# zijinxuxu/PDFNet

Measured on AMD Instinct MI355X. Metric: train-step images/sec @256x256 RGB-D B=32, higher is better.
Workload: dtype f32

## Files before the change

### include/pdfnet_hip.h

```cpp
#ifndef PDFNET_HIP_H
#define PDFNET_HIP_H
#ifdef __cplusplus
extern "C" {
#endif

#define PDF_E_BADARG (-1)
#define PDF_E_WORKSPACE (-2)
#define PDF_ACT_NONE 0
#define PDF_ACT_RELU 1
#define PDF_ACT_LRELU01 2


int pdf_linear_fwd(const float* x, const float* w, const float* bias, float* y,
                   int M, int N, int K, int ldx, int ldw, int ldy, int act, void* stream);
int pdf_linear_bwd_weight(const float* x, const float* dy, float* dw, float* db, float* ws, long ws_floats,
                          int M, int N, int K, int ldx, int lddy, int accumulate, void* stream);
long pdf_wgrad_workspace_floats(int M, int NI, int NJ);
int pdf_init(void);
int pdf_debug_init_device(void);
int pdf_debug_kernel_timing(int on);
int pdf_set_stats_output(float* part, long cap_floats);
long pdf_stats_result_tiles(void);
long pdf_stats_result_rows(void);
int pdf_set_bn_tile_stats(const float* part, long tiles, long rows_per_tile);
int pdf_debug_kernel_record_count(void);
int pdf_debug_kernel_record(int i, char* name, int cap, double* flops, double* bytes, float* ms);
int pdf_stream_wait(void* waiter, void* signaler);
int pdf_set_gemm_precision(int bf16);
int pdf_debug_gemm_precision(void);
int pdf_debug_last_tile(void);
int pdf_debug_igemm_launches(void);
int pdf_linear_bwd_data(const float* dy, const float* w, float* dx, int M, int N, int K, int lddy, int ldw, int lddx, void* stream);
int pdf_linear_fwd_pair(const float* x, const float* w0, const float* w1, const float* b0, const float* b1, float* y,
                        int M, int N, int K, int ldx, int ldw, int ldy, int act, void* stream);
int pdf_linear_bwd_data_pair(const float* dy, const float* w0, const float* w1, float* dx, int M, int N, int K,
                             int lddy, int ldw, int lddx, void* stream);
int pdf_linear_bwd_weight_pair(const float* x, const float* dy, float* dw0, float* dw1, float* db0, float* db1,
                               float* ws, long ws_floats, int M, int N, int K, int ldx, int lddy, int accumulate, void* stream);

int pdf_conv2d_fwd(const float* x, const float* w, const float* bias, float* y,
                   int N, int H, int W, int Cin, int ldx, int Cout, int KH, int KW,
                   int stride, int pad, int OH, int OW, int ldy, int act, void* stream);
int pdf_conv2d_bwd_data(const float* dy, const float* w, float* dx,
                        int N, int H, int W, int Cin, int lddx, int Cout, int KH, int KW,
                        int stride, int pad, int OH, int OW, int lddy, void* stream);
int pdf_conv2d_bwd_data_add(const float* dy, const float* w, float* dx,
                        int N, int H, int W, int Cin, int lddx, int Cout, int KH, int KW,
                        int stride, int pad, int OH, int OW, int lddy, void* stream);
int pdf_conv2d_bwd_weight(const float* x, const float* dy, float* dw, float* db, float* ws, long ws_floats,
                          int N, int H, int W, int Cin, int ldx, int Cout, int KH, int KW,
                          int stride, int pad, int OH, int OW, int lddy, int accumulate, void* stream);

int pdf_deconv2d_fwd(const float* x, const float* w, const float* bias, float* y,
                     int N, int H, int W, int Cin, int ldx, int Cout, int KH, int KW,
                     int stride, int pad, int OH, int OW, int ldy, void* stream);
int pdf_deconv2d_bwd_data(const float* dy, const float* w, float* dx,
                          int N, int H, int W, int Cin, int lddx, int Cout, int KH, int KW,
                          int stride, int pad, int OH, int OW, int lddy, void* stream);
int pdf_deconv2d_bwd_weight(const float* x, const float* dy, float* dw, float* ws, long ws_floats,
                            int N, int H, int W, int Cin, int ldx, int Cout, int KH, int KW,
                            int stride, int pad, int OH, int OW, int lddy, int accumulate, void* stream);
int pdf_bmm_strided(const float* A, const float* B, float* C, int batch, int M, int N, int K, int RB,
                    long sab, long sar, long sam, long sak, long sbb, long sbr, long sbk, long sbn,
                    long scb, long scm, long scn, int beta, void* stream);


int pdf_knn_ball_group(const float* pts, int ldp, int C, int Bc, int N, int S, int K, float r2,
                       int* idx, float* grouped, int ldg, void* stream);
int pdf_group_bwd(const float* dg, int ldg, const int* idx, float* dpts, int ldd, int C,
                  int Bc, int N, int S, int K, void* stream);
int pdf_gather_sub_fwd(const float* u, int ldu, const float* v, int ldv, const int* idx, int Bc, int N, int S, int K, int C,
                       float* y, int ldy, void* stream);
int pdf_gather_sub_bwd(const float* dy, int lddy, const int* idx, float* du, int ldu, float* dv, int ldv,
                       int Bc, int N, int S, int K, int C, void* stream);
int pdf_invert_index(const int* idx, int Bc, int N, int E, int* start, int* list, int* tmp, void* stream);
int pdf_gather_sub_bwd_sorted(const float* dy, int lddy, const int* start, const int* list, float* du, int ldu, float* dv, int ldv,
                              int Bc, int N, int S, int K, int C, void* stream);
int pdf_gather_rows(const float* feat, int ldf, int C, long HW, const long* ind, long ind_bstride,
                    int B, int M, int R, int shift, float* out, int ldo, void* stream);
int pdf_scatter_rows_add(const float* dout, int ldo, int C, long HW, const long* ind, long ind_bstride,
                         int B, int M, int R, int shift, float* dfeat, int ldf, void* stream);
int pdf_window_op(float* feat, int ldf, int C, int H, int W, const long* ind, long ind_bstride,
                  int B, int M, int r, float* buf, const float* src, int mode, void* stream);
int pdf_nms_top1(const float* hm, int BC, int H, int W, long* ind, float* score, void* stream);
int pdf_maxk_fwd(const float* x, int ldx, int C, long R, int K, float* y, int ldy, int* arg, void* stream);
int pdf_maxk_bwd(const float* dy, int ldy, const int* arg, int C, long R, int K, float* dx, int ldx, void* stream);
int pdf_bn_relu_maxk_fwd(const float* y, int ldy, int C, long R, int K, const float* gamma, const float* beta,
                         float* running_mean, float* running_var, float momentum, float eps, int training,
                         float* out, int ldo, int* arg, float* save_mean, float* save_rstd, float* scale, float* shift,
                         float* ws, void* stream);
int pdf_bn_relu_maxk_bwd(const float* dout, int lddo, const int* arg, const float* y, int ldy, const float* save_mean, const float* save_rstd,
                         const float* gamma, const float* scale, const float* shift, int C, long R, int K,
                         float* dy, int lddy, float* dgamma, float* dbeta, int accumulate, float* ws, void* stream);
long pdf_sa_fused_workspace_floats(int Bc, int S, int K, int C1, int C2, int C3);
int pdf_sa_fused_fwd(const float* u, const float* v, const int* idx, int Bc, int N, int S, int K, int C1, int C2, int C3,
                     const float* w2, const float* b2, const float* w3, const float* b3,
                     const float* gamma1, const float* beta1, const float* gamma2, const float* beta2, const float* gamma3, const float* beta3,
                     float* rmean1, float* rvar1, float* rmean2, float* rvar2, float* rmean3, float* rvar3, float momentum, float eps, int training,
                     float* out, int* arg, float* zsel, float* saved, float* ws, long ws_floats, void* stream);
int pdf_sa_fused_bwd(const float* dout, const float* u, const float* v, const int* idx, int Bc, int N, int S, int K, int C1, int C2, int C3,
                     const float* w2, const float* b2, const float* w3, const float* b3,
                     const float* out, const int* arg, const float* zsel, const float* saved,
                     float* dz1, float* dw2, float* db2, float* dw3, float* db3,
                     float* dgamma1, float* dbeta1, float* dgamma2, float* dbeta2, float* dgamma3, float* dbeta3,
                     float* ws, long ws_floats, void* stream);


long pdf_bn_workspace_floats(int C, long R);
int pdf_bn_train_fwd(const float* x, int ldx, int C, long R, const float* gamma, const float* beta,
                     float* running_mean, float* running_var, float momentum, float eps,
                     const float* res, int ldr, int relu, float* y, int ldy,
                     float* save_mean, float* save_rstd, float* scale, float* shift, float* ws, void* stream);
int pdf_bn_eval_fwd(const float* x, int ldx, int C, long R, const float* gamma, const float* beta,
                    const float* running_mean, const float* running_var, float eps,
                    const float* res, int ldr, int relu, float* y, int ldy, float* scale, float* shift, void* stream);
int pdf_bn_train_bwd(const float* dy, int lddy, const float* y, int ldy, int relu, const float* x, int ldx,
                     const float* save_mean, const float* save_rstd, const float* gamma,
                     const float* scale, const float* shift, int C, long R,
                     float* dx, int lddx, float* dres, int lddr, float* dgamma, float* dbeta, int accumulate,
                     float* ws, void* stream);
int pdf_bn_eval_bwd(const float* dy, int lddy, const float* y, int ldy, int relu, const float* x, int ldx,
                    const float* running_mean, const float* running_var, float eps, const float* scale, const float* shift,
                    int C, long R, float* dx, int lddx, float* dres, int lddr,
                    float* dgamma, float* dbeta, int accumulate, float* ws, void* stream);
int pdf_bn_relu_maxk_eval_bwd(const float* dout, int lddo, const int* arg, const float* y, int ldy,
                              const float* running_mean, const float* running_var, float eps, const float* scale, const float* shift,
                              int C, long R, int K, float* dy, int lddy, float* dgamma, float* dbeta, int accumulate, float* ws, void* stream);
int pdf_colsum(const float* g, int ldg, int C, long R, float* out, int accumulate, float* ws, void* stream);
int pdf_colsum_pair(const float* g, int ldg, int C, long R, float* out0, float* out1, int accumulate, float* ws, void* stream);
int pdf_layernorm_fwd(const float* x, int ldx, int F, long R, const float* gamma, const float* beta, float eps,
                      float* y, int ldy, float* mean, float* rstd, void* stream);
int pdf_layernorm_bwd(const float* dy, int lddy, const float* x, int ldx, int F, long R, const float* gamma,
                      const float* mean, const float* rstd, float* dx, int lddx, float* dgamma, float* dbeta, void* stream);
int pdf_layernorm_fused_fwd(const float* x, int ldx, const float* add, int ldadd, float p, unsigned long long seed,
                            const unsigned long long* step, int F, long R, long R_split,
                            const float* gamma0, const float* beta0, const float* gamma1, const float* beta1, float eps, int act,
                            float* z, int ldz, float* y, int ldy, float* mean, float* rstd, void* stream);
int pdf_layernorm_fused_bwd(const float* dy, int lddy, const float* y, int ldy, int act, const float* z, int ldz, int F, long R, long R_split,
                            const float* gamma0, const float* gamma1, const float* mean, const float* rstd,
                            const float* dz_in, int lddzin, float* dz, int lddz, float* dadd, int lddadd,
                            float p, unsigned long long seed, const unsigned long long* step,
                            float* dgamma0, float* dbeta0, float* dgamma1, float* dbeta1, void* stream);
int pdf_l2norm_fwd(const float* x, int ldx, int C, long R, const float* w, float eps, float* y, int ldy, float* norm, void* stream);
int pdf_l2norm_bwd(const float* dy, int lddy, const float* x, int ldx, int C, long R, const float* w, float eps,
                   const float* norm, float* dx, int lddx, float* dw, void* stream);
int pdf_l2norm_cat_fwd(int nparts, const float* const* x, const int* C, const float* const* w, float eps, long R,
                       float* y, int ldy, float* const* norm, void* stream);
int pdf_l2norm_cat_bwd(int nparts, const float* dy, int lddy, const float* const* x, const int* C, const float* const* w, float eps, long R,
                       float* const* norm, float* const* dx, float* const* dw, void* const* dx16_or_null, void* stream);

int pdf_act_fwd(const float* x, int ldx, float* y, int ldy, int C, long R, int act, void* stream);
int pdf_act_bwd(const float* dy, int lddy, const float* y, int ldy, float* dx, int lddx, int C, long R, int act, void* stream);
int pdf_sft_fwd(const float* fea, int ldf, const float* scale, int lds, const float* shift, int ldh,
                float* out, int ldo, int C, long R, void* stream);
int pdf_sft_bwd(const float* g, int ldg, const float* fea, int ldf, const float* scale, int lds,
                float* dfea, int lddf, float* dscale, int ldds, int C, long R, void* stream);
int pdf_sft3_fwd(const float* fea, int ldf, const float* cond, int ldc, const float* w_scale0, const float* b_scale0,
                 const float* w_scale1, const float* b_scale1, const float* w_shift0, const float* b_shift0,
                 const float* w_shift1, const float* b_shift1, float* out, int ldo, long R, void* stream);
int pdf_sft3_bwd(const float* g, int ldg, const float* fea, int ldf, const float* cond, int ldc,
                 const float* w_scale0, const float* b_scale0, const float* w_scale1, const float* b_scale1,
                 const float* w_shift0, const float* b_shift0, const float* w_shift1, const float* b_shift1,
                 float* dfea, int lddf, float* dcond, int lddc,
                 float* dw_scale0, float* db_scale0, float* dw_scale1, float* db_scale1,
                 float* dw_shift0, float* db_shift0, float* dw_shift1, float* db_shift1, int accumulate,
                 float* ws, long R, void* stream);
int pdf_set_bf16_operands(const void* op0_bf16, const void* op1_bf16);
int pdf_set_bf16_output(void* out_bf16);
int pdf_set_bn_input_bf16(const void* x16);
int pdf_set_input_affine_relu(const float* scale, const float* shift);
int pdf_cast_bf16(const float* src, void* dst, long n, void* stream);
int pdf_cast_bf16_transposed(const float* src, void* dst, const void* table, int nlayers, long total_tiles, void* stream);
int pdf_debug_shadow_operands(void);
int pdf_dropout(const float* x, float* y, long n, float p, unsigned long long seed, const unsigned long long* step, void* stream);
int pdf_dropout_add(const float* x, const float* res, float* y, long n, float p, unsigned long long seed,
                    const unsigned long long* step, void* stream);
int pdf_maxpool3s2_fwd(const float* x, int N, int H, int W, int C, float* y, unsigned char* arg, void* stream);
int pdf_maxpool3s2_bwd(const float* dy, const unsigned char* arg, int N, int H, int W, int C, float* dx, void* stream);
int pdf_maxpool3s2_bwd_add(const float* dy, const unsigned char* arg, int N, int H, int W, int C, float* dx, void* stream);
int pdf_upsample2x_fwd(const float* x, int N, int H, int W, int C, float* y, void* stream);
int pdf_upsample2x_bwd(const float* dy, int N, int H, int W, int C, float* dx, void* stream);
int pdf_pad2d(const float* src, int lds, long R, int C, float* dst, int ldd, long R2, int C2, void* stream);
int pdf_adam_step(float* p, const float* g, float* m, float* v, long n, float lr, float b1, float b2, float eps,
                  const float* corr, float grad_scale, void* stream);

int pdf_cheby2_fwd(const float* x, int ldx, int B, int V, int F, const int* col, const float* val, int Wd,
                   float* out, int ldo, void* stream);
int pdf_cheby2_bwd(const float* d, int ldd, int B, int V, int F, const int* colT, const float* valT, int Wd,
                   float* dx, int lddx, void* stream);
int pdf_cheby2_fwd_pair(const float* x, int ldx, int B, int V, int F, const int* col0, const float* val0,
                        const int* col1, const float* val1, int Wd, float* out, int ldo, void* stream);
int pdf_cheby2_bwd_pair(const float* d, int ldd, int B, int V, int F, const int* colT0, const float* valT0,
                        const int* colT1, const float* valT1, int Wd, float* dx, int lddx, void* stream);
int pdf_attn_fwd(const float* q, const float* k, const float* v, int ld, int B, int V, int H, int dh, int kv_shift,
                 float pdrop, unsigned long long seed, const unsigned long long* step, float* out, int ldo, float* stat, void* stream);
int pdf_attn_bwd(const float* q, const float* k, const float* v, int ld, const float* o, const float* dout, int ldo,
                 const float* stat, int B, int V, int H, int dh, int kv_shift, float pdrop, unsigned long long seed, const unsigned long long* step,
                 float* dq, float* dk, float* dv, int lddq, float* dvec, void* stream);

int pdf_fps(const float* xyz, int ld, int Bc, int N, int S, const int* start, int* idx, void* stream);

int pdf_rowloss_fwd(const float* pred, const float* tgt, long rows, long n, int mode, float* out, void* stream);
int pdf_rowloss_bwd(const float* pred, const float* tgt, const float* gout, long rows, long n, int mode, float* dpred, void* stream);
int pdf_face_loss_fwd(const float* pred, const float* gt, const long long* faces, int G, int B, int V, int Fc, float* part, void* stream);
int pdf_face_loss_bwd(const float* pred, const float* gt, const long long* faces, int G, int B, int V, int Fc,
                      const float* wn, const float* we, float* dpred, void* stream);

long pdf_dense_loss_workspace_floats(int B);
int pdf_dense_loss_fwd(const float* mask, const float* mask_gt, int mask_c, int mask_hw,
                       const float* hms, const float* hms_gt, int hms_c, int hms_hw,
                       const float* hm, const float* hm_gt, int hm_c, int hm_hw, int B, float* ws, float* out, void* stream);
int pdf_dense_loss_bwd(const float* mask, const float* mask_gt, float* dmask, int mask_c, int mask_hw,
                       const float* hms, const float* hms_gt, float* dhms, int hms_c, int hms_hw,
                       const float* hm, const float* hm_gt, float* dhm, int hm_c, int hm_hw, int B,
                       const float* g_mask, const float* g_hms, const float* g_hm, const float* stat, void* stream);
int pdf_point_dist_sum(const float* pred, const float* gt, int rows, int n, int dim, float* out, void* stream);

int pdf_procrustes_dist(const float* pred, const float* gt, int rows, int n, float* sum, float* dist, float* aligned, void* stream);
int pdf_mesh_nn_counts(const float* pred, const float* gt, int rows, int n, const float* thr, int T, int* counts, float* d_gt, float* d_pred,
                       void* stream);
int pdf_mesh_penetration(const float* verts, const long long* faces, int B, int n, int Fc,
                         float* wind, float* dist, int* count, float* depth, float* gap, void* stream);

int pdf_mesh_icp(const float* verts, const long long* faces, const float* cloud, const float* valid, int B, int n, int Fc, int P, int iters,
                 float trim, int rigid, float* out_verts, float* R, float* t, float* rms, int* inliers, float* closest, int* tri, void* stream);
int pdf_cloud_mesh_loss(const float* verts, const long long* faces, const float* cloud, const float* valid, int B, int n, int Fc, int P, float trim,
                        float* loss, int* inliers, float* grad, int* tri, float* closest, float* bary, void* stream);
int pdf_mesh_cloud_loss(const float* verts, const long long* faces, const float* cloud, const float* valid, int B, int n, int Fc, int P, float trim,
                        float margin, float* loss, int* inliers, int* visible, float* grad, int* vis, int* nn, void* stream);
int pdf_penetration_loss(const float* verts, const long long* faces, const float* valid, int B, int n, int Fc,
                         float* loss, int* count, float* grad_self, float* grad_other,
                         int* inside, int* tri, float* bary, float* closest, void* stream);
int pdf_silhouette_loss(const float* verts, const long long* faces, const float* K, const float* mask, const float* weight,
                        const float* valid, const int* table, int B, int n, int Fc, int M, int H, int W, float sigma, float z_near,
                        float* scratch, float* loss, float* sums, float* trans, float* grad, void* stream);

int pdf_render_hands(const float* verts, const long long* faces, const float* K, const float* valid, const float* colour, int colour_per_sample,
                     const int* table, int B, int n, int Fc, int M, int H, int W, float z_near, int ambient_only, float* scratch,
                     int* face, float* depth, float* bary, float* rgb, void* stream);
int pdf_render_compare(const int* face_pred, const int* face_gt, const float* depth_pred, const float* sensor, int B, int H, int W, int Fc,
                       int* iou, float* res, void* stream);

int pdf_depth2pcl(const float* depth, const float* mask, const float* K, const float* valid, int B, int H, int W,
                  unsigned long long seed, long* choose, float* cloud, int* count, void* stream);

int pdf_mano_lbs_fwd(const float* root_aa, const float* pose_aa, const float* shape, const float* trans,
                     const float* v_template, const float* shapedirs, const float* posedirs, const float* J_reg,
                     const float* weights, int B, int left_side, int center_idx, float* verts, float* joints, void* stream);
int pdf_mano_lbs_bwd(const float* root_aa, const float* pose_aa, const float* shape,
                     const float* v_template, const float* shapedirs, const float* posedirs, const float* J_reg,
                     const float* weights, int B, int left_side, int center_idx, const float* dverts, const float* djoints,
                     float* droot, float* dpose, float* dshape, float* dtrans, void* stream);
int pdf_mano_split_coeff(const float* params, int ldp, long HW, const long* ind, const float* K, int B, int input_res, int down,
                         float* orient, float* pose, float* shape, float* trans, void* stream);
int pdf_mano_split_coeff_bwd(const float* params, float* dparams, int ldp, long HW, const long* ind, const float* K, int B, int input_res, int down,
                             const float* dorient, const float* dpose, const float* dtrans, void* stream);

long pdf_mano_fit_workspace_floats(int B);
int pdf_mano_fit(const float* target, const float* valid, const float* weight, const float* init,
                 const float* v_template, const float* shapedirs, const float* posedirs, const float* J_reg, const float* weights,
                 int B, int left_side, int iters, float prior_pose, float prior_shape,
                 float* params, float* verts, float* joints, float* cost, int* info, float* lambda, float* A, float* g,
                 float* workspace, void* stream);
int pdf_mano_cloud_targets(const float* verts, const long long* faces, const float* cloud, const float* valid, const float* anchor,
                           float anchor_weight, int B, int n, int Fc, int P, float trim, float* target, float* weight, float* rms,
                           int* inliers, int* tri, float* closest, float* bary, void* stream);
long pdf_mano_fit_cloud_workspace_floats(int B, int outer);
int pdf_mano_fit_cloud(const float* cloud, const long long* faces, const float* valid, const float* init, const float* anchor,
                       float anchor_weight, float trim, int outer, int inner, float prior_pose, float prior_shape,
                       const float* v_template, const float* shapedirs, const float* posedirs, const float* J_reg, const float* weights,
                       int B, int Fc, int P, int left_side,
                       float* params, float* verts, float* joints, float* rms, int* inliers, float* cost, int* info,
                       float* workspace, void* stream);


typedef struct PdfCallOpts {
    const void* op0_bf16; const void* op1_bf16;
    void* out_bf16;
    const void* bn_x_bf16;
    float* stats_out; long stats_cap;
    long stats_tiles; long stats_rows;
    const float* tile_stats; long tile_n; long tile_rows;
    const float* in_scale; const float* in_shift;
    const void* op1_bf16_t;
    float* ws; long ws_floats;
    const float* wino_v;
} PdfCallOpts;
long pdf_conv2d_winograd_v_offset(int N, int H, int W, int Cin, int Cout, int KH, int KW, int stride, int pad);
int pdf_linear_fwd_x(const float* x, const float* w, const float* bias, float* y, int M, int N, int K, int ldx, int ldw, int ldy, int act, void* stream, PdfCallOpts* opts);
int pdf_linear_fwd_pair_x(const float* x, const float* w0, const float* w1, const float* b0, const float* b1, float* y, int M, int N, int K, int ldx, int ldw, int ldy, int act, void* stream, PdfCallOpts* opts);
int pdf_linear_bwd_data_x(const float* dy, const float* w, float* dx, int M, int N, int K, int lddy, int ldw, int lddx, void* stream, PdfCallOpts* opts);
int pdf_linear_bwd_data_pair_x(const float* dy, const float* w0, const float* w1, float* dx, int M, int N, int K, int lddy, int ldw, int lddx, void* stream, PdfCallOpts* opts);
int pdf_conv2d_fwd_x(const float* x, const float* w, const float* bias, float* y, int N, int H, int W, int Cin, int ldx, int Cout, int KH, int KW, int stride, int pad, int OH, int OW, int ldy, int act, void* stream, PdfCallOpts* opts);
int pdf_conv2d_bwd_data_x(const float* dy, const float* w, float* dx, int N, int H, int W, int Cin, int lddx, int Cout, int KH, int KW, int stride, int pad, int OH, int OW, int lddy, void* stream, PdfCallOpts* opts);
int pdf_conv2d_bwd_data_add_x(const float* dy, const float* w, float* dx, int N, int H, int W, int Cin, int lddx, int Cout, int KH, int KW, int stride, int pad, int OH, int OW, int lddy, void* stream, PdfCallOpts* opts);
int pdf_linear_bwd_weight_x(const float* x, const float* dy, float* dw, float* db, float* ws, long ws_floats, int M, int N, int K, int ldx, int lddy, int accumulate, void* stream, PdfCallOpts* opts);
int pdf_linear_bwd_weight_pair_x(const float* x, const float* dy, float* dw0, float* dw1, float* db0, float* db1, float* ws, long ws_floats, int M, int N, int K, int ldx, int lddy, int accumulate, void* stream, PdfCallOpts* opts);
int pdf_conv2d_bwd_weight_x(const float* x, const float* dy, float* dw, float* db, float* ws, long ws_floats, int N, int H, int W, int Cin, int ldx, int Cout, int KH, int KW, int stride, int pad, int OH, int OW, int lddy, int accumulate, void* stream, PdfCallOpts* opts);
int pdf_deconv2d_fwd_x(const float* x, const float* w, const float* bias, float* y, int N, int H, int W, int Cin, int ldx, int Cout, int KH, int KW, int stride, int pad, int OH, int OW, int ldy, void* stream, PdfCallOpts* opts);
int pdf_deconv2d_bwd_data_x(const float* dy, const float* w, float* dx, int N, int H, int W, int Cin, int lddx, int Cout, int KH, int KW, int stride, int pad, int OH, int OW, int lddy, void* stream, PdfCallOpts* opts);
int pdf_deconv2d_bwd_weight_x(const float* x, const float* dy, float* dw, float* ws, long ws_floats, int N, int H, int W, int Cin, int ldx, int Cout, int KH, int KW, int stride, int pad, int OH, int OW, int lddy, int accumulate, void* stream, PdfCallOpts* opts);
int pdf_bn_train_fwd_x(const float* x, int ldx, int C, long R, const float* gamma, const float* beta, float* running_mean, float* running_var, float momentum, float eps, const float* res, int ldr, int relu, float* y, int ldy, float* save_mean, float* save_rstd, float* scale, float* shift, float* ws, void* stream, PdfCallOpts* opts);
int pdf_bn_train_bwd_x(const float* dy, int lddy, const float* y, int ldy, int relu, const float* x, int ldx, const float* save_mean, const float* save_rstd, const float* gamma, const float* scale, const float* shift, int C, long R, float* dx, int lddx, float* dres, int lddr, float* dgamma, float* dbeta, int accumulate, float* ws, void* stream, PdfCallOpts* opts);
int pdf_bn_relu_maxk_fwd_x(const float* y, int ldy, int C, long R, int K, const float* gamma, const float* beta, float* running_mean, float* running_var, float momentum, float eps, int training, float* out, int ldo, int* arg, float* save_mean, float* save_rstd, float* scale, float* shift, float* ws, void* stream, PdfCallOpts* opts);
int pdf_l2norm_cat_fwd_x(int nparts, const float* const* x, const int* C, const float* const* w, float eps, long R, float* y, int ldy, float* const* norm, void* stream, PdfCallOpts* opts);
long pdf_conv2d_winograd_workspace_floats(int N, int H, int W, int Cin, int Cout, int KH, int KW, int stride, int pad, int backward);
int pdf_debug_armed_slots(void);
int pdf_debug_callopts_size(void);

int pdf_x3_split(const float* x, void* out, long n, long cs, void* stream);
long pdf_deconv2d_x3_workspace_floats(int N, int H, int W, int Cin, int Cout, int KH, int KW, int stride, int pad, int backward);
int pdf_set_x3_mode(int mode);
int pdf_stream_create(void** out, int priority, int* lo, int* hi);
int pdf_debug_x3_mode(void);
int pdf_debug_workspace_plan(int kind, int pass, int N, int H, int W, int Cin, int Cout, int KH, int KW, int stride, int pad, long* out, int cap);
int pdf_debug_x3_stamps(unsigned long long* out);
int pdf_x3_batched_gemm_nt(const void* A3, long csA, const void* B3, long csB, float* C, int batch, long gsA, long gsB, long gsC, int M, int N, int K, int variant, int nprod, void* stream);
int pdf_batched_gemm_nt(const float* A, const float* B, float* C, int batch, long gsA, long gsB, long gsC, int M, int N, int K, void* stream);
int pdf_x3_batched_gemm_tn(const void* P3, long csP, const void* Q3, long csQ, float* slab, int batch, long gsP, long gsQ, int M, int NI, int NJ, int splits, int variant, int nprod, void* stream);
int pdf_batched_gemm_tn(const float* P, const float* Q, float* slab, int batch, long gsP, long gsQ, int M, int NI, int NJ, int splits, void* stream);

typedef struct PdfMeshLin { const float* w[2]; const float* b[2]; } PdfMeshLin;
typedef struct PdfMeshLN { const float* g[2]; const float* b[2]; } PdfMeshLN;
typedef struct PdfMeshGcn { PdfMeshLin fc1, fc2, sc; PdfMeshLN n2, n3; unsigned long long seed; } PdfMeshGcn;
typedef struct PdfMeshAttn {
    PdfMeshLN ln; PdfMeshLin q, k, v, fc; PdfMeshLN ffln; PdfMeshLin f1, f2;
    unsigned long long seed_att, seed_z, seed_t, seed_x;
} PdfMeshAttn;
typedef struct PdfMeshLinG { float* w[2]; float* b[2]; } PdfMeshLinG;
typedef struct PdfMeshLNG { float* g[2]; float* b[2]; } PdfMeshLNG;
typedef struct PdfMeshGcnG { PdfMeshLinG fc1, fc2, sc; PdfMeshLNG n2, n3; } PdfMeshGcnG;
typedef struct PdfMeshAttnG { PdfMeshLNG ln; PdfMeshLinG q, k, v, fc; PdfMeshLNG ffln; PdfMeshLinG f1, f2; } PdfMeshAttnG;
typedef struct PdfMeshLevel {
    int level, B, training, cin0;
    float p;
    const unsigned long long* step;
    const float* x;
    float* out;
    const int* ell_col[2]; const float* ell_val[2]; const int* ell_colT[2]; const float* ell_valT[2]; int ell_w;
    PdfMeshGcn gcn[4];
    PdfMeshAttn self_, cross;
    float* tape;
    float* qkv;
    const float* dout;
    float* dx;
    float* gtape;
    PdfMeshGcnG ggcn[4]; PdfMeshAttnG gself, gcross;
    float* wg_ws; long wg_ws_floats;
} PdfMeshLevel;
long pdf_mesh_tape_floats(int level, int B);
long pdf_mesh_gtape_floats(int level, int B);
int pdf_mesh_level_fwd(const PdfMeshLevel* a, void* stream);
int pdf_mesh_level_bwd(const PdfMeshLevel* a, void* stream, void* side_stream);
int pdf_mesh_level_fwd_bf16(const PdfMeshLevel* a, void* stream);
int pdf_mesh_level_bwd_bf16(const PdfMeshLevel* a, void* stream, void* side_stream);
int pdf_mesh_level_fwd_x3(const PdfMeshLevel* a, void* stream);
int pdf_mesh_level_bwd_x3(const PdfMeshLevel* a, void* stream, void* side_stream);
int pdf_debug_mesh_level_size(void);

typedef struct PdfMeshLoss {
    const float* vp; const float* v2p; const float* hd3; const float* hd2; const float* r;
    const float* vgt[2]; const float* jgt[2]; const float* v2gt[2]; const float* lmsgt[2];
    const long long* ind; const float* K; const float* valid;
    const float* reg[2]; const long long* faces; const long long* perm[2];
    int B, Fc, size, down;
    float* part;
    float* out;
    float coef[12];
    const float* gmp;
    int edge_grad;
    float* dvp; float* dv2p; float* dhd3; float* dhd2; float* dr;
} PdfMeshLoss;
int pdf_mesh_loss_fwd(const PdfMeshLoss* a, void* stream);
int pdf_mesh_loss_bwd(const PdfMeshLoss* a, void* stream);
int pdf_debug_mesh_loss_size(void);
int pdf_debug_mesh_stamps(unsigned long long* out);

#ifdef __cplusplus
}
#endif
#endif
```

### pdfnet_amd/csrc/gemm.hip

```cpp
#include "common.h"

#include "gemm_common.h"
#include "gemm_internal.h"

constexpr int WG_ISSUE_AT = 1;
typedef unsigned int u32x4v __attribute__((ext_vector_type(4)));
__device__ __forceinline__ float4 as_f4(const u32x4v& v) { return *reinterpret_cast<const float4*>(&v); }

template <int BM, int BN, int WM, int WN, bool FAST, bool KN, int BKT, bool BUF, bool AFF>
__device__ __forceinline__ void igemm_nt_body(const IGemm& g) {
    constexpr int NT = WM * WN * 64;
    constexpr int BK = BKT, LD = BK + 1;
    constexpr int TM = BM / WM / 32, TN = BN / WN / 32;
    constexpr int TPR = BK / 4, RPP = NT / TPR;
    constexpr int RA = BM / RPP, RB = BN / RPP;
    __shared__ __attribute__((aligned(16))) float As[2][BM * LD];
    __shared__ __attribute__((aligned(16))) float Bs[2][BN * LD];

    const int tid = threadIdx.x, lane = tid & 63, wave = tid >> 6;
    const int wm = wave / WN, wn = wave % WN;
    const float* __restrict__ Ap = g.A; const float* __restrict__ Bp = g.B; const float* __restrict__ biasp = g.bias;
    float* __restrict__ Cp = g.C;
    if (g.batch > 0) { Ap += (long)blockIdx.y * g.gsA; Bp += (long)blockIdx.y * g.gsB; Cp += (long)blockIdx.y * g.gsC; }
    else if (blockIdx.y) { Ap += g.gsA; Cp += g.gsC; Bp = g.B1; biasp = g.bias1; }
// ... 1814 lines not shown
        if (g.q_scale != nullptr && g.uniform != 2) return PDF_E_BADARG;
        KTimer kt(buf && g.q_scale != nullptr ? "wgemm_tn_dma_aff" : buf ? "wgemm_tn_dma<3, true>" : fast ? "wgemm_tn_dma<3, false>" : "wgemm_tn<128, 128, 2, 2, false, 16>",
                  wflops, wbytes, s);
        if (buf && g.q_scale != nullptr) hipLaunchKernelGGL(wgemm_tn_dma_aff, grid, dim3(256), 0, s, g);
        else if (buf) hipLaunchKernelGGL((wgemm_tn_dma<3, true>), grid, dim3(256), 0, s, g);
        else if (fast) hipLaunchKernelGGL((wgemm_tn_dma<3, false>), grid, dim3(256), 0, s, g);
        else hipLaunchKernelGGL((wgemm_tn<128, 128, 2, 2, false>), grid, dim3(256), 0, s, g);
    }
    PDF_LAUNCH_CHECK();
    if (splits > 1) {
        Reduce r = {ws, out, out1, per, bws, db, db1, (int)perb, splits, accumulate};
        const bool two_d = splits >= 16 && per <= (1L << 20);
        KTimer kt(two_d ? "reduce_slabs_2d" : "reduce_slabs", 0.0, 4.0 * groups * (splits + 1 + (accumulate ? 1 : 0)) * (per + perb), s);
        if (two_d) {
            const int mb = (int)((per + 63) / 64);
            hipLaunchKernelGGL(reduce_slabs_2d, dim3(mb + (int)((perb + 63) / 64), groups), dim3(256), 0, s, r, mb);
        } else {
            const int mb = grid_for(per);
            hipLaunchKernelGGL(reduce_slabs, dim3(mb + (perb ? cdiv(perb, 256) : 0), groups), dim3(256), 0, s, r, mb);
        }
        PDF_LAUNCH_CHECK();
    }
    return 0;
}

PDF_API long pdf_wgrad_workspace_floats(int M, int NI, int NJ) {
    const bool small = (NI <= 64 || NJ <= 64);
    const int B = small ? 64 : 128;
    long tiles = (long)cdiv(NI, B) * cdiv(NJ, B);
    int splits = (int)((1024 + tiles - 1) / tiles);
    int max_by_rows = cdiv(M, 128);
    if (splits > max_by_rows) splits = max_by_rows;
    if (splits < 1) splits = 1;
    return (long)splits * ((long)NI * NJ + NI);
}

static int pdf_linear_bwd_weight_impl(const float* x, const float* dy, float* dw, float* db, float* ws, long ws_floats,
                                  int M, int N, int K, int ldx, int lddy, int accumulate, void* stream, PdfCallOpts& co) {
    hipStream_t s = (hipStream_t)stream;
    WGemm g = {};
    g.P = dy; g.Q = x; g.M = M; g.NI = N; g.Cq = K; g.T = 1; g.ldp = lddy; g.ldq = ldx; g.ldw = K;
    g.plain_q = 1; g.H = 1; g.W = M; g.QH = 1; g.QW = M; g.sy = 1; g.sx = 1;
    g.dy[0] = 0; g.dx[0] = 0; g.wt[0] = 0;
    g.Q16 = co.op0_bf16; g.P16 = co.op1_bf16;
    g.q_scale = co.in_scale; g.q_shift = co.in_shift;
    return launch_wgemm(g, dw, ws, ws_floats, accumulate, s, nullptr, db);
}
PDF_API int pdf_linear_bwd_weight_x(const float* x, const float* dy, float* dw, float* db, float* ws, long ws_floats,
                                  int M, int N, int K, int ldx, int lddy, int accumulate, void* stream, PdfCallOpts* opts) {
    return pdf_call_x(opts, pdf_linear_bwd_weight_impl, x, dy, dw, db, ws, ws_floats, M, N, K, ldx, lddy, accumulate, stream);
}
PDF_API int pdf_linear_bwd_weight(const float* x, const float* dy, float* dw, float* db, float* ws, long ws_floats,
                                  int M, int N, int K, int ldx, int lddy, int accumulate, void* stream) {
    return pdf_call_plain(pdf_linear_bwd_weight_impl, x, dy, dw, db, ws, ws_floats, M, N, K, ldx, lddy, accumulate, stream);
}


static int pdf_linear_bwd_weight_pair_impl(const float* x, const float* dy, float* dw0, float* dw1, float* db0, float* db1,
                                       float* ws, long ws_floats, int M, int N, int K, int ldx, int lddy, int accumulate, void* stream, PdfCallOpts& co) {
    hipStream_t s = (hipStream_t)stream;
    WGemm g = {};
    g.P = dy; g.Q = x; g.M = M; g.NI = N; g.Cq = K; g.T = 1; g.ldp = lddy; g.ldq = ldx; g.ldw = K;
    g.plain_q = 1; g.H = 1; g.W = M; g.QH = 1; g.QW = M; g.sy = 1; g.sx = 1;
    g.dy[0] = 0; g.dx[0] = 0; g.wt[0] = 0;
    g.gsP = (long)M * lddy; g.gsQ = (long)M * ldx;
    return launch_wgemm(g, dw0, ws, ws_floats, accumulate, s, dw1, db0, db1);
}
PDF_API int pdf_linear_bwd_weight_pair_x(const float* x, const float* dy, float* dw0, float* dw1, float* db0, float* db1,
                                       float* ws, long ws_floats, int M, int N, int K, int ldx, int lddy, int accumulate, void* stream, PdfCallOpts* opts) {
    return pdf_call_x(opts, pdf_linear_bwd_weight_pair_impl, x, dy, dw0, dw1, db0, db1, ws, ws_floats, M, N, K, ldx, lddy, accumulate, stream);
}
PDF_API int pdf_linear_bwd_weight_pair(const float* x, const float* dy, float* dw0, float* dw1, float* db0, float* db1,
                                       float* ws, long ws_floats, int M, int N, int K, int ldx, int lddy, int accumulate, void* stream) {
    return pdf_call_plain(pdf_linear_bwd_weight_pair_impl, x, dy, dw0, dw1, db0, db1, ws, ws_floats, M, N, K, ldx, lddy, accumulate, stream);
}



__global__ __launch_bounds__(256) void stem7x7_wgrad_kernel(const float* __restrict__ x, const float* __restrict__ dy, float* __restrict__ part,
                                                            int N, int H, int W, int OH, int OW, int lddy, int cpb) {
    constexpr int CH = 64, XW = 2 * CH + 5, RW = XW * 3, XF = 7 * RW, ZB = 2800, DYB = 3200, NJ = 147, NJP = 160;
    __shared__ __attribute__((aligned(16))) float sm[64 * NJP];
    float* Xs = sm;
    float* dYs = sm + DYB;
    const int tid = threadIdx.x, lane = tid & 63, wave = tid >> 6;
    for (int i = XF + tid; i < DYB; i += 256) sm[i] = 0.f;
    int boff[5];
#pragma unroll
    for (int t = 0; t < 5; ++t) {
        const int j = 32 * t + (lane & 31);
        const int tap = j / 3, ci = j - tap * 3, ky = tap / 7, kx = tap - ky * 7;
        boff[t] = j < NJ ? (ky * XW + kx) * 3 + ci : ZB;
    }
    const int wa = wave & 1, kh = wave >> 1;
    f32x16 acc[5];
#pragma unroll
    for (int t = 0; t < 5; ++t)
#pragma unroll
        for (int r = 0; r < 16; ++r) acc[t][r] = 0.f;
    const int cpr = OW / CH;
    const long total = (long)N * OH * cpr;
    const long c0 = (long)blockIdx.x * cpb, c1 = min(total, c0 + cpb);
    typedef float v4f __attribute__((ext_vector_type(4)));
    float xr[14]; v4f dr[4];
    auto gload = [&](long c) {
        const int n = (int)(c / ((long)OH * cpr));
        const int rem = (int)(c - (long)n * OH * cpr);
        const int oy = rem / cpr, ox0 = (rem - oy * cpr) * CH;
        const int lin0 = (2 * ox0 - 3) * 3;
#pragma unroll
        for (int r = 0; r < 7; ++r) {
            const int iy = 2 * oy - 3 + r;
            const float* row = x + ((long)(n * H + iy) * W) * 3;
#pragma unroll
            for (int h = 0; h < 2; ++h) {
                const int e = tid + 256 * h, lin = lin0 + e;
                const bool ok = iy >= 0 && iy < H && e < RW && lin >= 0 && lin < 3 * W;
                xr[r * 2 + h] = ok ? row[lin] : 0.f;
            }
        }
#pragma unroll
        for (int q = 0; q < 4; ++q) {
            const int e = tid + 256 * q, px = e >> 4, c4 = (e & 15) * 4;
            dr[q] = *reinterpret_cast<const v4f*>(&dy[((long)(n * OH + oy) * OW + ox0 + px) * lddy + c4]);
        }
    };
    if (c0 < c1) gload(c0);
    for (long c = c0; c < c1; ++c) {
        __syncthreads();
#pragma unroll
        for (int r = 0; r < 7; ++r)
#pragma unroll
            for (int h = 0; h < 2; ++h) { const int e = tid + 256 * h; if (e < RW) Xs[r * RW + e] = xr[r * 2 + h]; }
#pragma unroll
        for (int q = 0; q < 4; ++q) { const int e = tid + 256 * q; *reinterpret_cast<v4f*>(&dYs[(e >> 4) * 64 + (e & 15) * 4]) = dr[q]; }
        __syncthreads();
        if (c + 1 < c1) gload(c + 1);
#pragma unroll
        for (int ks = 0; ks < 16; ++ks) {
            const int px = 32 * kh + 2 * ks + (lane >> 5);
            const float a0 = dYs[px * 64 + 32 * wa + (lane & 31)];
            float b[5];
#pragma unroll
            for (int t = 0; t < 5; ++t) b[t] = Xs[boff[t] + px * 6];
#pragma unroll
            for (int t = 0; t < 5; ++t) acc[t] = __builtin_amdgcn_mfma_f32_32x32x2f32(a0, b[t], acc[t], 0, 0, 0);
        }
    }
    __syncthreads();
    for (int i = tid; i < 64 * NJP; i += 256) sm[i] = 0.f;
    __syncthreads();
#pragma unroll
    for (int t = 0; t < 5; ++t)
#pragma unroll
        for (int r = 0; r < 16; ++r) {
            const int co = 32 * wa + (r & 3) + 8 * (r >> 2) + 4 * (lane >> 5), j = 32 * t + (lane & 31);
            atomicAdd(&sm[co * NJP + j], acc[t][r]);
        }
    __syncthreads();
    for (int i = tid; i < 64 * NJ; i += 256) {
        const int co = i / NJ, j = i - co * NJ;
        part[(long)blockIdx.x * (64 * NJ) + i] = sm[co * NJP + j];
    }
}

static int pdf_conv2d_bwd_weight_impl(const float* x, const float* dy, float* dw, float* db, float* ws, long ws_floats,
                                  int N, int H, int W, int Cin, int ldx, int Cout, int KH, int KW,
                                  int stride, int pad, int OH, int OW, int lddy, int accumulate, void* stream, PdfCallOpts& co) {
    hipStream_t s = (hipStream_t)stream;
    if (KH * KW > MAX_TAPS) return PDF_E_BADARG;
    if (!g_gemm_bf16 && co.ws != nullptr && dy != nullptr && OH == H && OW == W && ldx % 4 == 0 && lddy % 4 == 0 && aligned16(x) && aligned16(dy) &&
        aligned16(co.ws)) {
        const WinoWgradPlan plan = wino_wgrad_plan(N, H, W, Cin, Cout, KH, KW, stride, pad);
        if (plan.ok && co.ws_floats >= plan.total)
            return pdf_internal_conv3x3_winograd_wgrad(plan, x, ldx, dy, lddy, dw, db, co.ws, accumulate, aligned16(co.wino_v) ? co.wino_v : nullptr, s);
    }
    if (dy == nullptr && (co.op1_bf16 == nullptr || db != nullptr || !g_gemm_bf16 || Cin % 16 != 0 || Cout % 16 != 0 || lddy % 8 != 0)) return PDF_E_BADARG;
    if (Cin == 3 && Cout == 3 && KH == 3 && KW == 3 && stride == 1 && db == nullptr && (long)N * OH * OW >= (1L << 16) && ws_floats >= 81L * 64) {
        const int nblk = (int)min((long)1024, ws_floats / 81);
        KTimer kt("tiny_conv_wgrad_kernel<3, 3, 3, 3> + reduce_slabs_2d", 2.0 * N * OH * OW * 81, 4.0 * N * (H * W + OH * OW) * 3, s);
        hipLaunchKernelGGL((tiny_conv_wgrad_kernel<3, 3, 3, 3>), dim3(nblk), dim3(256), 0, s, x, dy, ws, N, H, W, ldx, pad, OH, OW, lddy);
        Reduce r = {ws, dw, nullptr, 81, nullptr, nullptr, nullptr, 0, nblk, accumulate};
        hipLaunchKernelGGL(reduce_slabs_2d, dim3(2, 1), dim3(256), 0, s, r, 2);
        PDF_LAUNCH_CHECK();
        return 0;
    }
    if (Cin == 3 && ldx == 3 && Cout == 64 && KH == 7 && KW == 7 && stride == 2 && pad == 3 && db == nullptr && OW % 64 == 0 && OH * 2 == H && OW * 2 == W &&
        lddy % 4 == 0 && aligned16(dy) && ws_floats >= 64L * 147 * 64 && env_int(ENV_WG_STEM, 1)) {
        const long total = (long)N * OH * (OW / 64);
        int nblk = (int)min(min((long)512, ws_floats / (64 * 147)), total);
        const int cpb = (int)cdiv(total, nblk);
        nblk = (int)cdiv(total, cpb);
        KTimer kt("stem7x7_wgrad_kernel + reduce_slabs_2d", 2.0 * N * OH * OW * 64 * 147, 4.0 * N * ((double)H * W * 3 + (double)OH * OW * 64), s);
        hipLaunchKernelGGL(stem7x7_wgrad_kernel, dim3(nblk), dim3(256), 0, s, x, dy, ws, N, H, W, OH, OW, lddy, cpb);
        Reduce r = {ws, dw, nullptr, 64L * 147, nullptr, nullptr, nullptr, 0, nblk, accumulate};
        const int mb = (64 * 147 + 63) / 64;
        hipLaunchKernelGGL(reduce_slabs_2d, dim3(mb, 1), dim3(256), 0, s, r, mb);
        PDF_LAUNCH_CHECK();
        return 0;
    }
    if (Cout <= 4 && KH == 1 && KW == 1 && stride == 1 && pad == 0 && Cin % 4 == 0 && Cin <= 1024 && 256 % (Cin / 4) == 0 && ldx % 4 == 0 && aligned16(x)) {
        const long per = (long)Cout * Cin, perb = db ? Cout : 0;
        const int M = N * OH * OW;
        int nblk = (int)min((long)1024, ws_floats / (per + perb));
        if (nblk >= 1) {
            const int rpb = cdiv(M, nblk);
            nblk = cdiv(M, rpb);
            float* bws = ws + (long)nblk * per;
            KTimer kt("narrow_wgrad_kernel + reduce_slabs_2d", 2.0 * M * Cout * Cin, 4.0 * M * (Cout + Cin), s);
            hipLaunchKernelGGL(narrow_wgrad_kernel, dim3(nblk), dim3(256), 0, s, dy, x, ws, db ? bws : nullptr, M, Cout, Cin, lddy, ldx, rpb);
            Reduce r = {ws, dw, nullptr, per, bws, db, nullptr, (int)perb, nblk, accumulate};
            const int mb = (int)((per + 63) / 64);
            hipLaunchKernelGGL(reduce_slabs_2d, dim3(mb + (int)((perb + 63) / 64), 1), dim3(256), 0, s, r, mb);
            PDF_LAUNCH_CHECK();
            return 0;
        }
    }
    WGemm g = {};
    g.P = dy; g.Q = x; g.M = N * OH * OW; g.NI = Cout; g.Cq = Cin; g.T = KH * KW;
    g.ldp = lddy; g.ldq = ldx; g.ldw = KH * KW * Cin;
    g.H = H; g.W = W; g.QH = OH; g.QW = OW; g.sy = stride; g.sx = stride;
    g.plain_q = (KH == 1 && KW == 1 && stride == 1 && pad == 0) ? 1 : 0;
    for (int ky = 0; ky < KH; ++ky)
        for (int kx = 0; kx < KW; ++kx) {
            int t = ky * KW + kx;
            g.dy[t] = (int)(ky - pad); g.dx[t] = (int)(kx - pad); g.wt[t] = t;
        }
    g.Q16 = co.op0_bf16; g.P16 = co.op1_bf16;
    return launch_wgemm(g, dw, ws, ws_floats, accumulate, s, nullptr, db);
}
PDF_API int pdf_conv2d_bwd_weight_x(const float* x, const float* dy, float* dw, float* db, float* ws, long ws_floats,
                                  int N, int H, int W, int Cin, int ldx, int Cout, int KH, int KW,
                                  int stride, int pad, int OH, int OW, int lddy, int accumulate, void* stream, PdfCallOpts* opts) {
    return pdf_call_x(opts, pdf_conv2d_bwd_weight_impl, x, dy, dw, db, ws, ws_floats, N, H, W, Cin, ldx, Cout, KH, KW, stride, pad, OH, OW, lddy,
                      accumulate, stream);
}
PDF_API int pdf_conv2d_bwd_weight(const float* x, const float* dy, float* dw, float* db, float* ws, long ws_floats,
                                  int N, int H, int W, int Cin, int ldx, int Cout, int KH, int KW,
                                  int stride, int pad, int OH, int OW, int lddy, int accumulate, void* stream) {
    return pdf_call_plain(pdf_conv2d_bwd_weight_impl, x, dy, dw, db, ws, ws_floats, N, H, W, Cin, ldx, Cout, KH, KW, stride, pad, OH, OW, lddy,
                          accumulate, stream);
}


static int pdf_deconv2d_fwd_impl(const float* x, const float* w, const float* bias, float* y,
                             int N, int H, int W, int Cin, int ldx, int Cout, int KH, int KW,
                             int stride, int pad, int OH, int OW, int ldy, void* stream, PdfCallOpts& co) {
    hipStream_t s = (hipStream_t)stream;
    if (KH * KW > MAX_TAPS) return PDF_E_BADARG;
    if (!g_gemm_bf16 && co.ws != nullptr && ldx == Cin && ldy == Cout && aligned16(co.ws)) {
        const X3DeconvPlan plan = x3_deconv_plan(N, H, W, Cin, Cout, KH, KW, stride, pad, 0);
        if (plan.ok && OH == plan.OH && OW == plan.OW && co.ws_floats >= plan.total) return pdf_internal_x3_deconv_fwd(plan, x, w, bias, y, co.ws, ldy, s);
    }
    if (KH == stride && KW == stride && pad == 0) {
        IGemm g = {};
        g.A = x; g.B = w; g.C = y; g.bias = bias; g.A16 = co.op0_bf16; g.B16 = co.op1_bf16;
        g.M = N * H * W; g.N = KH * KW * Cout; g.K = Cin; g.Cin = Cin; g.lda = ldx; g.ldc = ldy;
        g.ldb = KH * KW * Cout; g.b_kn = 1; g.btap = 0;
        g.T = 1; g.plain_in = 1; g.plain_out = 0; g.dy[0] = 0; g.dx[0] = 0; g.wt[0] = 0;
        g.H = H; g.W = W; g.QH = H; g.QW = W; g.sy = 1; g.sx = 1;
        g.OH = OH; g.OW = OW; g.osy = stride; g.osx = stride; g.ooy = 0; g.oox = 0;
        g.ps_cout = Cout; g.ps_kw = KW;
        return launch_igemm(g, s);
    }
    for (int py = 0; py < stride; ++py)
        for (int px = 0; px < stride; ++px) {
            IGemm g = {};
            g.A = x; g.B = w; g.C = y; g.bias = bias; g.A16 = co.op0_bf16; g.B16 = co.op1_bf16;
            g.N = Cout; g.Cin = Cin; g.lda = ldx; g.ldb = KH * KW * Cout; g.b_kn = 1; g.btap = Cout; g.ldc = ldy;
            g.H = H; g.W = W;
            g.QH = (OH - py + stride - 1) / stride; g.QW = (OW - px + stride - 1) / stride;
            if (g.QH <= 0 || g.QW <= 0) continue;
            g.M = N * g.QH * g.QW;
            g.sy = 1; g.sx = 1;
            const int T = pdf_parity_taps(KH, KW, stride, pad, py, px, g.dy, g.dx, g.wt);
            if (T == 0) return PDF_E_BADARG;
            g.T = T; g.K = T * Cin;
            g.plain_in = 0; g.plain_out = 0;
            g.OH = OH; g.OW = OW; g.osy = stride; g.osx = stride; g.ooy = py; g.oox = px;
            int rc = launch_igemm(g, s);
            if (rc) return rc;
        }
    return 0;
}
PDF_API int pdf_deconv2d_fwd_x(const float* x, const float* w, const float* bias, float* y,
                             int N, int H, int W, int Cin, int ldx, int Cout, int KH, int KW,
                             int stride, int pad, int OH, int OW, int ldy, void* stream, PdfCallOpts* opts) {
    return pdf_call_x(opts, pdf_deconv2d_fwd_impl, x, w, bias, y, N, H, W, Cin, ldx, Cout, KH, KW, stride, pad, OH, OW, ldy, stream);
}
PDF_API int pdf_deconv2d_fwd(const float* x, const float* w, const float* bias, float* y,
                             int N, int H, int W, int Cin, int ldx, int Cout, int KH, int KW,
                             int stride, int pad, int OH, int OW, int ldy, void* stream) {
    return pdf_call_plain(pdf_deconv2d_fwd_impl, x, w, bias, y, N, H, W, Cin, ldx, Cout, KH, KW, stride, pad, OH, OW, ldy, stream);
}


static int pdf_deconv2d_bwd_data_impl(const float* dy, const float* w, float* dx,
                                  int N, int H, int W, int Cin, int lddx, int Cout, int KH, int KW,
                                  int stride, int pad, int OH, int OW, int lddy, void* stream, PdfCallOpts& co) {
    hipStream_t s = (hipStream_t)stream;
    if (KH * KW > MAX_TAPS) return PDF_E_BADARG;
    if (!g_gemm_bf16 && co.ws != nullptr && lddy == Cout && lddx >= Cin && aligned16(co.ws)) {
        const X3DeconvPlan plan = x3_deconv_plan(N, H, W, Cin, Cout, KH, KW, stride, pad, 1);
        if (plan.ok && OH == plan.OH && OW == plan.OW && co.ws_floats >= plan.total) return pdf_internal_x3_deconv_bwd_data(plan, dy, w, dx, co.ws, lddx, lddy, s);
    }
    IGemm g = {};
    g.A = dy; g.B = w; g.C = dx; g.bias = nullptr; g.A16 = co.op0_bf16; g.B16 = co.op1_bf16;
    g.M = N * H * W; g.N = Cin; g.K = KH * KW * Cout; g.Cin = Cout; g.lda = lddy; g.ldb = KH * KW * Cout; g.ldc = lddx;
    g.H = OH; g.W = OW; g.QH = H; g.QW = W; g.sy = stride; g.sx = stride;
    conv_taps(g, KH, KW, pad, 1);
    g.plain_in = 0; g.plain_out = 1;
    return launch_igemm(g, s);
}
PDF_API int pdf_deconv2d_bwd_data_x(const float* dy, const float* w, float* dx,
                                  int N, int H, int W, int Cin, int lddx, int Cout, int KH, int KW,
                                  int stride, int pad, int OH, int OW, int lddy, void* stream, PdfCallOpts* opts) {
    return pdf_call_x(opts, pdf_deconv2d_bwd_data_impl, dy, w, dx, N, H, W, Cin, lddx, Cout, KH, KW, stride, pad, OH, OW, lddy, stream);
}
PDF_API int pdf_deconv2d_bwd_data(const float* dy, const float* w, float* dx,
                                  int N, int H, int W, int Cin, int lddx, int Cout, int KH, int KW,
                                  int stride, int pad, int OH, int OW, int lddy, void* stream) {
    return pdf_call_plain(pdf_deconv2d_bwd_data_impl, dy, w, dx, N, H, W, Cin, lddx, Cout, KH, KW, stride, pad, OH, OW, lddy, stream);
}


static int pdf_deconv2d_bwd_weight_impl(const float* x, const float* dy, float* dw, float* ws, long ws_floats,
                                    int N, int H, int W, int Cin, int ldx, int Cout, int KH, int KW,
                                    int stride, int pad, int OH, int OW, int lddy, int accumulate, void* stream, PdfCallOpts& co) {
    hipStream_t s = (hipStream_t)stream;
    if (KH * KW > MAX_TAPS) return PDF_E_BADARG;
    if (!g_gemm_bf16 && co.ws != nullptr && ldx == Cin && lddy == Cout && aligned16(co.ws)) {
        const X3DeconvPlan plan = x3_deconv_plan(N, H, W, Cin, Cout, KH, KW, stride, pad, 2);
        if (plan.ok && OH == plan.OH && OW == plan.OW && co.ws_floats >= plan.total) return pdf_internal_x3_deconv_bwd_weight(plan, x, dy, dw, co.ws, lddy, accumulate, s);
    }
    WGemm g = {};
    g.P = x; g.Q = dy; g.P16 = co.op0_bf16; g.Q16 = co.op1_bf16; g.M = N * H * W; g.NI = Cin; g.Cq = Cout; g.T = KH * KW;
    g.ldp = ldx; g.ldq = lddy; g.ldw = KH * KW * Cout;
    g.H = OH; g.W = OW; g.QH = H; g.QW = W; g.sy = stride; g.sx = stride; g.plain_q = 0;
    for (int ky = 0; ky < KH; ++ky)
        for (int kx = 0; kx < KW; ++kx) {
            int t = ky * KW + kx;
            g.dy[t] = (int)(ky - pad); g.dx[t] = (int)(kx - pad); g.wt[t] = t;
        }
    return launch_wgemm(g, dw, ws, ws_floats, accumulate, s);
}
PDF_API int pdf_deconv2d_bwd_weight_x(const float* x, const float* dy, float* dw, float* ws, long ws_floats,
                                    int N, int H, int W, int Cin, int ldx, int Cout, int KH, int KW,
                                    int stride, int pad, int OH, int OW, int lddy, int accumulate, void* stream, PdfCallOpts* opts) {
    return pdf_call_x(opts, pdf_deconv2d_bwd_weight_impl, x, dy, dw, ws, ws_floats, N, H, W, Cin, ldx, Cout, KH, KW, stride, pad, OH, OW, lddy,
                      accumulate, stream);
}
PDF_API int pdf_deconv2d_bwd_weight(const float* x, const float* dy, float* dw, float* ws, long ws_floats,
                                    int N, int H, int W, int Cin, int ldx, int Cout, int KH, int KW,
                                    int stride, int pad, int OH, int OW, int lddy, int accumulate, void* stream) {
    return pdf_call_plain(pdf_deconv2d_bwd_weight_impl, x, dy, dw, ws, ws_floats, N, H, W, Cin, ldx, Cout, KH, KW, stride, pad, OH, OW, lddy,
                          accumulate, stream);
}
```

### pdfnet_amd/csrc/gemm_internal.h

```cpp
#pragma once
#include "common.h"

int pdf_internal_batched_gemm(const float* A, const float* B, float* C, int batch, long gsA, long gsB, long gsC, int M, int N, int K, hipStream_t s);
int pdf_internal_batched_wgemm(const float* P, const float* Q, float* slab, int batch, long gsP, long gsQ, int M, int NI, int NJ, int splits, hipStream_t s);

struct WsRegion { long off, len; };

struct WinoPlan {
    int ok;
    int N, H, W, Ck, Cn, flip;
    int m;
    long T, P;
    int x3;
    int shared_v_x3;
    WsRegion U, V, M;
    long total;
    long v_offset;
};
WinoPlan wino_plan(int N, int H, int W, int Ck, int Cn, int KH, int KW, int stride, int pad, int flip);
int pdf_internal_conv3x3_winograd(const WinoPlan& p, const float* x, int ldx, const float* w, const float* bias, float* y, int ldy, float* ws,
                                  int act, int accum, const float* v_shared, hipStream_t s);
struct WinoWgradPlan {
    int ok;
    int N, H, W, Cin, Cout;
    long T;
    int x3;
    int shared_v_x3;
    int splits;
    WsRegion V, Yh, slab, colsum;
    long total;
};
WinoWgradPlan wino_wgrad_plan(int N, int H, int W, int Cin, int Cout, int KH, int KW, int stride, int pad);
int pdf_internal_conv3x3_winograd_wgrad(const WinoWgradPlan& p, const float* x, int ldx, const float* dy, int lddy, float* dw, float* db, float* ws,
                                        int accumulate, const float* v_cached, hipStream_t s);

int pdf_internal_x3_mode();
int pdf_internal_x3_batched_gemm(const void* A3, long csA, const void* B3, long csB, float* C, int batch, long gsA, long gsB, long gsC,
                                 int M, int N, int K, int variant, int nprod, hipStream_t s);
int pdf_internal_x3_batched_wgemm(const void* P3, long csP, const void* Q3, long csQ, float* slab, int batch, long gsP, long gsQ,
                                  int M, int NI, int NJ, int splits, int variant, int nprod, hipStream_t s);
struct X3Operand { long off, len, ld, cs; };
struct X3DeconvPlan {
    int ok;
    int pass, general;
    int N, H, W, Cin, Cout, K, stride, pad, OH, OW;
    X3Operand w, a;
    int splits;
    WsRegion slab;
    long total;
};
X3DeconvPlan x3_deconv_plan(int N, int H, int W, int Cin, int Cout, int KH, int KW, int stride, int pad, int pass);
int pdf_internal_x3_deconv_fwd(const X3DeconvPlan& p, const float* x, const float* w, const float* bias, float* y, float* ws, int ldy, hipStream_t s);
int pdf_internal_x3_deconv_bwd_data(const X3DeconvPlan& p, const float* dy, const float* w, float* dx, float* ws, int lddx, int lddy, hipStream_t s);
int pdf_internal_x3_deconv_bwd_weight(const X3DeconvPlan& p, const float* x, const float* dy, float* dw, float* ws, int lddy, int accumulate, hipStream_t s);
```

### pdfnet_amd/csrc/gemm_x3.hip

```cpp
#include "gemm_common.h"
#include "gemm_internal.h"
#include <cstdio>

typedef __bf16 bf16x8v __attribute__((ext_vector_type(8)));
typedef short s16x4v __attribute__((ext_vector_type(4)));
typedef short s16x8v __attribute__((ext_vector_type(8)));
typedef int i32x4 __attribute__((ext_vector_type(4)));

__device__ __forceinline__ i32x4 x3_rsrc(const void* p, unsigned bytes) {
    const unsigned long long a = (unsigned long long)p;
    i32x4 r = {(int)(unsigned)(a & 0xffffffffu), (int)(unsigned)((a >> 32) & 0xffffu), (int)bytes, 0x00020000};
    return r;
}
__device__ __forceinline__ void x3_dma16(const i32x4& rsrc, unsigned lds_addr, unsigned voff) {
    asm volatile("s_mov_b32 m0, %0\n\tbuffer_load_dwordx4 %1, %2, 0 offen lds" ::"s"(lds_addr), "v"(voff), "s"(rsrc) : "memory");
}

__global__ __launch_bounds__(256) void x3_split_kernel(const float* __restrict__ x, unsigned short* __restrict__ o, long n8, long cs) {
    for (long i = blockIdx.x * 256L + threadIdx.x; i < n8; i += (long)gridDim.x * 256) {
        const float4 u = reinterpret_cast<const float4*>(x)[2 * i], v = reinterpret_cast<const float4*>(x)[2 * i + 1];
        uint4 h, m, l;
        pdf_x3_split2(u.x, u.y, h.x, m.x, l.x); pdf_x3_split2(u.z, u.w, h.y, m.y, l.y);
        pdf_x3_split2(v.x, v.y, h.z, m.z, l.z); pdf_x3_split2(v.z, v.w, h.w, m.w, l.w);
        *reinterpret_cast<uint4*>(o + 8 * i) = h;
// ... 432 lines not shown

    f32x16 acc[TM][TN];
#if X3_SPLIT_ACC
    f32x16 acc2[TM][TN];
#endif
#pragma unroll
    for (int a = 0; a < TM; ++a)
#pragma unroll
        for (int c = 0; c < TN; ++c)
#pragma unroll
            for (int r = 0; r < 16; ++r) {
                acc[a][c][r] = 0.f;
#if X3_SPLIT_ACC
                acc2[a][c][r] = 0.f;
#endif
            }

    const int fg = lane >> 4, fq = (lane & 15) >> 2, fp = lane & 3;
    const int fk = 8 * (fg >> 1) + fq;
    int pfo[TM], qfo[TN];
#pragma unroll
    for (int i = 0; i < TM; ++i) {
        const int col = (wm * TM + i) * 32 + 16 * (fg & 1) + 4 * fp;
        pfo[i] = fk * BI * 2 + (((col >> 3) ^ swzp(fk)) << 4) + (col & 7) * 2;
    }
#pragma unroll
    for (int j = 0; j < TN; ++j) {
        const int col = (wn * TN + j) * 32 + 16 * (fg & 1) + 4 * fp;
        qfo[j] = 3 * PIMG + fk * BJ * 2 + (((col >> 3) ^ swzq(fk)) << 4) + (col & 7) * 2;
    }
    typedef __attribute__((address_space(3))) s16x4v lds_s16x4;
    auto frag = [&](const unsigned char* p, int rowbytes) {
        const s16x4v lo = __builtin_amdgcn_ds_read_tr16_b64_v4i16((lds_s16x4*)(p));
        const s16x4v hi = __builtin_amdgcn_ds_read_tr16_b64_v4i16((lds_s16x4*)(p + 4 * rowbytes));
        s16x8v v = __builtin_shufflevector(lo, hi, 0, 1, 2, 3, 4, 5, 6, 7);
        return *reinterpret_cast<bf16x8v*>(&v);
    };

#pragma unroll
    for (int p = 0; p < ST - 1; ++p) {
        begin_issue(p);
#pragma unroll
        for (int q = 0; q < NIP + NIQ; ++q) piece(q);
    }
    int st = 0, stn = ST - 1;
    constexpr int NG = 2 * TM * TN, NP = NIP + NIQ, NR = (TM + TN) * 3;
    constexpr int NSLOT = NG * NPROD / 2;
    constexpr int RSL = NSLOT / 2 - 1 > 0 ? NSLOT / 2 - 1 : 1;
    using PR = X3Prod<NPROD>;
    for (int kt = 0; kt < nk; ++kt) {
        asm volatile("s_waitcnt vmcnt(%0)" ::"n"((ST - 2) * (NIP + NIQ)) : "memory");
        asm volatile("s_barrier" ::: "memory");
        begin_issue(stn);
        const unsigned char* sp = smem + st * STAGE;
        bf16x8v af[2][TM][3], bf[2][TN][3];
        auto read1 = [&](int ks, int q) {
            if (q < TM * 3) { const int i = q / 3, c = q % 3; af[ks][i][c] = frag(sp + c * PIMG + ks * 16 * BI * 2 + pfo[i], BI * 2); }
            else { const int j = (q - TM * 3) / 3, c = (q - TM * 3) % 3; bf[ks][j][c] = frag(sp + c * QIMG + ks * 16 * BJ * 2 + qfo[j], BJ * 2); }
        };
#pragma unroll
        for (int q = 0; q < NR; ++q) read1(0, q);
        __builtin_amdgcn_sched_barrier(0);
#pragma unroll
        for (int q = 0; q < NG * NPROD; ++q) {
            const int gi = q / NPROD, pr = q % NPROD;
            const int ks = gi / (TM * TN), i = (gi / TN) % TM, j = gi % TN;
#if X3_SPLIT_ACC
            if (PR::a[pr] + PR::b[pr] != 0) acc2[i][j] = __builtin_amdgcn_mfma_f32_32x32x16_bf16(af[ks][i][PR::a[pr]], bf[ks][j][PR::b[pr]], acc2[i][j], 0, 0, 0);
            else
#endif
            acc[i][j] = __builtin_amdgcn_mfma_f32_32x32x16_bf16(af[ks][i][PR::a[pr]], bf[ks][j][PR::b[pr]], acc[i][j], 0, 0, 0);
            if (q % 2 == 1 || q == NG * NPROD - 1) {
                const int slot = q / 2;
                __builtin_amdgcn_sched_barrier(0);
#pragma unroll
                for (int r = slot * NR / RSL; r < (slot + 1) * NR / RSL && r < NR; ++r)
                    if (slot < RSL) read1(1, r);
                if (slot % 2 == 0 && slot / 2 < NP) piece(slot / 2);
                if (slot == NSLOT - 1) {
#pragma unroll
                    for (int p = (NSLOT + 1) / 2; p < NP; ++p) piece(p);
                }
                __builtin_amdgcn_sched_barrier(0);
            }
        }
        st = st == ST - 1 ? 0 : st + 1;
        stn = stn == ST - 1 ? 0 : stn + 1;
    }
    asm volatile("s_waitcnt vmcnt(0)\n\ts_barrier" ::: "memory");
#if X3_SPLIT_ACC
#pragma unroll
    for (int a = 0; a < TM; ++a)
#pragma unroll
        for (int c = 0; c < TN; ++c) acc[a][c] += acc2[a][c];
#endif

    const int h = lane >> 5;
    const bool whole = i0 + BI <= NI && (double)NI * NJ * 4.0 < 4294967000.0;
    const auto rsW = __builtin_amdgcn_make_buffer_rsrc((void*)Wb, 0, whole ? (unsigned)NI * (unsigned)NJ * 4u : 0u, 0x00020000);
    const unsigned ldw4 = (unsigned)NJ * 4u;
#pragma unroll
    for (int j = 0; j < TN; ++j) {
        const int col = j0 + (wn * TN + j) * 32 + (lane & 31);
        const bool cok = col < NJ;
#pragma unroll
        for (int i = 0; i < TM; ++i) {
            const int r0 = i0 + (wm * TM + i) * 32 + 4 * h;
            if (whole) {
                const unsigned vo = cok ? (unsigned)(r0 * NJ + col) * 4u : 0xffffffffu;
                float v[16];
#pragma unroll
                for (int r = 0; r < 16; ++r) v[r] = acc[i][j][r];
                if (g.accum) {
#pragma unroll
                    for (int r = 0; r < 16; ++r) v[r] += __builtin_bit_cast(float, __builtin_amdgcn_raw_buffer_load_b32(rsW, vo, ((r & 3) + 8 * (r >> 2)) * ldw4, 0));
                }
#pragma unroll
                for (int r = 0; r < 16; ++r)
                    __builtin_amdgcn_raw_buffer_store_b32(__builtin_bit_cast(unsigned, v[r]), rsW, vo, ((r & 3) + 8 * (r >> 2)) * ldw4, 0);
            } else {
#pragma unroll
                for (int r = 0; r < 16; ++r) {
                    const int row = r0 + (r & 3) + 8 * (r >> 2);
                    if (cok && row < NI) Wb[(long)row * NJ + col] = acc[i][j][r] + (g.accum ? Wb[(long)row * NJ + col] : 0.f);
                }
            }
        }
    }
}

template <int WM, int WN, int TM, int TN, int ST>
static int x3_launch_tn(const X3Gemm& g, int nprod, hipStream_t s) {
    constexpr int BI = WM * TM * 32, BJ = WN * TN * 32;
    const dim3 grid((unsigned)(cdiv(g.M, BI) * cdiv(g.N, BJ) * g.splits * g.batch));
    char nm[96];
    snprintf(nm, sizeof nm, g.T > 0 ? "x3gemm_tn<%d, %d, %d, %d, %d, %d, true>" : "x3gemm_tn<%d, %d, %d, %d, %d, %d>", WM, WN, TM, TN, ST, g.T > 0 ? 6 : nprod);
    KTimer kt(nm, 2.0 * g.batch * g.K * g.M * g.N, g.batch * (6.0 * g.K * ((double)g.M + g.N) + 4.0 * g.splits * g.M * g.N), s);
    if (g.T > 0) hipLaunchKernelGGL((x3gemm_tn<WM, WN, TM, TN, ST, 6, true>), grid, dim3(WM * WN * 64), 0, s, g);
    else if (nprod == 9) hipLaunchKernelGGL((x3gemm_tn<WM, WN, TM, TN, ST, 9>), grid, dim3(WM * WN * 64), 0, s, g);
    else if (nprod == 3) hipLaunchKernelGGL((x3gemm_tn<WM, WN, TM, TN, ST, 3>), grid, dim3(WM * WN * 64), 0, s, g);
    else hipLaunchKernelGGL((x3gemm_tn<WM, WN, TM, TN, ST, 6>), grid, dim3(WM * WN * 64), 0, s, g);
    PDF_LAUNCH_CHECK();
    return 0;
}

static int x3_launch_tn_deconv(const X3Gemm& g, hipStream_t s) {
    if (g.M % 256 == 0 && (long)(g.M / 256) * cdiv(g.N, 128) * g.splits * g.batch >= 256) return x3_launch_tn<4, 2, 2, 2, 2>(g, 6, s);
    return x3_launch_tn<2, 4, 2, 1, 3>(g, 6, s);
}
int pdf_internal_x3_tn_splits(int M, int splits) {
    const int rps = cdiv(cdiv(M, splits < 1 ? 1 : splits), 32) * 32;
    return cdiv(M, rps);
}
int pdf_internal_x3_batched_wgemm(const void* P3, long csP, const void* Q3, long csQ, float* slab, int batch, long gsP, long gsQ,
                                  int M, int NI, int NJ, int splits, int variant, int nprod, hipStream_t s) {
    if (NI % 8 != 0 || NJ % 8 != 0 || M < 32 || M % 32 != 0 || batch < 1) return PDF_E_BADARG;
    if (2.0 * csP + (double)M * NI >= 2147483000.0 || 2.0 * csQ + (double)M * NJ >= 2147483000.0) return PDF_E_BADARG;
    X3Gemm g = {};
    g.A = (const unsigned short*)P3; g.B = (const unsigned short*)Q3; g.C = slab;
    g.csA = csP; g.csB = csQ; g.gsA = gsP; g.gsB = gsQ;
    g.M = NI; g.N = NJ; g.K = M; g.batch = batch;
    g.splits = pdf_internal_x3_tn_splits(M, splits);
    g.rows_per_split = cdiv(cdiv(M, splits < 1 ? 1 : splits), 32) * 32;
    int rc;
    if (variant < 0) variant = (NI % 256 == 0 && (long)(NI / 256) * cdiv(NJ, 128) * g.splits * batch >= 512) ? 2 : 0;
    if (variant == 3) rc = x3_launch_tn<2, 4, 2, 1, 3>(g, nprod, s);
    else if (variant == 1) rc = x3_launch_tn<2, 2, 2, 1, 3>(g, nprod, s);
    else if (variant == 2) rc = x3_launch_tn<4, 2, 2, 2, 2>(g, nprod, s);
    else rc = x3_launch_tn<2, 2, 2, 2, 3>(g, nprod, s);
    return rc != 0 ? (rc < 0 ? rc : -rc) : g.splits;
}
PDF_API int pdf_x3_batched_gemm_tn(const void* P3, long csP, const void* Q3, long csQ, float* slab, int batch, long gsP, long gsQ,
                                   int M, int NI, int NJ, int splits, int variant, int nprod, void* stream) {
    hipStream_t s = (hipStream_t)stream;
    const int rc = pdf_internal_x3_batched_wgemm(P3, csP, Q3, csQ, slab, batch, gsP, gsQ, M, NI, NJ, splits, variant, nprod, s);
    return rc > 0 ? 0 : (rc == 0 ? PDF_E_BADARG : rc);
}
PDF_API int pdf_batched_gemm_tn(const float* P, const float* Q, float* slab, int batch, long gsP, long gsQ, int M, int NI, int NJ, int splits, void* stream) {
    hipStream_t s = (hipStream_t)stream;
    const int rc = pdf_internal_batched_wgemm(P, Q, slab, batch, gsP, gsQ, M, NI, NJ, splits, s);
    return rc > 0 ? 0 : (rc == 0 ? PDF_E_BADARG : rc);
}

struct X3TrJobs { long in_off[16], out_off[16]; };
__global__ __launch_bounds__(256) void x3_split_transpose_kernel(const float* __restrict__ w, long ldw, unsigned short* __restrict__ o, int K, int N, long ldo, long cs,
                                                                 const X3TrJobs jobs) {
    __shared__ float sm[64][65];
    w += jobs.in_off[blockIdx.z]; o += jobs.out_off[blockIdx.z];
    const int tk = blockIdx.y * 64, tn = blockIdx.x * 64, t = threadIdx.x;
#pragma unroll
    for (int i = 0; i < 4; ++i) {
        const int r = t / 16 + 16 * i, c = (t % 16) * 4;
        float4 v = make_float4(0.f, 0.f, 0.f, 0.f);
        if (tk + r < K && tn + c < N) v = *reinterpret_cast<const float4*>(w + (long)(tk + r) * ldw + tn + c);
        sm[r][c] = v.x; sm[r][c + 1] = v.y; sm[r][c + 2] = v.z; sm[r][c + 3] = v.w;
    }
    __syncthreads();
    const int n = t / 4, k0 = (t % 4) * 16;
    if (tn + n < N && tk + k0 < K) {
        uint4 h[2], m[2], l[2];
#pragma unroll
        for (int q = 0; q < 2; ++q) {
            unsigned* hh = reinterpret_cast<unsigned*>(&h[q]); unsigned* mm = reinterpret_cast<unsigned*>(&m[q]); unsigned* ll = reinterpret_cast<unsigned*>(&l[q]);
#pragma unroll
            for (int e = 0; e < 4; ++e) pdf_x3_split2(sm[k0 + 8 * q + 2 * e][n], sm[k0 + 8 * q + 2 * e + 1][n], hh[e], mm[e], ll[e]);
        }
        unsigned short* d = o + (long)(tn + n) * ldo + tk + k0;
#pragma unroll
        for (int q = 0; q < 2; ++q) {
            *reinterpret_cast<uint4*>(d + 8 * q) = h[q];
            *reinterpret_cast<uint4*>(d + cs + 8 * q) = m[q];
            *reinterpret_cast<uint4*>(d + 2 * cs + 8 * q) = l[q];
        }
    }
}
__global__ __launch_bounds__(256) void x3_split_unshuffle_kernel(const float* __restrict__ dy, int lddy, unsigned short* __restrict__ o, long ldo, long cs,
                                                                 long M, int QH, int QW, int OH, int OW, int s, int C) {
    const int C8 = C / 8, T = s * s;
    const long total = M * T * C8;
    for (long i = blockIdx.x * 256L + threadIdx.x; i < total; i += (long)gridDim.x * 256) {
        const int c8 = (int)(i % C8);
        const long r = i / C8;
        const int tap = (int)(r % T);
        const long m = r / T;
        const int ky = tap / s, kx = tap - ky * s;
        const int hw = QH * QW, ni = (int)(m / hw), rem = (int)(m - (long)ni * hw), qy = rem / QW, qx = rem - qy * QW;
        const float* src = dy + (((long)ni * OH + qy * s + ky) * OW + qx * s + kx) * lddy + c8 * 8;
        const float4 u = *reinterpret_cast<const float4*>(src), v = *reinterpret_cast<const float4*>(src + 4);
        uint4 h, mm, l;
        pdf_x3_split2(u.x, u.y, h.x, mm.x, l.x); pdf_x3_split2(u.z, u.w, h.y, mm.y, l.y);
        pdf_x3_split2(v.x, v.y, h.z, mm.z, l.z); pdf_x3_split2(v.z, v.w, h.w, mm.w, l.w);
        unsigned short* d = o + m * ldo + (long)tap * C + c8 * 8;
        *reinterpret_cast<uint4*>(d) = h;
        *reinterpret_cast<uint4*>(d + cs) = mm;
        *reinterpret_cast<uint4*>(d + 2 * cs) = l;
    }
}
static int g_x3_mode = -1;
int pdf_internal_x3_mode() {
    if (g_x3_mode < 0) {
        int v = getenv("PDF_X3") ? (atoi(getenv("PDF_X3")) ? 7 : 0) : 7;
        if (getenv("PDF_X3_DECONV") && !atoi(getenv("PDF_X3_DECONV"))) v &= ~2;
        if (getenv("PDF_X3_MESH") && !atoi(getenv("PDF_X3_MESH"))) v &= ~4;
        g_x3_mode = v;
    }
    return g_x3_mode;
}
PDF_API int pdf_set_x3_mode(int mode) { g_x3_mode = mode < 0 ? -1 : (mode & 7); return 0; }
PDF_API int pdf_debug_x3_mode(void) { return pdf_internal_x3_mode(); }
static long x3_ld(long K) { return K + 64; }
static long x3_floats(long n) { return ((3 * n + 1) / 2 + 3) / 4 * 4; }
static bool x3_carve(X3Operand& o, long& at, long rows, long K, int zrow) {
    o.ld = x3_ld(K); o.cs = (rows + zrow) * o.ld; o.off = at; o.len = x3_floats(o.cs);
    at += o.len;
    return 3.0 * o.cs < 2147483000.0;
}
static int x3_general_wgrad_splits(long M, int NI, long NJ) {
    const long tiles = (long)cdiv(NI, 128) * cdiv(NJ, 128);
    long sp = (512 + tiles - 1) / tiles;
    if (sp > M / 2048) sp = M / 2048;
    return (int)(sp < 1 ? 1 : sp);
}
X3DeconvPlan x3_deconv_plan(int N, int H, int W, int Cin, int Cout, int KH, int KW, int stride, int pad, int pass) {
    X3DeconvPlan p = {};
    if (!(pdf_internal_x3_mode() & 2) || KH != KW || stride < 2 || Cin % 32 != 0 || Cout % 32 != 0) return p;
    const int K = KH;
    p.pass = pass; p.general = K != stride || pad != 0;
    p.N = N; p.H = H; p.W = W; p.Cin = Cin; p.Cout = Cout; p.K = K; p.stride = stride; p.pad = pad;
    p.OH = (H - 1) * stride - 2 * pad + K; p.OW = (W - 1) * stride - 2 * pad + K;
    const long Min = (long)N * H * W, Mout = (long)N * p.OH * p.OW, NT = (long)K * K * Cout;
    bool fits;
    if (!p.general) {
        if (Min < 1024 || 2.0 * Min * NT * Cin < 3.0e10) return p;
        if (pass == 2 && (Min % 32 != 0 || 3.0 * Cin * NT * 4.0 >= 4294967000.0)) return p;
        fits = pass == 2 ? x3_carve(p.w, p.total, Min, Cin, 0) : pass ? x3_carve(p.w, p.total, Cin, NT, 0) : x3_carve(p.w, p.total, NT, Cin, 0);
        fits &= pass ? x3_carve(p.a, p.total, Min, NT, 0) : x3_carve(p.a, p.total, Min, Cin, 0);
    } else {
        if (K % stride != 0 || K * K > 16 || K <= stride || pad < 0 || pad >= K || p.OH % stride != 0 || p.OW % stride != 0) return p;
        if (2.0 * Min * K * K * Cin * Cout < 3.0e10) return p;
        if (pass == 2) {
            if ((H & (H - 1)) || (W & (W - 1)) || Min % 32 != 0 || Cout % 128 != 0) return p;
            fits = x3_carve(p.w, p.total, Min, Cin, 0);
            fits &= x3_carve(p.a, p.total, Mout, Cout, 1);
            p.splits = x3_general_wgrad_splits(Min, Cin, NT);
            p.slab = {p.total, (long)p.splits * Cin * NT};
            p.total += p.slab.len;
        } else if (pass == 0) {
            const long T = (long)(K / stride) * (K / stride);
            fits = x3_carve(p.w, p.total, (long)stride * stride * Cout, T * Cin, 0);
            fits &= x3_carve(p.a, p.total, Min, Cin, 1);
        } else {
            fits = x3_carve(p.w, p.total, Cin, NT, 0);
            fits &= x3_carve(p.a, p.total, Mout, Cout, 1);
        }
    }
    p.total += 64;
    if (!fits) { p = X3DeconvPlan{}; return p; }
    p.ok = 1;
    return p;
}
PDF_API long pdf_deconv2d_x3_workspace_floats(int N, int H, int W, int Cin, int Cout, int KH, int KW, int stride, int pad, int backward) {
    return pdf_debug_gemm_precision() ? 0 : x3_deconv_plan(N, H, W, Cin, Cout, KH, KW, stride, pad, backward).total;
}
static void x3_gemm_desc(X3Gemm& g, const void* A3, long csA, long lda, const void* B3, long csB, long ldb, float* C, int M, int N, int K, int ldc) {
    g = X3Gemm{};
    g.A = (const unsigned short*)A3; g.B = (const unsigned short*)B3; g.C = C;
    g.csA = csA; g.csB = csB; g.M = M; g.N = N; g.K = K; g.batch = 1; g.ldc = ldc; g.lda = (int)lda; g.ldb = (int)ldb;
    g.col_major_tiles = cdiv(N, 128) > 4 * cdiv(M, 128);
}
static int x3_launch_auto(const X3Gemm& g, hipStream_t s) {
    const int v = x3_nt_variant(g.M, g.N, g.K, g.batch);
    if (v == 0) return x3_launch_nt<4, 2, 2, 2, 2>(g, 6, s);
    if (v == 1) return x3_launch_nt<2, 2, 2, 2, 3>(g, 6, s);
    return x3_launch_nt<2, 4, 2, 1, 3>(g, 6, s);
}
static int x3_zero_rows(unsigned short* o3, const X3Operand& o, hipStream_t s) {
    for (int c = 0; c < 3; ++c)
        if (hipMemsetAsync(o3 + c * o.cs + o.cs - o.ld, 0, (size_t)o.ld * 2, s) != hipSuccess) return PDF_E_BADARG;
    return 0;
}
static void x3_split_unshuffle(const float* dy, int lddy, unsigned short* o3, const X3DeconvPlan& p, hipStream_t s) {
    const long M = (long)p.N * p.H * p.W, NT = (long)p.K * p.K * p.Cout;
    KTimer kt("x3_split_unshuffle_kernel", 0.0, 10.0 * M * NT, s);
    hipLaunchKernelGGL(x3_split_unshuffle_kernel, dim3(grid_for(M * NT / 8, 256, 256 * 16)), dim3(256), 0, s, dy, lddy, o3, p.a.ld, p.a.cs, M, p.H, p.W, p.OH, p.OW, p.stride, p.Cout);
}
static void x3_all_taps(X3Gemm& g, const X3DeconvPlan& p) {
    g.QH = p.H; g.QW = p.W; g.AH = p.OH; g.AW = p.OW; g.sy = p.stride; g.sx = p.stride; g.T = p.K * p.K; g.Cc = p.Cout; g.zrow = p.a.cs - p.a.ld;
    for (int ky = 0; ky < p.K; ++ky)
        for (int kx = 0; kx < p.K; ++kx) { g.tdy[ky * p.K + kx] = ky - p.pad; g.tdx[ky * p.K + kx] = kx - p.pad; }
}
int pdf_internal_x3_deconv_fwd(const X3DeconvPlan& p, const float* x, const float* w, const float* bias, float* y, float* ws, int ldy, hipStream_t s) {
    const int N = p.N, H = p.H, W = p.W, Cin = p.Cin, Cout = p.Cout, K = p.K, stride = p.stride;
    const long M = (long)N * H * W;
    unsigned short* w3 = reinterpret_cast<unsigned short*>(ws + p.w.off);
    unsigned short* x3 = reinterpret_cast<unsigned short*>(ws + p.a.off);
    if (!p.general) {
        const long NT = (long)K * K * Cout;
        {
            KTimer kt("x3_split_transpose_kernel", 0.0, 10.0 * NT * Cin, s);
            hipLaunchKernelGGL(x3_split_transpose_kernel, dim3((unsigned)cdiv(NT, 64), (unsigned)cdiv(Cin, 64)), dim3(256), 0, s, w, NT, w3, Cin, (int)NT, p.w.ld, p.w.cs, X3TrJobs{});
        }
        hipLaunchKernelGGL(x3_split_rows_kernel, dim3(grid_for(M * Cin / 8, 256, 256 * 16)), dim3(256), 0, s, x, (long)Cin, x3, p.a.ld, p.a.cs, M, Cin / 8);
        PDF_LAUNCH_CHECK();
        X3Gemm g;
        x3_gemm_desc(g, x3, p.a.cs, p.a.ld, w3, p.w.cs, p.w.ld, y, (int)M, (int)NT, Cin, ldy);
        g.ps_cout = Cout; g.ps_kw = K; g.ps_s = stride; g.QH = H; g.QW = W; g.OH = p.OH; g.OW = p.OW; g.bias = bias;
        return x3_launch_auto(g, s);
    }
    const int T = (K / stride) * (K / stride), P = stride * stride;
    if (P > 4 || P * T > 16) return PDF_E_BADARG;
    int tdy[4][16], tdx[4][16], wt[16];
    X3TrJobs jobs = {};
    for (int pc = 0; pc < P; ++pc) {
        if (pdf_parity_taps(K, K, stride, p.pad, pc / stride, pc % stride, tdy[pc], tdx[pc], wt) != T) return PDF_E_BADARG;
        for (int n = 0; n < T; ++n) {
            jobs.in_off[pc * T + n] = (long)wt[n] * Cout;
            jobs.out_off[pc * T + n] = (long)pc * Cout * p.w.ld + (long)n * Cin;
        }
    }
    {
        KTimer kt("x3_split_transpose_kernel", 0.0, 10.0 * K * K * Cout * Cin, s);
        hipLaunchKernelGGL(x3_split_transpose_kernel, dim3((unsigned)cdiv(Cout, 64), (unsigned)cdiv(Cin, 64), (unsigned)(P * T)), dim3(256), 0, s,
                           w, (long)K * K * Cout, w3, Cin, Cout, p.w.ld, p.w.cs, jobs);
    }
    hipLaunchKernelGGL(x3_split_rows_kernel, dim3(grid_for(M * Cin / 8, 256, 256 * 16)), dim3(256), 0, s, x, (long)Cin, x3, p.a.ld, p.a.cs, M, Cin / 8);
    if (int rc = x3_zero_rows(x3, p.a, s)) return rc;
    PDF_LAUNCH_CHECK();
    for (int pc = 0; pc < P; ++pc) {
        const int py = pc / stride, px = pc % stride, QH = (p.OH - py + stride - 1) / stride, QW = (p.OW - px + stride - 1) / stride;
        X3Gemm g;
        x3_gemm_desc(g, x3, p.a.cs, p.a.ld, w3 + (long)pc * Cout * p.w.ld, p.w.cs, p.w.ld, y, N * QH * QW, Cout, T * Cin, ldy);
        g.ps_cout = Cout; g.ps_kw = 1; g.ps_s = stride; g.QH = QH; g.QW = QW; g.OH = p.OH; g.OW = p.OW; g.ooy = py; g.oox = px; g.bias = bias;
        g.AH = H; g.AW = W; g.sy = 1; g.sx = 1; g.T = T; g.Cc = Cin; g.zrow = p.a.cs - p.a.ld;
        for (int n = 0; n < T; ++n) { g.tdy[n] = tdy[pc][n]; g.tdx[n] = tdx[pc][n]; }
        if (int rc = x3_launch_auto(g, s)) return rc;
    }
    return 0;
}
int pdf_internal_x3_deconv_bwd_data(const X3DeconvPlan& p, const float* dy, const float* w, float* dx, float* ws, int lddx, int lddy, hipStream_t s) {
    const int Cin = p.Cin, Cout = p.Cout;
    const long M = (long)p.N * p.H * p.W, Mout = (long)p.N * p.OH * p.OW, NT = (long)p.K * p.K * Cout;
    unsigned short* w3 = reinterpret_cast<unsigned short*>(ws + p.w.off);
    unsigned short* d3 = reinterpret_cast<unsigned short*>(ws + p.a.off);
    {
        KTimer kt("x3_split_rows_kernel", 0.0, 10.0 * NT * Cin, s);
        hipLaunchKernelGGL(x3_split_rows_kernel, dim3(grid_for(NT * Cin / 8, 256, 256 * 16)), dim3(256), 0, s, w, NT, w3, p.w.ld, p.w.cs, (long)Cin, (int)(NT / 8));
    }
    X3Gemm g;
    x3_gemm_desc(g, d3, p.a.cs, p.a.ld, w3, p.w.cs, p.w.ld, dx, (int)M, Cin, (int)NT, lddx);
    if (!p.general) x3_split_unshuffle(dy, lddy, d3, p, s);
    else {
        {
            KTimer kt("x3_split_rows_kernel", 0.0, 10.0 * Mout * Cout, s);
            hipLaunchKernelGGL(x3_split_rows_kernel, dim3(grid_for(Mout * Cout / 8, 256, 256 * 16)), dim3(256), 0, s, dy, (long)lddy, d3, p.a.ld, p.a.cs, Mout, Cout / 8);
        }
        if (int rc = x3_zero_rows(d3, p.a, s)) return rc;
        x3_all_taps(g, p);
    }
    PDF_LAUNCH_CHECK();
    return x3_launch_auto(g, s);
}

__global__ __launch_bounds__(256) void x3_slab_reduce_kernel(const float* __restrict__ slab, int splits, long n4, float* __restrict__ dw, int accumulate) {
    for (long i = blockIdx.x * 256L + threadIdx.x; i < n4; i += (long)gridDim.x * 256) {
        float4 v = reinterpret_cast<const float4*>(slab)[i];
        for (int y = 1; y < splits; ++y) { const float4 u = reinterpret_cast<const float4*>(slab)[(long)y * n4 + i]; v.x += u.x; v.y += u.y; v.z += u.z; v.w += u.w; }
        if (accumulate) { const float4 u = reinterpret_cast<const float4*>(dw)[i]; v.x += u.x; v.y += u.y; v.z += u.z; v.w += u.w; }
        reinterpret_cast<float4*>(dw)[i] = v;
    }
}
int pdf_internal_x3_deconv_bwd_weight(const X3DeconvPlan& p, const float* x, const float* dy, float* dw, float* ws, int lddy, int accumulate, hipStream_t s) {
    const int Cin = p.Cin, Cout = p.Cout;
    const long M = (long)p.N * p.H * p.W, Mout = (long)p.N * p.OH * p.OW, NT = (long)p.K * p.K * Cout;
    unsigned short* x3 = reinterpret_cast<unsigned short*>(ws + p.w.off);
    unsigned short* d3 = reinterpret_cast<unsigned short*>(ws + p.a.off);
    hipLaunchKernelGGL(x3_split_rows_kernel, dim3(grid_for(M * Cin / 8, 256, 256 * 16)), dim3(256), 0, s, x, (long)Cin, x3, p.w.ld, p.w.cs, M, Cin / 8);
    X3Gemm g = {};
    g.A = x3; g.B = d3; g.C = dw;
    g.csA = p.w.cs; g.csB = p.a.cs; g.lda = (int)p.w.ld; g.ldb = (int)p.a.ld;
    g.M = Cin; g.N = (int)NT; g.K = (int)M; g.batch = 1; g.splits = 1; g.rows_per_split = (int)M; g.accum = accumulate;
    if (!p.general) {
        x3_split_unshuffle(dy, lddy, d3, p, s);
        PDF_LAUNCH_CHECK();
        return x3_launch_tn_deconv(g, s);
    }
    {
        KTimer kt("x3_split_rows_kernel", 0.0, 10.0 * Mout * Cout, s);
        hipLaunchKernelGGL(x3_split_rows_kernel, dim3(grid_for(Mout * Cout / 8, 256, 256 * 16)), dim3(256), 0, s, dy, (long)lddy, d3, p.a.ld, p.a.cs, Mout, Cout / 8);
    }
    if (int rc = x3_zero_rows(d3, p.a, s)) return rc;
    PDF_LAUNCH_CHECK();
    float* slab = ws + p.slab.off;
    g.rows_per_split = cdiv(cdiv(M, p.splits), 32) * 32; g.splits = cdiv(M, g.rows_per_split);
    if (g.splits > 1) { g.C = slab; g.accum = 0; }
    x3_all_taps(g, p);
    g.lw = __builtin_ctz(p.W); g.lhw = __builtin_ctz(p.H * p.W);
    if (int rc = x3_launch_tn_deconv(g, s)) return rc;
    if (g.splits > 1) {
        KTimer kt("x3_slab_reduce_kernel", 0.0, 4.0 * (g.splits + 1) * Cin * NT, s);
        hipLaunchKernelGGL(x3_slab_reduce_kernel, dim3(grid_for((long)Cin * NT / 4)), dim3(256), 0, s, slab, g.splits, (long)Cin * NT / 4, dw, accumulate);
        PDF_LAUNCH_CHECK();
    }
    return 0;
}

PDF_API int pdf_debug_workspace_plan(int kind, int pass, int N, int H, int W, int Cin, int Cout, int KH, int KW, int stride, int pad, long* out, int cap) {
    long v[8 + 2 * 4] = {0, 0, 0, 0, 0, -1, -1, 0};
    WsRegion r[4];
    int n = 0;
    if (kind == 0 && pass == 2) {
        const WinoWgradPlan p = wino_wgrad_plan(N, H, W, Cin, Cout, KH, KW, stride, pad);
        v[0] = p.ok; v[1] = p.total; v[2] = p.ok ? 4 : 0; v[3] = p.x3; v[4] = p.splits; v[6] = p.shared_v_x3;
        if (p.ok) { r[0] = p.V; r[1] = p.Yh; r[2] = p.slab; r[3] = p.colsum; n = 4; }
    } else if (kind == 0) {
        const WinoPlan p = wino_plan(N, H, W, pass ? Cout : Cin, pass ? Cin : Cout, KH, KW, stride, pad, pass);
        v[0] = p.ok; v[1] = p.total; v[2] = p.m; v[3] = p.x3; v[5] = p.v_offset; v[6] = p.shared_v_x3;
        if (p.ok) { r[0] = p.U; r[1] = p.V; r[2] = p.M; n = 3; }
    } else {
        const X3DeconvPlan p = pdf_debug_gemm_precision() ? X3DeconvPlan{} : x3_deconv_plan(N, H, W, Cin, Cout, KH, KW, stride, pad, pass);
        v[0] = p.ok; v[1] = p.total; v[2] = p.general; v[3] = p.ok; v[4] = p.splits;
        if (p.ok) { r[0] = {p.w.off, p.w.len}; r[1] = {p.a.off, p.a.len}; r[2] = p.slab; n = p.slab.len > 0 ? 3 : 2; }
    }
    v[7] = n;
    for (int i = 0; i < n; ++i) { v[8 + 2 * i] = r[i].off; v[9 + 2 * i] = r[i].len; }
    for (int i = 0; i < 8 + 2 * n && i < cap; ++i) out[i] = v[i];
    return 8 + 2 * n;
}
```

### pdfnet_amd/csrc/norm.hip

```cpp
#include "common.h"
#include <initializer_list>
#include <cstdlib>

#define BN_CT 64
#define BN_TX(V) (BN_CT / (V))
#define BN_TY(V) (256 / BN_TX(V))
template <int V> using vf = float __attribute__((ext_vector_type(V)));
template <int V> __device__ __forceinline__ vf<V> vld(const float* p) { return *reinterpret_cast<const vf<V>*>(p); }
template <int V> __device__ __forceinline__ void vst(float* p, vf<V> v) { *reinterpret_cast<vf<V>*>(p) = v; }
template <int V> __device__ __forceinline__ vf<V> vfma(vf<V> a, vf<V> b, vf<V> c) {
    vf<V> r;
#pragma unroll
    for (int i = 0; i < V; ++i) r[i] = fmaf(a[i], b[i], c[i]);
    return r;
}
__device__ __forceinline__ float add_rounded_product(float acc, float p, float q) {
#pragma clang fp contract(off)
    const float pq = p * q;
    return acc + pq;
}
__device__ __forceinline__ float sum_of_rounded_products(float a, float b, float c, float d) {
#pragma clang fp contract(off)
    const float ab = a * b, cd = c * d;
    return ab + cd;
// ... 720 lines not shown
        for (long r = r0 + ty; r < r1; r += BN_TY(V)) a += vld<V>(g + r * ldg + c0);
    }
    bn_block_reduce<V>(a, a, sa, sb, part, C, c0, false);
}

static int colsum_launch(const float* g, int ldg, int C, long R, float* out, float* out1, int accumulate, float* ws, hipStream_t s) {
    if (R <= 0 || C <= 0) return 0;
    const unsigned groups = out1 ? 2 : 1;
    const BnSplit sp = bn_split(C, R);
    const dim3 grid(cdiv(C, BN_CT), (unsigned)sp.chunks, groups);
    if (v4_ok(C, {ldg, (int)((R * ldg) % 4)}, {g}))
        hipLaunchKernelGGL(colsum_partial_kernel<4>, grid, dim3(256), 0, s, g, ldg, C, R, sp.rpc, ws);
    else
        hipLaunchKernelGGL(colsum_partial_kernel<1>, grid, dim3(256), 0, s, g, ldg, C, R, sp.rpc, ws);
    PDF_LAUNCH_CHECK();
    hipLaunchKernelGGL(colsum_finalize_kernel, dim3(cdiv(C, FIN_TX), groups), dim3(FIN_TX, FIN_TY), 0, s, ws, (int)sp.chunks, C, out, out1, accumulate);
    PDF_LAUNCH_CHECK();
    return 0;
}
int pdf_internal_colsum(const float* g, int ldg, int C, long R, float* out, int accumulate, float* ws, hipStream_t s) {
    return colsum_launch(g, ldg, C, R, out, nullptr, accumulate, ws, s);
}
long pdf_internal_colsum_ws(int C, long R) { return pdf_bn_workspace_floats(C, R); }
PDF_API int pdf_colsum(const float* g, int ldg, int C, long R, float* out, int accumulate, float* ws, void* stream) {
    hipStream_t s = (hipStream_t)stream;
    return colsum_launch(g, ldg, C, R, out, nullptr, accumulate, ws, s);
}
PDF_API int pdf_colsum_pair(const float* g, int ldg, int C, long R, float* out0, float* out1, int accumulate, float* ws, void* stream) {
    hipStream_t s = (hipStream_t)stream;
    return colsum_launch(g, ldg, C, R, out0, out1, accumulate, ws, s);
}

#define LN_MAXV 16
__global__ __launch_bounds__(256) void layernorm_fwd_kernel(const float* __restrict__ x, int ldx, const float* __restrict__ add, int ldadd,
                                                            float p, unsigned long long seed, const unsigned long long* __restrict__ step,
                                                            int F, long R, long R_split, const float* __restrict__ gamma0, const float* __restrict__ beta0,
                                                            const float* __restrict__ gamma1, const float* __restrict__ beta1, float eps, int act,
                                                            float* __restrict__ z, int ldz, float* __restrict__ y, int ldy,
                                                            float* __restrict__ mean, float* __restrict__ rstd) {
    const int lane = threadIdx.x & 63;
    const long rb = blockIdx.y ? R_split : 0, re = blockIdx.y ? R : min(R, R_split);
    const float* __restrict__ gamma = blockIdx.y ? gamma1 : gamma0;
    const float* __restrict__ beta = blockIdx.y ? beta1 : beta0;
    const long w0 = (blockIdx.x * (long)blockDim.x + threadIdx.x) >> 6;
    const long nw = ((long)gridDim.x * blockDim.x) >> 6;
    const float sc = 1.f / (1.f - p);
    if (add != nullptr && p > 0.f && step != nullptr) seed += step[0] * 0x9E3779B97F4A7C15ull;
    for (long r = rb + w0; r < re; r += nw) {
        float v[LN_MAXV];
        float sum = 0.f;
#pragma unroll
        for (int i = 0; i < LN_MAXV; ++i) {
            int c = lane + 64 * i;
            float t = 0.f;
            if (c < F) {
                t = x[r * ldx + c];
                if (add != nullptr) {
                    float a = add[r * ldadd + c];
                    if (p > 0.f) a = pdf_uniform(seed, (unsigned long long)(r * F + c)) >= p ? a * sc : 0.f;
                    t += a;
                    z[r * ldz + c] = t;
                }
            }
            v[i] = t;
            sum += t;
        }
        const float mu = wave_sum(sum) / (float)F;
        float sq = 0.f;
#pragma unroll
        for (int i = 0; i < LN_MAXV; ++i) {
            int c = lane + 64 * i;
            float d = c < F ? v[i] - mu : 0.f;
            sq += d * d;
        }
        const float rs = 1.0f / sqrtf(wave_sum(sq) / (float)F + eps);
#pragma unroll
        for (int i = 0; i < LN_MAXV; ++i) {
            int c = lane + 64 * i;
            if (c < F) {
                float o = (v[i] - mu) * rs * gamma[c] + beta[c];
                if (act == 1) o = fmaxf(o, 0.f);
                y[r * ldy + c] = o;
            }
        }
        if (lane == 0) { mean[r] = mu; rstd[r] = rs; }
    }
}

static int ln_fwd_launch(const float* x, int ldx, const float* add, int ldadd, float p, unsigned long long seed, const unsigned long long* step,
                         int F, long R, long R_split, const float* g0, const float* b0, const float* g1, const float* b1, float eps, int act,
                         float* z, int ldz, float* y, int ldy, float* mean, float* rstd, hipStream_t s) {
    if (F > 64 * LN_MAXV || (add != nullptr && z == nullptr)) return PDF_E_BADARG;
    if (R <= 0) return 0;
    const unsigned groups = R_split < R ? 2 : 1;
    const long rows = groups == 2 ? max(R_split, R - R_split) : R;
    hipLaunchKernelGGL(layernorm_fwd_kernel, dim3(grid_for(rows * 64), groups), dim3(256), 0, s, x, ldx, add, ldadd, p, seed, step, F, R, R_split,
                       g0, b0, g1, b1, eps, act, z, ldz, y, ldy, mean, rstd);
    PDF_LAUNCH_CHECK();
    return 0;
}
PDF_API int pdf_layernorm_fwd(const float* x, int ldx, int F, long R, const float* gamma, const float* beta, float eps,
                              float* y, int ldy, float* mean, float* rstd, void* stream) {
    hipStream_t s = (hipStream_t)stream;
    return ln_fwd_launch(x, ldx, nullptr, 0, 0.f, 0, nullptr, F, R, R, gamma, beta, gamma, beta, eps, 0, nullptr, 0, y, ldy, mean, rstd, s);
}
PDF_API int pdf_layernorm_fused_fwd(const float* x, int ldx, const float* add, int ldadd, float p, unsigned long long seed,
                                    const unsigned long long* step, int F, long R, long R_split,
                                    const float* gamma0, const float* beta0, const float* gamma1, const float* beta1, float eps, int act,
                                    float* z, int ldz, float* y, int ldy, float* mean, float* rstd, void* stream) {
    hipStream_t s = (hipStream_t)stream;
    return ln_fwd_launch(x, ldx, add, ldadd, p, seed, step, F, R, R_split, gamma0, beta0, gamma1, beta1, eps, act, z, ldz, y, ldy, mean, rstd, s);
}

template <bool DZ, bool PARAMS>
__global__ __launch_bounds__(256) void layernorm_bwd_kernel(const float* __restrict__ dy, int lddy, const float* __restrict__ y, int ldy, int act,
                                                            const float* __restrict__ zin, int ldz, int F, long R, long R_split,
                                                            const float* __restrict__ gamma0, const float* __restrict__ gamma1,
                                                            const float* __restrict__ mean, const float* __restrict__ rstd,
                                                            const float* __restrict__ dz_in, int lddzin, float* __restrict__ dz, int lddz,
                                                            float* __restrict__ dadd, int lddadd, float p, unsigned long long seed,
                                                            const unsigned long long* __restrict__ step,
                                                            float* __restrict__ dgamma0, float* __restrict__ dbeta0,
                                                            float* __restrict__ dgamma1, float* __restrict__ dbeta1) {
    __shared__ float sg[PARAMS ? 64 * LN_MAXV : 1], sb[PARAMS ? 64 * LN_MAXV : 1];
    if constexpr (PARAMS) {
        for (int i = threadIdx.x; i < F; i += 256) { sg[i] = 0.f; sb[i] = 0.f; }
        __syncthreads();
    }
    const int lane = threadIdx.x & 63;
    const long rb = blockIdx.y ? R_split : 0, re = blockIdx.y ? R : min(R, R_split);
    const float* __restrict__ gamma = blockIdx.y ? gamma1 : gamma0;
    float* __restrict__ dgamma = blockIdx.y ? dgamma1 : dgamma0;
    float* __restrict__ dbeta = blockIdx.y ? dbeta1 : dbeta0;
    const long w0 = (blockIdx.x * (long)blockDim.x + threadIdx.x) >> 6;
    const long nw = ((long)gridDim.x * blockDim.x) >> 6;
    const float sc = 1.f / (1.f - p);
    if (dadd != nullptr && p > 0.f && step != nullptr) seed += step[0] * 0x9E3779B97F4A7C15ull;
    float ag[LN_MAXV], ab[LN_MAXV];
#pragma unroll
    for (int i = 0; i < LN_MAXV; ++i) { ag[i] = 0.f; ab[i] = 0.f; }
    for (long r = rb + w0; r < re; r += nw) {
        const float mu = mean[r], rs = rstd[r];
        float g[LN_MAXV], xh[LN_MAXV];
        float s1 = 0.f, s2 = 0.f;
#pragma unroll
        for (int i = 0; i < LN_MAXV; ++i) {
            int c = lane + 64 * i;
            float d = 0.f, h = 0.f;
            if (c < F) {
                d = dy[r * lddy + c];
                if (act == 1 && !(y[r * ldy + c] > 0.f)) d = 0.f;
                h = (zin[r * ldz + c] - mu) * rs;
                if constexpr (PARAMS) { ag[i] += d * h; ab[i] += d; }
                d *= gamma[c];
            }
            g[i] = d; xh[i] = h;
            s1 += d; s2 += d * h;
        }
        if constexpr (!DZ) continue;
        s1 = wave_sum(s1) / (float)F;
        s2 = wave_sum(s2) / (float)F;
#pragma unroll
        for (int i = 0; i < LN_MAXV; ++i) {
            int c = lane + 64 * i;
            if (c < F) {
                float o = rs * (g[i] - s1 - xh[i] * s2);
                if (dz_in != nullptr) o += dz_in[r * lddzin + c];
                dz[r * lddz + c] = o;
                if (dadd != nullptr) {
                    if (p > 0.f) o = pdf_uniform(seed, (unsigned long long)(r * F + c)) >= p ? o * sc : 0.f;
                    dadd[r * lddadd + c] = o;
                }
            }
        }
    }
    if constexpr (PARAMS) {
#pragma unroll
        for (int i = 0; i < LN_MAXV; ++i) {
            int c = lane + 64 * i;
            if (c < F) { atomicAdd(&sg[c], ag[i]); atomicAdd(&sb[c], ab[i]); }
        }
        __syncthreads();
        for (int i = threadIdx.x; i < F; i += 256) {
            if (dgamma != nullptr) atomicAdd(&dgamma[i], sg[i]);
            if (dbeta != nullptr) atomicAdd(&dbeta[i], sb[i]);
        }
    }
}

static int ln_bwd_launch(const float* dy, int lddy, const float* y, int ldy, int act, const float* z, int ldz, int F, long R, long R_split,
                         const float* g0, const float* g1, const float* mean, const float* rstd, const float* dz_in, int lddzin,
                         float* dz, int lddz, float* dadd, int lddadd, float p, unsigned long long seed, const unsigned long long* step,
                         float* dg0, float* db0, float* dg1, float* db1, hipStream_t s) {
    if (F > 64 * LN_MAXV || (act == 1 && y == nullptr)) return PDF_E_BADARG;
    if (R <= 0) return 0;
    const unsigned groups = R_split < R ? 2 : 1;
    const long rows = groups == 2 ? max(R_split, R - R_split) : R;
    const bool params = dg0 != nullptr || db0 != nullptr || dg1 != nullptr || db1 != nullptr;
    if (dz == nullptr && !params) return 0;
    if (dz == nullptr && (dadd != nullptr || dz_in != nullptr)) return PDF_E_BADARG;
    const int grid = grid_for(rows * 64, 256, dz == nullptr ? 128 : params ? 512 : 4096);
#define LN_BWD(DZ_, PA_) hipLaunchKernelGGL((layernorm_bwd_kernel<DZ_, PA_>), dim3(grid, groups), dim3(256), 0, s, dy, lddy, y, ldy, act, z, ldz, F, R, \
                       R_split, g0, g1, mean, rstd, dz_in, lddzin, dz, lddz, dadd, lddadd, p, seed, step, dg0, db0, dg1, db1)
    if (dz == nullptr) LN_BWD(false, true); else if (params) LN_BWD(true, true); else LN_BWD(true, false);
#undef LN_BWD
    PDF_LAUNCH_CHECK();
    return 0;
}
PDF_API int pdf_layernorm_bwd(const float* dy, int lddy, const float* x, int ldx, int F, long R, const float* gamma,
                              const float* mean, const float* rstd, float* dx, int lddx, float* dgamma, float* dbeta, void* stream) {
    hipStream_t s = (hipStream_t)stream;
    return ln_bwd_launch(dy, lddy, nullptr, 0, 0, x, ldx, F, R, R, gamma, gamma, mean, rstd, nullptr, 0, dx, lddx, nullptr, 0, 0.f, 0, nullptr,
                         dgamma, dbeta, dgamma, dbeta, s);
}
PDF_API int pdf_layernorm_fused_bwd(const float* dy, int lddy, const float* y, int ldy, int act, const float* z, int ldz, int F, long R, long R_split,
                                    const float* gamma0, const float* gamma1, const float* mean, const float* rstd,
                                    const float* dz_in, int lddzin, float* dz, int lddz, float* dadd, int lddadd,
                                    float p, unsigned long long seed, const unsigned long long* step,
                                    float* dgamma0, float* dbeta0, float* dgamma1, float* dbeta1, void* stream) {
    hipStream_t s = (hipStream_t)stream;
    return ln_bwd_launch(dy, lddy, y, ldy, act, z, ldz, F, R, R_split, gamma0, gamma1, mean, rstd, dz_in, lddzin, dz, lddz, dadd, lddadd, p, seed, step,
                         dgamma0, dbeta0, dgamma1, dbeta1, s);
}

__global__ __launch_bounds__(256) void l2norm_fwd_kernel(const float* __restrict__ x, int ldx, int C, long R, const float* __restrict__ w,
                                                         float eps, float* __restrict__ y, int ldy, float* __restrict__ norm) {
    const int lane = threadIdx.x & 63;
    const long w0 = (blockIdx.x * (long)blockDim.x + threadIdx.x) >> 6;
    const long nw = ((long)gridDim.x * blockDim.x) >> 6;
    for (long r = w0; r < R; r += nw) {
        float sq = 0.f;
        for (int c = lane; c < C; c += 64) { float v = x[r * ldx + c]; sq += v * v; }
        const float n = sqrtf(wave_sum(sq)) + eps;
        for (int c = lane; c < C; c += 64) y[r * ldy + c] = w[c] * (x[r * ldx + c] / n);
        if (lane == 0) norm[r] = n;
    }
}

PDF_API int pdf_l2norm_fwd(const float* x, int ldx, int C, long R, const float* w, float eps, float* y, int ldy, float* norm, void* stream) {
    hipStream_t s = (hipStream_t)stream;
    if (R <= 0) return 0;
    hipLaunchKernelGGL(l2norm_fwd_kernel, dim3(grid_for(R * 64)), dim3(256), 0, s, x, ldx, C, R, w, eps, y, ldy, norm);
    PDF_LAUNCH_CHECK();
    return 0;
}

#define L2_MAXV 8
__global__ __launch_bounds__(256) void l2norm_bwd_kernel(const float* __restrict__ dy, int lddy, const float* __restrict__ x, int ldx, int C, long R,
                                                         const float* __restrict__ w, float eps, const float* __restrict__ norm,
                                                         float* __restrict__ dx, int lddx, float* __restrict__ dw) {
    extern __shared__ float sw[];
    for (int i = threadIdx.x; i < C; i += 256) sw[i] = 0.f;
    __syncthreads();
    const int lane = threadIdx.x & 63;
    const long w0 = (blockIdx.x * (long)blockDim.x + threadIdx.x) >> 6;
    const long nw = ((long)gridDim.x * blockDim.x) >> 6;
    float acc[L2_MAXV], wv[L2_MAXV];
#pragma unroll
    for (int i = 0; i < L2_MAXV; ++i) { acc[i] = 0.f; int c = lane + 64 * i; wv[i] = c < C ? w[c] : 0.f; }
    for (long r = w0; r < R; r += nw) {
        const float n = norm[r];
        float g[L2_MAXV], xv[L2_MAXV];
        float dot = 0.f;
#pragma unroll
        for (int i = 0; i < L2_MAXV; ++i) {
            int c = lane + 64 * i;
            g[i] = c < C ? dy[r * lddy + c] : 0.f;
            xv[i] = c < C ? x[r * ldx + c] : 0.f;
            dot += wv[i] * g[i] * xv[i];
        }
        dot = wave_sum(dot);
        const float nn = n - eps;
        const float k = nn > 0.f ? dot / (n * n * nn) : 0.f;
        const float in = 1.f / n;
#pragma unroll
        for (int i = 0; i < L2_MAXV; ++i) {
            int c = lane + 64 * i;
            if (c < C) dx[r * lddx + c] = wv[i] * g[i] * in - xv[i] * k;
            acc[i] += g[i] * xv[i] * in;
        }
    }
#pragma unroll
    for (int i = 0; i < L2_MAXV; ++i) { int c = lane + 64 * i; if (c < C) atomicAdd(&sw[c], acc[i]); }
    __syncthreads();
    for (int i = threadIdx.x; i < C; i += 256) atomicAdd(&dw[i], sw[i]);
}

PDF_API int pdf_l2norm_bwd(const float* dy, int lddy, const float* x, int ldx, int C, long R, const float* w, float eps,
                           const float* norm, float* dx, int lddx, float* dw, void* stream) {
    hipStream_t s = (hipStream_t)stream;
    if (R <= 0) return 0;
    if (C > 64 * L2_MAXV) return PDF_E_BADARG;
    int grid = grid_for(R * 64, 256, 1024);
    hipLaunchKernelGGL(l2norm_bwd_kernel, dim3(grid), dim3(256), C * sizeof(float), s, dy, lddy, x, ldx, C, R, w, eps, norm, dx, lddx, dw);
    PDF_LAUNCH_CHECK();
    return 0;
}

#define L2_MAXPARTS 4
struct L2Parts {
    const float* x[L2_MAXPARTS]; const float* w[L2_MAXPARTS]; float* norm[L2_MAXPARTS]; float* dx[L2_MAXPARTS]; float* dw[L2_MAXPARTS];
    unsigned short* dx16[L2_MAXPARTS];
    int C[L2_MAXPARTS], off[L2_MAXPARTS];
};
__global__ __launch_bounds__(256) void l2norm_cat_fwd_kernel(const L2Parts p, long R, float eps, float* __restrict__ y, int ldy,
                                                             unsigned short* __restrict__ y16) {
    const int part = blockIdx.y, C = p.C[part], lane = threadIdx.x & 63;
    const float* __restrict__ x = p.x[part]; const float* __restrict__ w = p.w[part];
    float* __restrict__ yo = y + p.off[part];
    const long w0 = (blockIdx.x * (long)blockDim.x + threadIdx.x) >> 6;
    const long nw = ((long)gridDim.x * blockDim.x) >> 6;
    for (long r = w0; r < R; r += nw) {
        float sq = 0.f;
        for (int c = lane; c < C; c += 64) { float v = x[r * C + c]; sq += v * v; }
        const float n = sqrtf(wave_sum(sq)) + eps;
        for (int c = lane; c < C; c += 64) {
            const float v = w[c] * (x[r * C + c] / n);
            yo[r * ldy + c] = v;
            if (y16 != nullptr) {
                const float vn = __shfl_down(v, 1, 64);
                if ((lane & 1) == 0) *reinterpret_cast<unsigned int*>(y16 + p.off[part] + r * ldy + c) = pdf_pk_bf16(v, vn);
            }
        }
        if (lane == 0) p.norm[part][r] = n;
    }
}
__global__ __launch_bounds__(256) void l2norm_cat_fwd_c256_kernel(const L2Parts p, long R, float eps, float* __restrict__ y, int ldy,
                                                                  unsigned short* __restrict__ y16) {
    typedef float v4f __attribute__((ext_vector_type(4)));
    typedef unsigned int v2u __attribute__((ext_vector_type(2)));
    const int part = blockIdx.y, lane = threadIdx.x & 63;
    const float* __restrict__ x = p.x[part];
    float* __restrict__ yo = y + p.off[part];
    const v4f wv = reinterpret_cast<const v4f*>(p.w[part])[lane];
    const long w0 = (blockIdx.x * (long)blockDim.x + threadIdx.x) >> 6;
    const long nw = ((long)gridDim.x * blockDim.x) >> 6;
    for (long r = w0; r < R; r += 2 * nw) {
        const long r1 = r + nw;
        const bool two = r1 < R;
        const v4f a = reinterpret_cast<const v4f*>(x + r * 256)[lane];
        v4f b = {0.f, 0.f, 0.f, 0.f};
        if (two) b = reinterpret_cast<const v4f*>(x + r1 * 256)[lane];
        const float na = sqrtf(wave_sum(a.x * a.x + a.y * a.y + a.z * a.z + a.w * a.w)) + eps;
        const float nb = sqrtf(wave_sum(b.x * b.x + b.y * b.y + b.z * b.z + b.w * b.w)) + eps;
        const v4f oa = {wv.x * (a.x / na), wv.y * (a.y / na), wv.z * (a.z / na), wv.w * (a.w / na)};
        *reinterpret_cast<v4f*>(yo + r * ldy + 4 * lane) = oa;
        if (y16 != nullptr) *reinterpret_cast<v2u*>(y16 + p.off[part] + r * ldy + 4 * lane) = v2u{pdf_pk_bf16(oa.x, oa.y), pdf_pk_bf16(oa.z, oa.w)};
        if (lane == 0) p.norm[part][r] = na;
        if (two) {
            const v4f ob = {wv.x * (b.x / nb), wv.y * (b.y / nb), wv.z * (b.z / nb), wv.w * (b.w / nb)};
            *reinterpret_cast<v4f*>(yo + r1 * ldy + 4 * lane) = ob;
            if (y16 != nullptr) *reinterpret_cast<v2u*>(y16 + p.off[part] + r1 * ldy + 4 * lane) = v2u{pdf_pk_bf16(ob.x, ob.y), pdf_pk_bf16(ob.z, ob.w)};
            if (lane == 0) p.norm[part][r1] = nb;
        }
    }
}
template <int MAXV>
__global__ __launch_bounds__(256) void l2norm_cat_bwd_kernel(const L2Parts p, long R, float eps, const float* __restrict__ dy, int lddy) {
    __shared__ float sw[64 * MAXV];
    const int q = blockIdx.y, C = p.C[q], lane = threadIdx.x & 63;
    const float* __restrict__ x = p.x[q]; const float* __restrict__ w = p.w[q]; const float* __restrict__ norm = p.norm[q];
    const float* __restrict__ g0 = dy + p.off[q];
    float* __restrict__ dx = p.dx[q];
    unsigned short* __restrict__ dx16 = p.dx16[q];
    for (int i = threadIdx.x; i < C; i += 256) sw[i] = 0.f;
    __syncthreads();
    const long w0 = (blockIdx.x * (long)blockDim.x + threadIdx.x) >> 6;
    const long nw = ((long)gridDim.x * blockDim.x) >> 6;
    float acc[MAXV], wv[MAXV];
#pragma unroll
    for (int i = 0; i < MAXV; ++i) { acc[i] = 0.f; const int c = lane + 64 * i; wv[i] = c < C ? w[c] : 0.f; }
    for (long r = w0; r < R; r += nw) {
        const float n = norm[r];
        float g[MAXV], xv[MAXV];
        float dot = 0.f;
#pragma unroll
        for (int i = 0; i < MAXV; ++i) {
            const int c = lane + 64 * i;
            g[i] = c < C ? g0[r * lddy + c] : 0.f;
            xv[i] = c < C ? x[r * C + c] : 0.f;
            dot += wv[i] * g[i] * xv[i];
        }
        dot = wave_sum(dot);
        const float nn = n - eps;
        const float k = nn > 0.f ? dot / (n * n * nn) : 0.f;
        const float in = 1.f / n;
#pragma unroll
        for (int i = 0; i < MAXV; ++i) {
            const int c = lane + 64 * i;
            const float o = wv[i] * g[i] * in - xv[i] * k;
            if (c < C) dx[r * C + c] = o;
            if (dx16 != nullptr) {
                const float on = __shfl_down(o, 1, 64);
                if (c < C && (lane & 1) == 0) *reinterpret_cast<unsigned int*>(dx16 + r * C + c) = pdf_pk_bf16(o, on);
            }
            acc[i] += g[i] * xv[i] * in;
        }
    }
#pragma unroll
    for (int i = 0; i < MAXV; ++i) { const int c = lane + 64 * i; if (c < C) atomicAdd(&sw[c], acc[i]); }
    __syncthreads();
    for (int i = threadIdx.x; i < C; i += 256) atomicAdd(&p.dw[q][i], sw[i]);
}
static int l2_parts(L2Parts& p, int nparts, const float* const* x, const float* const* w, float* const* norm, float* const* dx, float* const* dw,
                    const int* C) {
    if (nparts < 1 || nparts > L2_MAXPARTS) return PDF_E_BADARG;
    int off = 0;
    for (int i = 0; i < nparts; ++i) {
        if (C[i] <= 0 || C[i] > 64 * L2_MAXV) return PDF_E_BADARG;
        p.x[i] = x[i]; p.w[i] = w[i]; p.norm[i] = norm[i]; p.dx[i] = dx ? dx[i] : nullptr; p.dw[i] = dw ? dw[i] : nullptr;
        p.C[i] = C[i]; p.off[i] = off;
        off += C[i];
    }
    return 0;
}
static int pdf_l2norm_cat_fwd_impl(int nparts, const float* const* x, const int* C, const float* const* w, float eps, long R,
                               float* y, int ldy, float* const* norm, void* stream, PdfCallOpts& co) {
    hipStream_t s = (hipStream_t)stream;
    void* y16 = co.out_bf16;
    if (R <= 0) return 0;
    L2Parts p = {};
    if (int rc = l2_parts(p, nparts, x, w, norm, nullptr, nullptr, C)) return rc;
    for (int i = 0; y16 != nullptr && i < nparts; ++i) if (C[i] % 64) return PDF_E_BADARG;
    bool c256 = ldy % 4 == 0 && (reinterpret_cast<uintptr_t>(y) & 15) == 0 && (y16 == nullptr || (reinterpret_cast<uintptr_t>(y16) & 7) == 0);
    for (int i = 0; i < nparts; ++i)
        c256 = c256 && C[i] == 256 && p.off[i] % 4 == 0 && (reinterpret_cast<uintptr_t>(x[i]) & 15) == 0 && (reinterpret_cast<uintptr_t>(w[i]) & 15) == 0;
    if (c256) hipLaunchKernelGGL(l2norm_cat_fwd_c256_kernel, dim3(grid_for(R * 32, 256, 4096), nparts), dim3(256), 0, s, p, R, eps, y, ldy,
                                 reinterpret_cast<unsigned short*>(y16));
    else hipLaunchKernelGGL(l2norm_cat_fwd_kernel, dim3(grid_for(R * 64, 256, 2048), nparts), dim3(256), 0, s, p, R, eps, y, ldy,
                            reinterpret_cast<unsigned short*>(y16));
    PDF_LAUNCH_CHECK();
    return 0;
}
PDF_API int pdf_l2norm_cat_fwd_x(int nparts, const float* const* x, const int* C, const float* const* w, float eps, long R,
                               float* y, int ldy, float* const* norm, void* stream, PdfCallOpts* opts) {
    return pdf_call_x(opts, pdf_l2norm_cat_fwd_impl, nparts, x, C, w, eps, R, y, ldy, norm, stream);
}
PDF_API int pdf_l2norm_cat_fwd(int nparts, const float* const* x, const int* C, const float* const* w, float eps, long R,
                               float* y, int ldy, float* const* norm, void* stream) {
    return pdf_call_plain(pdf_l2norm_cat_fwd_impl, nparts, x, C, w, eps, R, y, ldy, norm, stream);
}

PDF_API int pdf_l2norm_cat_bwd(int nparts, const float* dy, int lddy, const float* const* x, const int* C, const float* const* w, float eps, long R,
                               float* const* norm, float* const* dx, float* const* dw, void* const* dx16, void* stream) {
    hipStream_t s = (hipStream_t)stream;
    if (R <= 0) return 0;
    L2Parts p = {};
    if (int rc = l2_parts(p, nparts, x, w, norm, dx, dw, C)) return rc;
    for (int i = 0; dx16 != nullptr && i < nparts; ++i) {
        if (dx16[i] != nullptr && C[i] % 64) return PDF_E_BADARG;
        p.dx16[i] = reinterpret_cast<unsigned short*>(dx16[i]);
    }
    int cmax = 0;
    for (int i = 0; i < nparts; ++i) cmax = max(cmax, C[i]);
    const dim3 grid(grid_for(R * 64, 256, 1024), nparts);
    if (cmax <= 256) hipLaunchKernelGGL(l2norm_cat_bwd_kernel<4>, grid, dim3(256), 0, s, p, R, eps, dy, lddy);
    else hipLaunchKernelGGL(l2norm_cat_bwd_kernel<L2_MAXV>, grid, dim3(256), 0, s, p, R, eps, dy, lddy);
    PDF_LAUNCH_CHECK();
    return 0;
}
```

### pdfnet_amd/functional.py

```python
import collections
import ctypes
import torch
from torch.autograd import Function

from . import hip
from .hip import ptr, ptr_at, stream

ACT_NONE, ACT_RELU, ACT_LRELU = 0, 1, 2
import os as _os

_byref = ctypes.byref
_CallOpts = hip.CallOpts
USE_SIDE_STREAMS = _os.environ.get("PDFNET_SIDE_STREAMS", "1") != "0"
_side = {}


def _record(obj, stream_):
    if torch.is_tensor(obj):
        obj.record_stream(stream_)
        s16 = getattr(obj, '_pdf_bf16', None)
        if s16 is not None:
            s16.record_stream(stream_)
    elif isinstance(obj, (list, tuple)):
        for o in obj:
            _record(o, stream_)
    elif isinstance(obj, dict):
        for o in obj.values():
            _record(o, stream_)


class fork:
    _busy = {}

    def __init__(self, fn):
        self.stream = None
        if not USE_SIDE_STREAMS:
            self.out = fn()
            return
        cur = torch.cuda.current_stream()
        dev = torch.cuda.current_device()
        pool = _side.setdefault(('fork', dev), [])
        busy = fork._busy.setdefault(dev, set())
        free = [i for i in range(len(pool)) if i not in busy]
        if not free:
            pool.append(torch.cuda.Stream())
            free = [len(pool) - 1]
        self.idx, self.dev = free[0], dev
        busy.add(self.idx)
        self.stream = pool[self.idx]
        self.stream.wait_stream(cur)
        with torch.cuda.stream(self.stream):
            self.out = fn()

    def join(self):
        if self.stream is not None:
            cur = torch.cuda.current_stream()
            cur.wait_stream(self.stream)
            _record(self.out, cur)
            fork._busy[self.dev].discard(self.idx)
            self.stream = None
        return self.out


def parallel(*fns):
    if not USE_SIDE_STREAMS or len(fns) == 1:
        return [f() for f in fns]
    cur = torch.cuda.current_stream()
    key = (cur.device_index if hasattr(cur, 'device_index') else torch.cuda.current_device())
    pool = _side.setdefault(key, [])
    while len(pool) < len(fns) - 1:
        pool.append(torch.cuda.Stream())
    streams = [cur] + pool[:len(fns) - 1]
    for s_ in streams[1:]:
        s_.wait_stream(cur)
    out = []
    for f, s_ in zip(fns, streams):
        with torch.cuda.stream(s_):
            out.append(f())
    for r, s_ in zip(out[1:], streams[1:]):
        cur.wait_stream(s_)
        _record(r, cur)
    return out

CL = torch.channels_last


def set_gemm_precision(dtype):
    if dtype not in ('fp32', 'bf16'):
        raise ValueError("pdfnet_amd: gemm precision must be 'fp32' or 'bf16'")
    global _GEMM_BF16
    hip.lib().pdf_set_gemm_precision(1 if dtype == 'bf16' else 0)
    _GEMM_BF16 = dtype == 'bf16'


def gemm_precision():
    return 'bf16' if hip.lib().pdf_debug_gemm_precision() else 'fp32'


BF16_SHADOWS = _os.environ.get("PDFNET_BF16_SHADOWS", "1") != "0"


_GEMM_BF16 = False


def shadows_on():
    return BF16_SHADOWS and _GEMM_BF16


def attach_shadow(t, s16):
    t._pdf_bf16, t._pdf_bf16_ver = s16, t._version
    return t


def shadow_of(t):
    if t is None or not (BF16_SHADOWS and _GEMM_BF16):
        return None
    s16 = getattr(t, '_pdf_bf16', None)
    if s16 is None or t._version != getattr(t, '_pdf_bf16_ver', -1) or s16.shape != t.shape or s16.stride() != t.stride():
        return None
    return s16


TRANSPOSED_SHADOWS = _os.environ.get("PDFNET_BF16_TRANSPOSED", "1") != "0"


def shadow_t_of(w):
    if not TRANSPOSED_SHADOWS or shadow_of(w) is None:
        return None
    return getattr(w, '_pdf_bf16_t', None)


def new_shadow(t):
    return torch.empty_like(t, dtype=torch.bfloat16) if shadows_on() else None


_bs = _os.environ.get("PDFNET_BF16_STORAGE", "auto")
BF16_STORAGE = 'auto' if _bs == "auto" else _bs != "0"
BF16_STORAGE_MIN_BATCH = int(_os.environ.get("PDFNET_BF16_STORAGE_MIN_BATCH", "32"))


def storage_on(batch=None):
    if not (BF16_SHADOWS and _GEMM_BF16):
        return False
    if BF16_STORAGE == 'auto':
        return batch is not None and batch >= BF16_STORAGE_MIN_BATCH
    return bool(BF16_STORAGE)


def _lazy_bn(t):
    v = getattr(t, '_pdf_lazy', None)
    if v is None or v[3] != t._version:
        return None
    return v[:3]


DEBUG_PHANTOMS = _os.environ.get("PDFNET_DEBUG_PHANTOMS", "0") != "0"


def _stored16(t):
    v = getattr(t, '_pdf_y16', None)
    if v is None:
        return None
    if v[1] != t._version:
        raise RuntimeError("pdfnet_amd: a bf16-storage phantom tensor was modified in place; its fp32 storage holds no value (PDFNET_BF16_STORAGE)")
    return v[0]



def _O(**kw):
    o = None
    for k, v in kw.items():
        if v is not None:
            if o is None:
                o = _CallOpts()
            setattr(o, k, v)
    if o is None:
        return None, None
    return o, _byref(o)


WINOGRAD = _os.environ.get("PDFNET_WINOGRAD", "1") != "0"
WINOGRAD_INFERENCE = _os.environ.get("PDFNET_WINOGRAD_INFERENCE", "0") != "0"
_ws_sizes = {}


def _ws_query(fn, *args):
    n = _ws_sizes.get((fn, args))
    if n is None:
        n = _ws_sizes[(fn, args)] = getattr(_L(), fn)(*args)
    return n


def _ws_alloc(n, dev):
    return (torch.empty(n, dtype=torch.float32, device=dev), n) if n > 0 else (None, None)


def _wino_ws(N, H, W, Cin, Cout, KH, KW, stride, pad, backward, dev):
    if not WINOGRAD or _GEMM_BF16 or KH != 3 or KW != 3 or stride != 1 or pad != 1 or Cin < 64 or Cout < 64:
        return None, None
    return _ws_alloc(_ws_query("pdf_conv2d_winograd_workspace_floats", N, H, W, Cin, Cout, KH, KW, stride, pad, backward), dev)


X3_DECONV = _os.environ.get("PDFNET_X3_DECONV", "1") != "0"


def set_x3(mode):
    _L().pdf_set_x3_mode(-1 if mode is None else int(mode))
    _ws_sizes.clear()


def _x3_deconv_ws(N, H, W, Cin, Cout, KH, KW, stride, pad, backward, dev):
    if not X3_DECONV or _GEMM_BF16 or KH != KW or stride < 2:
        return None, None
    return _ws_alloc(_ws_query("pdf_deconv2d_x3_workspace_floats", N, H, W, Cin, Cout, KH, KW, stride, pad, backward), dev)


WINOGRAD_KEEP_V = _os.environ.get("PDFNET_WINOGRAD_KEEP_V", "1") != "0"


def _wino_v_offset(N, H, W, Cin, Cout, KH, KW, stride, pad):
    return _ws_query("pdf_conv2d_winograd_v_offset", N, H, W, Cin, Cout, KH, KW, stride, pad)


WINOGRAD_SHARE = _os.environ.get("PDFNET_WINOGRAD_SHARE", "1") != "0"


def share_winograd_input(x):
    if WINOGRAD_SHARE and x is not None and getattr(x, '_pdf_wino_share', None) is None:
        x._pdf_wino_share = {}
    return x


BN_EPILOGUE_STATS = _os.environ.get("PDFNET_BN_EPILOGUE_STATS", "1") != "0"
_be = _os.environ.get("PDFNET_BN_EPILOGUE_STATS_BF16", "auto")
BN_EPILOGUE_STATS_BF16 = 'auto' if _be == "auto" else _be != "0"


def bf16_modes(batch):
    if not _GEMM_BF16:
        return {'gemm': 'fp32'}
    stats = (batch >= BF16_STORAGE_MIN_BATCH) if BN_EPILOGUE_STATS_BF16 == 'auto' else bool(BN_EPILOGUE_STATS_BF16)
    return {'gemm': 'bf16', 'shadows': BF16_SHADOWS, 'conv_to_bn_storage': 'bf16' if storage_on(batch) else 'fp32',
            'bn_statistics': ('fp32 accumulators in the GEMM epilogue' if (stats and BN_EPILOGUE_STATS) else "the BatchNorm's own pass over the stored tensor"),
            'auto_threshold_batch': BF16_STORAGE_MIN_BATCH}


def _stats_request(stats, rows, cols, dev, batch=None):
    if not (stats and BN_EPILOGUE_STATS):
        return None
    if _GEMM_BF16:
        on = (batch is not None and batch >= BF16_STORAGE_MIN_BATCH) if BN_EPILOGUE_STATS_BF16 == 'auto' else bool(BN_EPILOGUE_STATS_BF16)
        if not on:
            return None
    cap = ((rows + 31) // 32) * cols * 2
    return torch.empty(cap, dtype=torch.float32, device=dev)


def _stats_attach(y, part, o):
    if part is None:
        return
    if o.stats_tiles > 0:
        y._pdf_bn_tiles = (part, o.stats_tiles, o.stats_rows, y._version)


def tile_stats_of(x):
    t = getattr(x, '_pdf_bn_tiles', None)
    if t is None or t[3] != x._version:
        return None
    return t


def carry_stats(src, dst):
    t = getattr(src, '_pdf_bn_tiles', None)
    if t is not None and dst.data_ptr() == src.data_ptr():
        dst._pdf_bn_tiles = t
    return dst


class _forced_fp32:

    def __init__(self, on):
        self.on = on and hip.lib().pdf_debug_gemm_precision() != 0

    def __enter__(self):
        if self.on:
            hip.lib().pdf_set_gemm_precision(0)

    def __exit__(self, *exc):
        if self.on:
            hip.lib().pdf_set_gemm_precision(1)
        return False


def _L():
    return hip.lib()


def cl(x):
    return x.contiguous(memory_format=CL)


def _rows(x):
    if x.dim() == 4:
        return x.shape[0] * x.shape[2] * x.shape[3], x.shape[1]
    return x.numel() // x.shape[-1], x.shape[-1]


def _canon(x):
    return cl(x) if x.dim() == 4 else x.contiguous()


def _zeros_cl(shape, dev):
    return torch.empty(shape, dtype=torch.float32, device=dev, memory_format=CL).zero_()


def _ws(nfloats, dev):
    return torch.empty(max(int(nfloats), 1), dtype=torch.float32, device=dev)


_wgrad_ws_cache = {}
_bn_ws_cache = {}


def _wgrad_ws(M, NI, NJ, dev):
    n = _wgrad_ws_cache.get((M, NI, NJ))
    if n is None:
        n = _wgrad_ws_cache[(M, NI, NJ)] = _L().pdf_wgrad_workspace_floats(M, NI, NJ)
    return _ws(n, dev), n


def _bn_ws_floats(C, R):
    n = _bn_ws_cache.get((C, R))
    if n is None:
        n = _bn_ws_cache[(C, R)] = _L().pdf_bn_workspace_floats(C, R)
    return n


ASYNC_WGRAD = _os.environ.get("PDFNET_ASYNC_WGRAD", "1") != "0"
_wg_streams = {}
_wg_used = set()


WGRAD_STREAM_PRIORITY = int(_os.environ.get("PDFNET_WGRAD_STREAM_PRIORITY", "0"))


class wgrad_stream:

    def __init__(self, enabled, *tensors, params=(), also_wait=None):
        self.enabled = enabled and ASYNC_WGRAD and USE_SIDE_STREAMS
        self.tensors = tensors
        self.params = params
        self.also_wait = also_wait

    def __enter__(self):
        if not self.enabled:
            return self
        dev = hip._raw_device()
        cur_raw = hip._raw_stream(dev)
        key = (dev, cur_raw)
        ent = _wg_streams.get(key)
        if ent is None:
            if WGRAD_STREAM_PRIORITY > 0:
                import ctypes as _ct
                raw = _ct.c_void_p()
                _L().pdf_stream_create(_ct.byref(raw), WGRAD_STREAM_PRIORITY, None, None)
                s = torch.cuda.ExternalStream(raw.value)
            else:
                s = torch.cuda.Stream(priority=WGRAD_STREAM_PRIORITY)
            ent = _wg_streams[key] = (s, s.cuda_stream, s.stream_id, s.device_index, s.device_type)
        side, side_raw = ent[0], ent[1]
        wait = _L().pdf_stream_wait
        wait(side_raw, cur_raw)
        if self.also_wait is not None and self.also_wait != cur_raw:
            wait(side_raw, self.also_wait)
        for p in self.params:
            if p is not None:
                last = getattr(p, '_pdf_wg_last', None)
                if last is not None and last is not ent:
                    wait(side_raw, last[1])
                p._pdf_wg_last = ent
        for t in self.tensors:
            if t is not None:
                t.record_stream(side)
                s16 = getattr(t, '_pdf_bf16', None)
                if s16 is not None:
                    s16.record_stream(side)
        _wg_used.add(key)
        self._prev = torch._C._cuda_getCurrentStream(dev)
        torch._C._cuda_setStream(stream_id=ent[2], device_index=ent[3], device_type=ent[4])
        return self

    def __exit__(self, *exc):
        if self.enabled:
            p = self._prev
            torch._C._cuda_setStream(stream_id=p[0], device_index=p[1], device_type=p[2])
        return False


WGRAD_GROUP = int(_os.environ.get("PDFNET_WGRAD_GROUP", "1"))
_wg_pending = {}


def _wg_defer(fn, tensors, params):
    key = hip._raw_stream(hip._raw_device())
    lst = _wg_pending.setdefault(key, [])
    lst.append((fn, tensors, params))
    if len(lst) >= WGRAD_GROUP:
        _wg_flush_key(key)


def _wg_flush_key(key):
    items = _wg_pending.pop(key, None)
    if not items:
        return
    with wgrad_stream(True, *[t for it in items for t in it[1]], params=[p for it in items for p in it[2]], also_wait=key):
        for it in items:
            it[0]()


def flush_wgrad():
    for key in list(_wg_pending):
        _wg_flush_key(key)


def join_wgrad(keep=False):
    flush_wgrad()
    cur = hip.stream()
    for key in list(_wg_used):
        _L().pdf_stream_wait(cur, _wg_streams[key][1])
    if not keep:
        _wg_used.clear()


def _main_grad(param, like):
    if param is None or not getattr(param, '_pdf_main_grad', False):
        return None
    g = getattr(param, '_pdf_grad_alias', None)
    if g is None:
        g = param.grad
    if g is None or g.shape != like.shape or g.stride() != like.stride():
        return None
    return g


def _colsum_into(g, C, R, ldg, out):
    ws = _ws(_bn_ws_floats(C, R), g.device)
    _L().pdf_colsum(ptr(g), ldg, C, R, ptr(out), 1, ptr(ws), stream())


def _colsum(g, C, R, ldg):
    out = torch.empty(C, dtype=torch.float32, device=g.device)
    ws = _ws(_bn_ws_floats(C, R), g.device)
    _L().pdf_colsum(ptr(g), ldg, C, R, ptr(out), 0, ptr(ws), stream())
    return out


ASYNC_WGRAD_MIN_FLOP = float(_os.environ.get("PDFNET_ASYNC_WGRAD_MIN_GFLOP", "0")) * 1e9


def _param_grads(ctx, x, g, w, w_par, b_par, has_b, launch_w, C, R, flops, fused_bias=False, shadows=()):
    need_w = ctx.needs_input_grad[1]
    need_b = has_b and ctx.needs_input_grad[2]
    mg_w = _main_grad(w_par, w) if need_w else None
    mg_b = _main_grad(b_par, b_par) if need_b else None
    dw = db = None
    ride = fused_bias and need_w and need_b and (mg_w is None) == (mg_b is None)
    if mg_w is not None or mg_b is not None:
        def run():
            if mg_w is not None:
                launch_w(mg_w, mg_b if ride else None, 1)
            if mg_b is not None and not ride:
                _colsum_into(g, C, R, C, mg_b)
        if WGRAD_GROUP > 1 and ASYNC_WGRAD and USE_SIDE_STREAMS and flops >= ASYNC_WGRAD_MIN_FLOP:
            _wg_defer(run, (x, g) + tuple(shadows), (w_par, b_par))
        else:
            with wgrad_stream(flops >= ASYNC_WGRAD_MIN_FLOP, x, g, *shadows, params=(w_par, b_par)):
                run()
    if need_w and mg_w is None:
        dw = torch.empty_like(w)
        if ride:
            db = torch.empty(C, dtype=torch.float32, device=x.device)
        launch_w(dw, db, 0)
    if need_b and mg_b is None and not ride:
        db = _colsum(g, C, R, C)
    return dw, db


def _act_bwd(dy, y, act):
    R, C = _rows(y)
    g = torch.empty_like(y)
    _L().pdf_act_bwd(ptr(dy), C, ptr(y), C, ptr(g), C, C, R, act, stream())
    return g


class _Conv2d(Function):

    @staticmethod
    def forward(ctx, x, w, b, stride, pad, act, skip=False, stats=False):
        hip.require_gpu(x, w)
        w_in = w
        x_in = x
        x, w = cl(x), cl(w)
        N, Cin, H, W = x.shape
        Cout, _, KH, KW = w.shape
        OH = (H + 2 * pad - KH) // stride + 1
        OW = (W + 2 * pad - KW) // stride + 1
        y = torch.empty((N, Cout, OH, OW), dtype=torch.float32, device=x.device, memory_format=CL)
        x16, w16 = shadow_of(x), shadow_of(w)
        part = _stats_request(stats, N * OH * OW, Cout, x.device, batch=N)
        y16 = None
        if (stats and storage_on(N) and b is None and act == ACT_NONE and Cin % 16 == 0 and Cout % 16 == 0
                and (N * OH * OW) % 128 == 0):
            y16 = torch.empty_like(y, dtype=torch.bfloat16)
        ws, nws = _wino_ws(N, H, W, Cin, Cout, KH, KW, stride, pad, 0, x.device) if (WINOGRAD_INFERENCE or any(ctx.needs_input_grad[:3])) else (None, None)
        share = getattr(x_in, '_pdf_wino_share', None) if (ws is not None and WINOGRAD_KEEP_V) else None
        v_off = _wino_v_offset(N, H, W, Cin, Cout, KH, KW, stride, pad) if (ws is not None and WINOGRAD_KEEP_V) else -1
        v_src = None
        if share is not None and v_off >= 0:
            ent = share.get((N, H, W, Cin))
            if ent is not None and ent[2] == x_in._version:
                v_src = ent
                if ent[4] != hip._raw_stream(hip._raw_device()):
                    cs = torch.cuda.current_stream()
                    cs.wait_event(ent[3])
                    ent[0].record_stream(cs)
        o, oa = _O(op0_bf16=ptr(x16), op1_bf16=ptr(w16), out_bf16=ptr(y16), stats_out=ptr(part), stats_cap=part.numel() if part is not None else None,
                   ws=ptr(ws), ws_floats=nws, wino_v=(v_src[0].data_ptr() + 4 * v_src[1]) if v_src is not None else None)
        _L().pdf_conv2d_fwd_x(ptr(x), ptr(w), ptr(b), ptr(y), N, H, W, Cin, Cin, Cout, KH, KW, stride, pad, OH, OW, Cout, act, stream(), oa)
        if share is not None and v_off >= 0 and v_src is None:
            ev = torch.cuda.Event()
            ev.record()
            share[(N, H, W, Cin)] = (ws, v_off, x_in._version, ev, hip._raw_stream(hip._raw_device()))
        _stats_attach(y, part, o)
        if y16 is not None:
            if DEBUG_PHANTOMS:
                y.fill_(float('nan'))
            y._pdf_y16 = (y16, y._version)
        ctx.wino_v = None
        if v_off >= 0 and ctx.needs_input_grad[1]:
            ctx.wino_v = (v_src[0], v_src[1]) if v_src is not None else (ws, v_off)
        ctx.save_for_backward(x, w, y if act else None)
        ctx.s16 = (x16, w16)
        ctx.w16t = shadow_t_of(w) if w16 is not None else None
        ctx.cfg = (stride, pad, act, b is not None)
        ctx.params = (w_in, b)
        if skip:
            return y, x_in.view_as(x_in)
        return y

    @staticmethod
    def backward(ctx, dy, dskip=None):
        x, w, y = ctx.saved_tensors
        stride, pad, act, has_b = ctx.cfg
        N, Cin, H, W = x.shape
        Cout, _, KH, KW = w.shape
        OH, OW = dy.shape[2], dy.shape[3]
        g16 = _stored16(dy)
        if g16 is not None:
            g, gp = dy, None
        else:
            g = cl(dy)
            if act:
                g = _act_bwd(g, y, act)
            g16, gp = shadow_of(g), ptr(g)
        x16, w16 = ctx.s16
        dx = dw = db = None
        L = _L()
        if ctx.needs_input_grad[0]:
            ws, nws = _wino_ws(N, H, W, Cin, Cout, KH, KW, stride, pad, 1, x.device) if (OH == H and OW == W and gp is not None) else (None, None)
            _, oa = _O(op0_bf16=ptr(g16), op1_bf16=ptr(w16), op1_bf16_t=ptr(ctx.w16t) if g16 is not None else None, ws=ptr(ws), ws_floats=nws)
            if dskip is not None and stride == 1 and dskip.shape == x.shape and dskip.is_contiguous(memory_format=CL):
                dx = dskip
                L.pdf_conv2d_bwd_data_add_x(gp, ptr(w), ptr(dx), N, H, W, Cin, Cin, Cout, KH, KW, stride, pad, OH, OW, Cout, stream(), oa)
            else:
                dx = torch.zeros_like(x) if stride > KH else torch.empty_like(x)
                L.pdf_conv2d_bwd_data_x(gp, ptr(w), ptr(dx), N, H, W, Cin, Cin, Cout, KH, KW, stride, pad, OH, OW, Cout, stream(), oa)
                if dskip is not None:
                    dx = dx + dskip
        w_par, b_par = ctx.params
        R = N * OH * OW

        keep = ctx.wino_v
        ctx.wino_v = None

        def launch_w(out, out_b, acc):
            ws, n = _wgrad_ws(R, Cout, KH * KW * Cin, x.device)
            wws, nww = _wino_ws(N, H, W, Cin, Cout, KH, KW, stride, pad, 2, x.device) if (OH == H and OW == W and gp is not None) else (None, None)
            v = (keep[0].data_ptr() + 4 * keep[1]) if (keep is not None and wws is not None) else None
            L.pdf_conv2d_bwd_weight_x(ptr(x), gp, ptr(out), ptr(out_b), ptr(ws), n, N, H, W, Cin, Cin, Cout, KH, KW,
                                      stride, pad, OH, OW, Cout, acc, stream(), _O(op0_bf16=ptr(x16), op1_bf16=ptr(g16), ws=ptr(wws), ws_floats=nww, wino_v=v)[1])
        dw, db = _param_grads(ctx, x, g, w, w_par, b_par, has_b, launch_w, Cout, R, 2.0 * R * Cout * KH * KW * Cin, fused_bias=True,
                              shadows=(x16, g16, keep[0] if keep is not None else None))
        return dx, dw, db, None, None, None, None, None


def conv2d(x, w, b=None, stride=1, pad=0, act=ACT_NONE, stats=False):
    return _Conv2d.apply(x, w, b, stride, pad, act, False, stats)


def conv2d_with_skip(x, w, b=None, stride=1, pad=0, act=ACT_NONE, stats=False):
    return _Conv2d.apply(x, w, b, stride, pad, act, True, stats)


class _Deconv2d(Function):

    @staticmethod
    def forward(ctx, x, w, b, stride, pad):
        hip.require_gpu(x, w)
        w_in = w
        x, w = cl(x), cl(w)
        N, Cin, H, W = x.shape
        _, Cout, KH, KW = w.shape
        OH = (H - 1) * stride - 2 * pad + KH
        OW = (W - 1) * stride - 2 * pad + KW
        L = _L()
        y = torch.empty((N, Cout, OH, OW), dtype=torch.float32, device=x.device, memory_format=CL)
        x16, w16 = shadow_of(x), shadow_of(w)
        ws, nws = _x3_deconv_ws(N, H, W, Cin, Cout, KH, KW, stride, pad, 0, x.device)
        L.pdf_deconv2d_fwd_x(ptr(x), ptr(w), ptr(b), ptr(y), N, H, W, Cin, Cin, Cout, KH, KW, stride, pad, OH, OW, Cout, stream(),
                             _O(op0_bf16=ptr(x16), op1_bf16=ptr(w16), ws=ptr(ws), ws_floats=nws)[1])
        ctx.save_for_backward(x, w)
        ctx.s16 = (x16, w16)
        ctx.cfg = (stride, pad, b is not None)
        ctx.params = (w_in, b)
        return y

    @staticmethod
    def backward(ctx, dy):
        x, w = ctx.saved_tensors
        stride, pad, has_b = ctx.cfg
        N, Cin, H, W = x.shape
        _, Cout, KH, KW = w.shape
        OH, OW = dy.shape[2], dy.shape[3]
        g = cl(dy)
        x16, w16 = ctx.s16
        g16 = shadow_of(g)
        L = _L()
        dx = dw = db = None
        if ctx.needs_input_grad[0]:
            dx = torch.empty_like(x)
            ws, nws = _x3_deconv_ws(N, H, W, Cin, Cout, KH, KW, stride, pad, 1, x.device)
            L.pdf_deconv2d_bwd_data_x(ptr(g), ptr(w), ptr(dx), N, H, W, Cin, Cin, Cout, KH, KW, stride, pad, OH, OW, Cout, stream(),
                                      _O(op0_bf16=ptr(g16), op1_bf16=ptr(w16), ws=ptr(ws), ws_floats=nws)[1])
        w_par, b_par = ctx.params

        def launch_w(out, out_b, acc):
            ws, n = _wgrad_ws(N * H * W, Cin, KH * KW * Cout, x.device)
            xws, nx = _x3_deconv_ws(N, H, W, Cin, Cout, KH, KW, stride, pad, 2, x.device)
            L.pdf_deconv2d_bwd_weight_x(ptr(x), ptr(g), ptr(out), ptr(ws), n, N, H, W, Cin, Cin, Cout, KH, KW,
                                        stride, pad, OH, OW, Cout, acc, stream(), _O(op0_bf16=ptr(x16), op1_bf16=ptr(g16), ws=ptr(xws), ws_floats=nx)[1])
        dw, db = _param_grads(ctx, x, g, w, w_par, b_par, has_b, launch_w, Cout, N * OH * OW, 2.0 * N * H * W * Cin * KH * KW * Cout, shadows=(x16, g16))
        return dx, dw, db, None, None


def deconv2d(x, w, b=None, stride=1, pad=0):
    return _Deconv2d.apply(x, w, b, stride, pad)


class _Linear(Function):

    @staticmethod
    def forward(ctx, x, w, b, act, fp32=False, stats=False):
        hip.require_gpu(x, w)
        w_in = w
        lz = _lazy_bn(x)
        if lz is not None:
            x, aff = lz[0], (lz[1], lz[2])
        else:
            aff = None
        x, w = x.contiguous(), w.contiguous()
        K = x.shape[-1]
        M = x.numel() // K
        Nn = w.shape[0]
        y = torch.empty(x.shape[:-1] + (Nn,), dtype=torch.float32, device=x.device)
        x16, w16 = (None, None) if (fp32 or aff is not None) else (shadow_of(x), shadow_of(w))
        with _forced_fp32(fp32):
            part = _stats_request(stats, M, Nn, x.device)
            o, oa = _O(op0_bf16=ptr(x16), op1_bf16=ptr(w16), stats_out=ptr(part), stats_cap=part.numel() if part is not None else None,
                       in_scale=ptr(aff[0]) if aff is not None else None, in_shift=ptr(aff[1]) if aff is not None else None)
            _L().pdf_linear_fwd_x(ptr(x), ptr(w), ptr(b), ptr(y), M, Nn, K, K, K, Nn, act, stream(), oa)
            _stats_attach(y, part, o)
        ctx.save_for_backward(x, w, y if act else None, *(aff if aff is not None else ()))
        ctx.s16 = (x16, w16)
        ctx.w16t = shadow_t_of(w) if w16 is not None else None
        ctx.fp32 = fp32
        ctx.cfg = (act, b is not None)
        ctx.params = (w_in, b)
        return y

    @staticmethod
    def backward(ctx, dy):
        x, w, y = ctx.saved_tensors[:3]
        aff = ctx.saved_tensors[3:5] if len(ctx.saved_tensors) > 3 else None
        act, has_b = ctx.cfg
        K = x.shape[-1]
        M = x.numel() // K
        Nn = w.shape[0]
        g = dy.contiguous()
        if act:
            g = _act_bwd(g, y, act)
        x16, w16 = ctx.s16
        g16 = None if ctx.fp32 else shadow_of(g)
        L = _L()
        dx = dw = db = None
        if ctx.needs_input_grad[0]:
            dx = torch.empty_like(x)
            with _forced_fp32(ctx.fp32):
                L.pdf_linear_bwd_data_x(ptr(g), ptr(w), ptr(dx), M, Nn, K, Nn, K, K, stream(),
                                        _O(op0_bf16=ptr(g16), op1_bf16=ptr(w16), op1_bf16_t=ptr(ctx.w16t) if g16 is not None else None)[1])
        w_par, b_par = ctx.params

        def launch_w(out, out_b, acc):
            ws, n = _wgrad_ws(M, Nn, K, x.device)
            with _forced_fp32(ctx.fp32):
                _, oa = _O(op0_bf16=ptr(x16), op1_bf16=ptr(g16), in_scale=ptr(aff[0]) if aff is not None else None,
                           in_shift=ptr(aff[1]) if aff is not None else None)
                L.pdf_linear_bwd_weight_x(ptr(x), ptr(g), ptr(out), ptr(out_b), ptr(ws), n, M, Nn, K, K, Nn, acc, stream(), oa)
        dw, db = _param_grads(ctx, x, g, w, w_par, b_par, has_b, launch_w, Nn, M, 2.0 * M * Nn * K, fused_bias=True,
                              shadows=(x16, g16) + (tuple(aff) if aff is not None else ()))
        return dx, dw, db, None, None, None


def linear(x, w, b=None, act=ACT_NONE, fp32=False, stats=False):
    return _Linear.apply(x, w, b, act, fp32, stats)


def as_matrix(weight):
    w2 = weight.permute(0, 2, 3, 1).reshape(weight.shape[0], -1)
    if w2.data_ptr() != weight.data_ptr():
        return w2
    w16 = shadow_of(weight)
    if w16 is not None:
        s2 = w16.permute(0, 2, 3, 1).reshape(weight.shape[0], -1)
        if s2.data_ptr() == w16.data_ptr():
            attach_shadow(w2, s2)
    if getattr(weight, '_pdf_main_grad', False) and weight.grad is not None:
        g2 = weight.grad.permute(0, 2, 3, 1).reshape(weight.shape[0], -1)
        if g2.data_ptr() == weight.grad.data_ptr():
            w2._pdf_main_grad = True
            w2._pdf_grad_alias = g2
    return w2


class _LinearPair(Function):

    @staticmethod
    def forward(ctx, x, w0, b0, w1, b1, act):
        hip.require_gpu(x, w0, w1)
        if x.shape[0] != 2 or w0.shape != w1.shape or (b0 is None) != (b1 is None):
            raise ValueError("pdfnet_amd: linear_pair wants x [2, ..., K] and two equal-shaped layers")
        w0_in, w1_in = w0, w1
        x, w0, w1 = x.contiguous(), w0.contiguous(), w1.contiguous()
        K = x.shape[-1]
        M = x.numel() // K // 2
        Nn = w0.shape[0]
        y = torch.empty(x.shape[:-1] + (Nn,), dtype=torch.float32, device=x.device)
        _L().pdf_linear_fwd_pair_x(ptr(x), ptr(w0), ptr(w1), ptr(b0), ptr(b1), ptr(y), M, Nn, K, K, K, Nn, act, stream(), None)
        ctx.save_for_backward(x, w0, w1, y if act else None)
        ctx.cfg = (act, b0 is not None)
        ctx.params = (w0_in, b0, w1_in, b1)
        return y

    @staticmethod
    def backward(ctx, dy):
        x, w0, w1, y = ctx.saved_tensors
        act, has_b = ctx.cfg
        K = x.shape[-1]
        M = x.numel() // K // 2
        Nn = w0.shape[0]
        g = dy.contiguous()
        if act:
            g = _act_bwd(g, y, act)
        L = _L()
        dx = None
        if ctx.needs_input_grad[0]:
            dx = torch.empty_like(x)
            L.pdf_linear_bwd_data_pair_x(ptr(g), ptr(w0), ptr(w1), ptr(dx), M, Nn, K, Nn, K, K, stream(), None)
        w0_par, b0_par, w1_par, b1_par = ctx.params
        need_w = ctx.needs_input_grad[1] or ctx.needs_input_grad[3]
        need_b = has_b and (ctx.needs_input_grad[2] or ctx.needs_input_grad[4])
        mg_w0, mg_w1 = (_main_grad(w0_par, w0), _main_grad(w1_par, w1)) if need_w else (None, None)
        mg_b0, mg_b1 = (_main_grad(b0_par, b0_par), _main_grad(b1_par, b1_par)) if need_b else (None, None)
        direct_w = mg_w0 is not None and mg_w1 is not None
        direct_b = mg_b0 is not None and mg_b1 is not None

        def launch_w(o0, o1, p0, p1, acc):
            n = 2 * L.pdf_wgrad_workspace_floats(M, Nn, K)
            L.pdf_linear_bwd_weight_pair_x(ptr(x), ptr(g), ptr(o0), ptr(o1), ptr(p0), ptr(p1), ptr(_ws(n, x.device)), n, M, Nn, K, K, Nn, acc, stream(), None)

        def launch_b(o0, o1, acc):
            ws = _ws(2 * _bn_ws_floats(Nn, M), x.device)
            L.pdf_colsum_pair(ptr(g), Nn, Nn, M, ptr(o0), ptr(o1), acc, ptr(ws), stream())
        dw0 = dw1 = db0 = db1 = None
        ride = need_w and need_b and direct_w == direct_b
        if (need_w and direct_w) or (need_b and direct_b):
            with wgrad_stream(True, x, g, params=(w0_par, b0_par, w1_par, b1_par)):
                if need_w and direct_w:
                    launch_w(mg_w0, mg_w1, mg_b0 if ride else None, mg_b1 if ride else None, 1)
                if need_b and direct_b and not ride:
                    launch_b(mg_b0, mg_b1, 1)
        if need_w and not direct_w:
            dw0, dw1 = torch.empty_like(w0), torch.empty_like(w1)
            if ride:
                db0, db1 = torch.empty(Nn, device=x.device), torch.empty(Nn, device=x.device)
            launch_w(dw0, dw1, db0, db1, 0)
        if need_b and not direct_b and not ride:
            db0, db1 = torch.empty(Nn, device=x.device), torch.empty(Nn, device=x.device)
            launch_b(db0, db1, 0)
        return dx, dw0, db0, dw1, db1, None


def linear_pair(x, w0, b0, w1, b1, act=ACT_NONE):
    return _LinearPair.apply(x, w0, b0, w1, b1, act)


class _BatchNorm(Function):

    @staticmethod
    def forward(ctx, x, gamma, beta, rmean, rvar, res, training, momentum, eps, relu, lazy=False):
        hip.require_gpu(x)
        x16 = _stored16(x)
        if x16 is not None and not training:
            raise RuntimeError("pdfnet_amd: a bf16-storage phantom reached a BatchNorm in eval mode -- the producing convolution must "
                               "be called with stats=<that BatchNorm>.training (only a training-mode BatchNorm reads the bf16 tensor)")
        if _lazy_bn(x) is not None:
            raise RuntimeError("pdfnet_amd: the unwritten output of a lazy BatchNorm reached another BatchNorm; only a linear layer may consume it")
        if x16 is None:
            x = _canon(x)
        res = _canon(res) if res is not None else None
        R, C = _rows(x)
        y = torch.empty_like(x)
        dev = x.device
        scale = torch.empty(C, device=dev)
        shift = torch.empty(C, device=dev)
        L = _L()
        if training:
            mean = torch.empty(C, device=dev)
            rstd = torch.empty(C, device=dev)
            tiles = tile_stats_of(x)
            if tiles is not None:
                ws = None
            else:
                ws = _ws(_bn_ws_floats(C, R), dev)
            lazy = bool(lazy) and relu and res is None and x16 is None and not _GEMM_BF16 and x.dim() == 2 and C % 16 == 0 and R % 16 == 0
            y16 = new_shadow(y) if (C % 4 == 0 and not lazy) else None
            _, oa = _O(out_bf16=ptr(y16), bn_x_bf16=ptr(x16), tile_stats=ptr(tiles[0]) if tiles is not None else None,
                       tile_n=tiles[1] if tiles is not None else None, tile_rows=tiles[2] if tiles is not None else None)
            L.pdf_bn_train_fwd_x(None if x16 is not None else ptr(x), C, C, R, ptr(gamma), ptr(beta), ptr(rmean), ptr(rvar), momentum, eps,
                                 ptr(res), C, int(relu), None if lazy else ptr(y), C, ptr(mean), ptr(rstd), ptr(scale), ptr(shift), ptr(ws), stream(), oa)
            if y16 is not None:
                attach_shadow(y, y16)
            if lazy:
                y._pdf_lazy = (x, scale, shift, y._version)
            recompute = relu and res is None
            ctx.save_for_backward(x16 if x16 is not None else x, gamma, mean, rstd, (scale if recompute else (y if relu else None)), (shift if recompute else None))
            ctx.x_is_16 = x16 is not None
        else:
            L.pdf_bn_eval_fwd(ptr(x), C, C, R, ptr(gamma), ptr(beta), ptr(rmean), ptr(rvar), eps,
                              ptr(res), C, int(relu), ptr(y), C, ptr(scale), ptr(shift), stream())
            recompute = relu and res is None
            ctx.save_for_backward(x, scale, rmean, rvar, y if (relu and not recompute) else None, shift if recompute else None)
            ctx.x_is_16 = False
        ctx.cfg = (training, relu, res is not None, eps)
        ctx.params = (gamma, beta)
        return y

    @staticmethod
    def backward(ctx, dy):
        training, relu, has_res, eps = ctx.cfg
        if not training:
            return _BatchNorm._backward_frozen(ctx, dy)
        x, gamma, mean, rstd, y, shift = ctx.saved_tensors
        scale = None
        mode = int(relu)
        if relu and not has_res:
            scale, y, mode = y, None, 2
        R, C = _rows(x)
        g = _canon(dy)
        x_is_16 = ctx.x_is_16
        dx = torch.empty_like(x, dtype=torch.float32)
        dres = torch.empty_like(dx) if has_res else None
        g_par, b_par = ctx.params
        mg_g, mg_b = _main_grad(g_par, g_par), _main_grad(b_par, b_par)
        direct = mg_g is not None and mg_b is not None
        dgamma = mg_g if direct else torch.empty(C, device=x.device)
        dbeta = mg_b if direct else torch.empty(C, device=x.device)
        L = _L()
        ws = _ws(_bn_ws_floats(C, R) + 3 * C, x.device)
        dx16 = new_shadow(dx) if C % 4 == 0 else None
        _, oa = _O(out_bf16=ptr(dx16), bn_x_bf16=ptr(x) if x_is_16 else None)
        L.pdf_bn_train_bwd_x(ptr(g), C, ptr(y), C, mode, None if x_is_16 else ptr(x), C, ptr(mean), ptr(rstd), ptr(gamma), ptr(scale), ptr(shift), C, R,
                             None if x_is_16 else ptr(dx), C, ptr(dres), C, ptr(dgamma), ptr(dbeta), int(direct), ptr(ws), stream(), oa)
        if x_is_16:
            if DEBUG_PHANTOMS:
                dx.fill_(float('nan'))
            dx._pdf_y16 = (dx16, dx._version)
        elif dx16 is not None:
            attach_shadow(dx, dx16)
        if direct:
            dgamma = dbeta = None
        return dx, dgamma, dbeta, None, None, dres, None, None, None, None, None

    @staticmethod
    def _backward_frozen(ctx, dy):
        x, scale, rmean, rvar, y, shift = ctx.saved_tensors
        _, relu, has_res, eps = ctx.cfg
        mode = (2 if not has_res else 1) if relu else 0
        need_x, need_g, need_b = ctx.needs_input_grad[:3]
        need_res = has_res and ctx.needs_input_grad[5]
        sums = need_g or need_b
        if not (need_x or sums or need_res):
            return (None,) * 11
        R, C = _rows(x)
        g = _canon(dy)
        dx = torch.empty_like(x) if need_x else None
        dres = torch.empty_like(x) if need_res else None
        dgamma = dbeta = ws = None
        direct = False
        if sums:
            g_par, b_par = ctx.params
            mg_g, mg_b = _main_grad(g_par, g_par), _main_grad(b_par, b_par)
            direct = need_g and need_b and mg_g is not None and mg_b is not None
            dgamma = mg_g if direct else torch.empty(C, device=x.device)
            dbeta = mg_b if direct else torch.empty(C, device=x.device)
            ws = _ws(_bn_ws_floats(C, R), x.device)
        _L().pdf_bn_eval_bwd(ptr(g), C, ptr(y), C, mode, ptr(x), C, ptr(rmean), ptr(rvar), eps, ptr(scale), ptr(shift), C, R,
                             ptr(dx), C, ptr(dres), C, ptr(dgamma), ptr(dbeta), int(direct), ptr(ws), stream())
        if direct:
            dgamma = dbeta = None
        return dx, (dgamma if need_g else None), (dbeta if need_b else None), None, None, dres, None, None, None, None, None


def batch_norm(x, gamma, beta, rmean, rvar, training, momentum=0.1, eps=1e-5, relu=False, res=None, lazy=False):
    return _BatchNorm.apply(x, gamma, beta, rmean, rvar, res, training, momentum, eps, relu, lazy)


class _Pad2d(Function):

    @staticmethod
    def forward(ctx, x, R2, C2):
        hip.require_gpu(x)
        x = x.contiguous()
        R, C = x.shape
        y = torch.empty((R2, C2), dtype=torch.float32, device=x.device)
        _L().pdf_pad2d(ptr(x), C, R, C, ptr(y), C2, R2, C2, stream())
        ctx.shape = (R, C)
        return y

    @staticmethod
    def backward(ctx, dy):
        R, C = ctx.shape
        dy = dy.contiguous()
        dx = torch.empty((R, C), dtype=torch.float32, device=dy.device)
        _L().pdf_pad2d(ptr(dy), dy.shape[1], dy.shape[0], dy.shape[1], ptr(dx), C, R, C, stream())
        return dx, None, None


def pad2d(x, rows, cols):
    if x.shape[0] == rows and x.shape[1] == cols:
        return x
    return _Pad2d.apply(x, rows, cols)


class _Act(Function):
    @staticmethod
    def forward(ctx, x, act):
        hip.require_gpu(x)
        x = _canon(x)
        R, C = _rows(x)
        y = torch.empty_like(x)
        _L().pdf_act_fwd(ptr(x), C, ptr(y), C, C, R, act, stream())
        ctx.save_for_backward(y)
        ctx.act = act
        return y

    @staticmethod
    def backward(ctx, dy):
        (y,) = ctx.saved_tensors
        return _act_bwd(_canon(dy), y, ctx.act), None


def relu(x):
    return _Act.apply(x, ACT_RELU)


class _MaxPool3s2(Function):

    @staticmethod
    def forward(ctx, x, skip=False):
        x_in = x
        x = cl(x)
        N, C, H, W = x.shape
        OH, OW = (H - 1) // 2 + 1, (W - 1) // 2 + 1
        y = torch.empty((N, C, OH, OW), device=x.device, memory_format=CL)
        arg = torch.empty(y.numel(), dtype=torch.uint8, device=x.device)
        _L().pdf_maxpool3s2_fwd(ptr(x), N, H, W, C, ptr(y), ptr(arg), stream())
        ctx.save_for_backward(arg)
        ctx.shape = (N, C, H, W)
        ctx.set_materialize_grads(False)
        if skip:
            return y, x_in.view_as(x_in)
        return y

    @staticmethod
    def backward(ctx, dy, dskip=None):
        (arg,) = ctx.saved_tensors
        N, C, H, W = ctx.shape
        if dy is None:
            return dskip, None
        if dskip is not None and dskip.shape == (N, C, H, W) and dskip.is_contiguous(memory_format=CL) and dskip.dtype == torch.float32:
            _L().pdf_maxpool3s2_bwd_add(ptr(cl(dy)), ptr(arg), N, H, W, C, ptr(dskip), stream())
            return dskip, None
        dx = torch.empty((N, C, H, W), device=dy.device, memory_format=CL) if C % 4 == 0 else _zeros_cl((N, C, H, W), dy.device)
        _L().pdf_maxpool3s2_bwd(ptr(cl(dy)), ptr(arg), N, H, W, C, ptr(dx), stream())
        if dskip is not None:
            dx = dx + dskip
        return dx, None


def maxpool3s2(x, skip=False):
    return _MaxPool3s2.apply(x, skip)


class _Up2(Function):
    @staticmethod
    def forward(ctx, x):
        x = cl(x)
        N, C, H, W = x.shape
        y = torch.empty((N, C, 2 * H, 2 * W), device=x.device, memory_format=CL)
        _L().pdf_upsample2x_fwd(ptr(x), N, H, W, C, ptr(y), stream())
        ctx.shape = (N, C, H, W)
        return y

    @staticmethod
    def backward(ctx, dy):
        N, C, H, W = ctx.shape
        dx = torch.empty((N, C, H, W), dtype=torch.float32, device=dy.device, memory_format=CL)
        _L().pdf_upsample2x_bwd(ptr(cl(dy)), N, H, W, C, ptr(dx), stream())
        return dx


def upsample2x(x):
    return _Up2.apply(x)


class _L2Norm(Function):
    @staticmethod
    def forward(ctx, x, w, eps):
        x = cl(x)
        R, C = _rows(x)
        y = torch.empty_like(x)
        norm = torch.empty(R, device=x.device)
        _L().pdf_l2norm_fwd(ptr(x), C, C, R, ptr(w), eps, ptr(y), C, ptr(norm), stream())
        ctx.save_for_backward(x, w, norm)
        ctx.eps = eps
        return y

    @staticmethod
    def backward(ctx, dy):
        x, w, norm = ctx.saved_tensors
        R, C = _rows(x)
        dx = torch.empty_like(x)
        dw = torch.zeros_like(w)
        _L().pdf_l2norm_bwd(ptr(cl(dy)), C, ptr(x), C, C, R, ptr(w), ctx.eps, ptr(norm), ptr(dx), C, ptr(dw), stream())
        return dx, dw, None


def l2norm(x, w, eps=1e-10):
    return _L2Norm.apply(x, w, eps)


def _ptr_array(tensors):
    import ctypes
    return (ctypes.c_void_p * len(tensors))(*[t.data_ptr() for t in tensors])


def _int_array(values):
    import ctypes
    return (ctypes.c_int * len(values))(*values)


class _L2NormCat(Function):

    @staticmethod
    def forward(ctx, eps, *args):
        n = len(args) // 2
        xs, ws = [cl(x) for x in args[:n]], list(args[n:])
        hip.require_gpu(*xs)
        B, _, H, W = xs[0].shape
        if any(x.shape[0] != B or x.shape[2:] != xs[0].shape[2:] for x in xs):
            raise ValueError("pdfnet_amd: l2norm_cat wants maps of one batch and resolution")
        Cs = [x.shape[1] for x in xs]
        Ct, R = sum(Cs), B * H * W
        out = torch.empty((B, Ct, H, W), dtype=torch.float32, device=xs[0].device, memory_format=CL)
        norms = [torch.empty(R, device=out.device) for _ in xs]
        out16 = new_shadow(out) if all(C % 64 == 0 for C in Cs) else None
        if out16 is not None:
            attach_shadow(out, out16)
        _L().pdf_l2norm_cat_fwd_x(n, _ptr_array(xs), _int_array(Cs), _ptr_array(ws), eps, R, ptr(out), Ct, _ptr_array(norms), stream(), _O(out_bf16=ptr(out16))[1])
        ctx.save_for_backward(*xs, *ws, *norms)
        ctx.cfg = (eps, n, Cs)
        return out

    @staticmethod
    def backward(ctx, dy):
        eps, n, Cs = ctx.cfg
        t = ctx.saved_tensors
        xs, ws, norms = t[:n], t[n:2 * n], t[2 * n:]
        g = cl(dy)
        Ct = sum(Cs)
        R = xs[0].numel() // Cs[0]
        dxs, dws = [torch.empty_like(x) for x in xs], [torch.zeros_like(w) for w in ws]
        d16 = [new_shadow(d) for d in dxs] if all(C % 64 == 0 for C in Cs) and _os.environ.get('PDFNET_L2_SHADOW', '1') != '0' else None
        if d16 is not None and d16[0] is None:
            d16 = None
        _L().pdf_l2norm_cat_bwd(n, ptr(g), Ct, _ptr_array(xs), _int_array(Cs), _ptr_array(ws), eps, R, _ptr_array(norms),
                                _ptr_array(dxs), _ptr_array(dws), _ptr_array(d16) if d16 is not None else None, stream())
        if d16 is not None:
            for d, s16 in zip(dxs, d16):
                attach_shadow(d, s16)
        return (None,) + tuple(dxs) + tuple(dws)


def l2norm_cat(xs, ws, eps=1e-10):
    return _L2NormCat.apply(eps, *xs, *ws)


class _LayerNorm(Function):
    @staticmethod
    def forward(ctx, x, gamma, beta, eps):
        hip.require_gpu(x)
        x = x.contiguous()
        R, Fd = x.numel() // x.shape[-1], x.shape[-1]
        y = torch.empty_like(x)
        mean = torch.empty(R, device=x.device)
        rstd = torch.empty(R, device=x.device)
        _L().pdf_layernorm_fwd(ptr(x), Fd, Fd, R, ptr(gamma), ptr(beta), eps, ptr(y), Fd, ptr(mean), ptr(rstd), stream())
        ctx.save_for_backward(x, gamma, mean, rstd)
        ctx.params = (gamma, beta)
        return y

    @staticmethod
    def backward(ctx, dy):
        x, gamma, mean, rstd = ctx.saved_tensors
        R, Fd = x.numel() // x.shape[-1], x.shape[-1]
        dx = torch.empty_like(x)
        g_par, b_par = ctx.params
        mg_g, mg_b = _main_grad(g_par, g_par), _main_grad(b_par, b_par)
        direct = mg_g is not None and mg_b is not None
        dg = mg_g if direct else torch.zeros_like(gamma)
        db = mg_b if direct else torch.zeros_like(gamma)
        _L().pdf_layernorm_bwd(ptr(dy.contiguous()), Fd, ptr(x), Fd, Fd, R, ptr(gamma), ptr(mean), ptr(rstd), ptr(dx), Fd, ptr(dg), ptr(db), stream())
        if direct:
            dg = db = None
        return dx, dg, db, None


def layer_norm(x, gamma, beta, eps=1e-6):
    return _LayerNorm.apply(x, gamma, beta, eps)


class _LayerNormFused(Function):

    @staticmethod
    def forward(ctx, x, add, g0, b0, g1, b1, eps, act, p, seed):
        hip.require_gpu(x)
        x = x.contiguous()
        R, Fd = x.numel() // x.shape[-1], x.shape[-1]
        pair = g1 is not None
        if pair and (x.shape[0] != 2):
            raise ValueError("pdfnet_amd: paired layer_norm wants x stacked [2, ...]")
        split = R // 2 if pair else R
        y = torch.empty_like(x)
        mean = torch.empty(R, device=x.device)
        rstd = torch.empty(R, device=x.device)
        z = None
        if add is not None:
            add = add.contiguous()
            z = torch.empty_like(x)
        _L().pdf_layernorm_fused_fwd(ptr(x), Fd, ptr(add), Fd, p, seed, ptr(step_counter(x.device)), Fd, R, split,
                                     ptr(g0), ptr(b0), ptr(g1 if pair else g0), ptr(b1 if pair else b0), eps, act,
                                     ptr(z), Fd, ptr(y), Fd, ptr(mean), ptr(rstd), stream())
        ctx.save_for_backward(x if z is None else z, g0, g1, mean, rstd, y if act else None)
        ctx.cfg = (act, p, seed, add is not None, pair)
        ctx.params = (g0, b0, g1, b1)
        ctx.set_materialize_grads(False)
        if z is None:
            return y
        return z, y

    @staticmethod
    def backward(ctx, *grads):
        zin, g0, g1, mean, rstd, y = ctx.saved_tensors
        act, p, seed, has_add, pair = ctx.cfg
        dz_in, dy = grads if has_add else (None, grads[0])
        R, Fd = zin.numel() // zin.shape[-1], zin.shape[-1]
        split = R // 2 if pair else R
        if dy is None:
            if dz_in is None:
                return (None,) * 10
            dadd = _Dropout.apply(dz_in, p, seed, True) if p > 0 else dz_in
            return dz_in, dadd, None, None, None, None, None, None, None, None
        pars = ctx.params
        mgs = [_main_grad(t, t) if t is not None else None for t in pars]
        need = [t is not None for t in pars]
        direct = all(m is not None for m, n in zip(mgs, need) if n)
        outs = [m if direct else (torch.zeros_like(t) if t is not None else None) for m, t in zip(mgs, pars)]
        dz = torch.empty_like(zin)
        dadd = torch.empty_like(zin) if has_add else None
        d0, e0 = outs[0], outs[1]
        d1, e1 = (outs[2], outs[3]) if pair else (d0, e0)
        dy = dy.contiguous()
        dz_in = dz_in.contiguous() if dz_in is not None else None
        gb = ptr(g1 if pair else g0)
        if direct and ASYNC_WGRAD and USE_SIDE_STREAMS:
            _L().pdf_layernorm_fused_bwd(ptr(dy), Fd, ptr(y), Fd, act, ptr(zin), Fd, Fd, R, split, ptr(g0), gb, ptr(mean), ptr(rstd),
                                         ptr(dz_in), Fd, ptr(dz), Fd, ptr(dadd), Fd, p, seed, ptr(step_counter(zin.device)),
                                         None, None, None, None, stream())
            with wgrad_stream(True, dy, y, zin, mean, rstd, params=pars):
                _L().pdf_layernorm_fused_bwd(ptr(dy), Fd, ptr(y), Fd, act, ptr(zin), Fd, Fd, R, split, ptr(g0), gb, ptr(mean), ptr(rstd),
                                             None, Fd, None, Fd, None, Fd, 0.0, 0, None, ptr(d0), ptr(e0), ptr(d1), ptr(e1), stream())
        else:
            _L().pdf_layernorm_fused_bwd(ptr(dy), Fd, ptr(y), Fd, act, ptr(zin), Fd, Fd, R, split, ptr(g0), gb,
                                         ptr(mean), ptr(rstd), ptr(dz_in), Fd, ptr(dz), Fd,
                                         ptr(dadd), Fd, p, seed, ptr(step_counter(zin.device)), ptr(d0), ptr(e0), ptr(d1), ptr(e1), stream())
        if direct:
            outs = [None] * 4
        return dz, dadd, outs[0], outs[1], outs[2], outs[3], None, None, None, None


def layer_norm_fused(x, gamma, beta, eps=1e-6, act=ACT_NONE, add=None, p=0.0, training=False, gamma1=None, beta1=None):
    p = float(p) if (training and add is not None) else 0.0
    return _LayerNormFused.apply(x, add, gamma, beta, gamma1, beta1, eps, act, p, next_seed() if p > 0 else 0)


class _Dropout(Function):
    @staticmethod
    def forward(ctx, x, p, seed, _unused=None):
        x = x.contiguous()
        y = torch.empty_like(x)
        _L().pdf_dropout(ptr(x), ptr(y), x.numel(), p, seed, ptr(step_counter(x.device)), stream())
        ctx.cfg = (p, seed)
        return y

    @staticmethod
    def backward(ctx, dy):
        p, seed = ctx.cfg
        dy = dy.contiguous()
        dx = torch.empty_like(dy)
        _L().pdf_dropout(ptr(dy), ptr(dx), dy.numel(), p, seed, ptr(step_counter(dy.device)), stream())
        return dx, None, None, None


class _DropoutAdd(Function):

    @staticmethod
    def forward(ctx, x, res, p, seed):
        x, res = x.contiguous(), res.contiguous()
        y = torch.empty_like(x)
        _L().pdf_dropout_add(ptr(x), ptr(res), ptr(y), x.numel(), p, seed, ptr(step_counter(x.device)), stream())
        ctx.cfg = (p, seed)
        return y

    @staticmethod
    def backward(ctx, dy):
        p, seed = ctx.cfg
        dx = dy
        if p > 0 and ctx.needs_input_grad[0]:
            dy = dy.contiguous()
            dx = torch.empty_like(dy)
            _L().pdf_dropout(ptr(dy), ptr(dx), dy.numel(), p, seed, ptr(step_counter(dy.device)), stream())
        return dx, dy, None, None


def dropout_add(x, res, p, training):
    p = float(p) if training else 0.0
    return _DropoutAdd.apply(x, res, p, next_seed() if p > 0 else 0)


_seed_state = [0x5DEECE66D]


def next_seed():
    _seed_state[0] = (_seed_state[0] * 6364136223846793005 + 1442695040888963407) & ((1 << 63) - 1)
    return _seed_state[0]


_step_counters = {}


def step_counter(dev):
    key = str(dev)
    if key not in _step_counters:
        _step_counters[key] = torch.zeros(1, dtype=torch.int64, device=dev)
    return _step_counters[key]


def manual_seed(s):
    _seed_state[0] = (int(s) * 2654435761 + 12345) & ((1 << 63) - 1)


def dropout(x, p, training):
    if not training or p <= 0.0:
        return x
    return _Dropout.apply(x, float(p), next_seed())


class _SFTModulate(Function):

    @staticmethod
    def forward(ctx, fea, scale, shift):
        fea, scale, shift = fea.contiguous(), scale.contiguous(), shift.contiguous()
        R, C = _rows(fea)
        out = torch.empty_like(fea)
        _L().pdf_sft_fwd(ptr(fea), C, ptr(scale), C, ptr(shift), C, ptr(out), C, C, R, stream())
        ctx.save_for_backward(fea, scale)
        return out

    @staticmethod
    def backward(ctx, g):
        fea, scale = ctx.saved_tensors
        g = g.contiguous()
        R, C = _rows(fea)
        dfea = torch.empty_like(fea)
        dscale = torch.empty_like(fea)
        _L().pdf_sft_bwd(ptr(g), C, ptr(fea), C, ptr(scale), C, ptr(dfea), C, ptr(dscale), C, C, R, stream())
        return dfea, dscale, g


def sft_modulate(fea, scale, shift):
    return _SFTModulate.apply(fea, scale, shift)


class _SFT3(Function):

    @staticmethod
    def forward(ctx, fea, cond, *params):
        hip.require_gpu(fea, cond)
        fea, cond = fea.contiguous(), cond.contiguous()
        if fea.shape[-1] != 3 or cond.shape[-1] != 3 or len(params) != 8:
            raise ValueError("pdfnet_amd: sft3 wants 3-channel rows and four (weight, bias) pairs")
        pc = [p.contiguous() for p in params]
        R = fea.numel() // 3
        out = torch.empty_like(fea)
        _L().pdf_sft3_fwd(ptr(fea), 3, ptr(cond), 3, *[ptr(p) for p in pc], ptr(out), 3, R, stream())
        ctx.save_for_backward(fea, cond, *pc)
        ctx.params = params
        return out

    @staticmethod
    def backward(ctx, g):
        fea, cond = ctx.saved_tensors[:2]
        pc = ctx.saved_tensors[2:]
        g = g.contiguous()
        R = fea.numel() // 3
        dfea = torch.empty_like(fea)
        dcond = torch.empty_like(cond) if ctx.needs_input_grad[1] else None
        ws = _ws(48 * 256, g.device)
        mg = [_main_grad(p, p) if ctx.needs_input_grad[2 + i] else None for i, p in enumerate(ctx.params)]
        direct = all(m is not None for m in mg)
        if direct:
            outs, ret = mg, [None] * 8
        else:
            outs = [torch.empty_like(p) if ctx.needs_input_grad[2 + i] else None for i, p in enumerate(pc)]
            ret = outs
        _L().pdf_sft3_bwd(ptr(g), 3, ptr(fea), 3, ptr(cond), 3, *[ptr(p) for p in pc], ptr(dfea), 3, ptr(dcond), 3,
                          *[ptr(o) for o in outs], 1 if direct else 0, ptr(ws), R, stream())
        return (dfea, dcond) + tuple(ret)


def sft3(fea, cond, params):
    return _SFT3.apply(fea, cond, *params)


class _GatherRows(Function):

    @staticmethod
    def forward(ctx, feat, ind, R, shift, ldo, chain=False):
        hip.require_gpu(feat, ind)
        feat_in = feat
        feat = cl(feat)
        B, C, H, W = feat.shape
        M = ind.shape[1]
        assert ind.dtype == torch.int64 and ind.stride(1) == 1
        out = torch.empty((B, M, ldo), device=feat.device)
        _L().pdf_gather_rows(ptr(feat), C, C, H * W, ptr(ind), ind.stride(0), B, M, R, shift, ptr(out), ldo, stream())
        ctx.save_for_backward(ind)
        ctx.cfg = (B, C, H, W, M, R, shift, ldo)
        ctx.set_materialize_grads(False)
        if chain:
            return out, feat_in.view_as(feat_in)
        return out

    @staticmethod
    def backward(ctx, g, dalias=None):
        (ind,) = ctx.saved_tensors
        B, C, H, W, M, R, shift, ldo = ctx.cfg
        if g is None:
            return dalias, None, None, None, None, None
        dfeat, extra = _chain_target(dalias, (B, C, H, W), g.device)
        _L().pdf_scatter_rows_add(ptr(g.contiguous()), ldo, C, H * W, ptr(ind), ind.stride(0), B, M, R, shift, ptr(dfeat), C, stream())
        if extra is not None:
            dfeat = dfeat + extra
        return dfeat, None, None, None, None, None


def _chain_target(dalias, shape, dev):
    if dalias is None:
        return _zeros_cl(shape, dev), None
    if tuple(dalias.shape) == tuple(shape) and dalias.dtype == torch.float32 and dalias.is_contiguous(memory_format=CL):
        return dalias, None
    return _zeros_cl(shape, dev), dalias


def gather_rows(feat, ind, R=1, shift=0, ldo=None, chain=False):
    return _GatherRows.apply(feat, ind, R, shift, ldo or feat.shape[1], chain)


class _WindowGather(Function):

    @staticmethod
    def forward(ctx, feat, ind, r, chain=False):
        hip.require_gpu(feat, ind)
# ... 1426 lines not shown
```

Before: 715.4.

## Emit x3 split dy planes from l2norm_cat backward for deconv backward

The l2norm_cat backward kernel now also writes its dx output as three-way bf16 split planes (unshuffled for the strided deconv layout) when the input came from an x3 deconv. The deconv backward data and weight passes reuse these planes instead of running their own split/unshuffle kernels on dy. This removes two extra passes over the gradient tensor, at the cost of more global writes and some LDS staging inside the l2norm backward, plus a separate plane buffer allocation.

```diff
diff --git a/include/pdfnet_hip.h b/include/pdfnet_hip.h
--- a/include/pdfnet_hip.h
+++ b/include/pdfnet_hip.h
@@ -285,6 +285,8 @@
     const void* op1_bf16_t;
     float* ws; long ws_floats;
     const float* wino_v;
+    void* dy_x3; long dy_x3_cs; long dy_x3_ld;
+    void* l2_x3[4]; long l2_x3_cs[4]; long l2_x3_ld[4]; int l2_x3_s[4]; int l2_x3_oh; int l2_x3_ow;
 } PdfCallOpts;
 long pdf_conv2d_winograd_v_offset(int N, int H, int W, int Cin, int Cout, int KH, int KW, int stride, int pad);
 int pdf_linear_fwd_x(const float* x, const float* w, const float* bias, float* y, int M, int N, int K, int ldx, int ldw, int ldy, int act, void* stream, PdfCallOpts* opts);
@@ -304,12 +306,14 @@
 int pdf_bn_train_bwd_x(const float* dy, int lddy, const float* y, int ldy, int relu, const float* x, int ldx, const float* save_mean, const float* save_rstd, const float* gamma, const float* scale, const float* shift, int C, long R, float* dx, int lddx, float* dres, int lddr, float* dgamma, float* dbeta, int accumulate, float* ws, void* stream, PdfCallOpts* opts);
 int pdf_bn_relu_maxk_fwd_x(const float* y, int ldy, int C, long R, int K, const float* gamma, const float* beta, float* running_mean, float* running_var, float momentum, float eps, int training, float* out, int ldo, int* arg, float* save_mean, float* save_rstd, float* scale, float* shift, float* ws, void* stream, PdfCallOpts* opts);
 int pdf_l2norm_cat_fwd_x(int nparts, const float* const* x, const int* C, const float* const* w, float eps, long R, float* y, int ldy, float* const* norm, void* stream, PdfCallOpts* opts);
+int pdf_l2norm_cat_bwd_planes_x(int nparts, const float* dy, int lddy, const float* const* x, const int* C, const float* const* w, float eps, long R, float* const* norm, float* const* dx, float* const* dw, void* const* dx16_or_null, void* stream, PdfCallOpts* opts);
 long pdf_conv2d_winograd_workspace_floats(int N, int H, int W, int Cin, int Cout, int KH, int KW, int stride, int pad, int backward);
 int pdf_debug_armed_slots(void);
 int pdf_debug_callopts_size(void);
 
 int pdf_x3_split(const float* x, void* out, long n, long cs, void* stream);
 long pdf_deconv2d_x3_workspace_floats(int N, int H, int W, int Cin, int Cout, int KH, int KW, int stride, int pad, int backward);
+long pdf_deconv2d_x3_dy_layout(int N, int H, int W, int Cin, int Cout, int KH, int KW, int stride, int pad, long* out);
 int pdf_set_x3_mode(int mode);
 int pdf_stream_create(void** out, int priority, int* lo, int* hi);
 int pdf_debug_x3_mode(void);
diff --git a/pdfnet_amd/csrc/gemm.hip b/pdfnet_amd/csrc/gemm.hip
--- a/pdfnet_amd/csrc/gemm.hip
+++ b/pdfnet_amd/csrc/gemm.hip
@@ -2140,7 +2140,7 @@
     if (KH * KW > MAX_TAPS) return PDF_E_BADARG;
     if (!g_gemm_bf16 && co.ws != nullptr && lddy == Cout && lddx >= Cin && aligned16(co.ws)) {
         const X3DeconvPlan plan = x3_deconv_plan(N, H, W, Cin, Cout, KH, KW, stride, pad, 1);
-        if (plan.ok && OH == plan.OH && OW == plan.OW && co.ws_floats >= plan.total) return pdf_internal_x3_deconv_bwd_data(plan, dy, w, dx, co.ws, lddx, lddy, s);
+        if (plan.ok && OH == plan.OH && OW == plan.OW && co.ws_floats >= plan.total) return pdf_internal_x3_deconv_bwd_data(plan, dy, w, dx, co.ws, lddx, lddy, x3_deconv_dy_planes(plan, co), s);
     }
     IGemm g = {};
     g.A = dy; g.B = w; g.C = dx; g.bias = nullptr; g.A16 = co.op0_bf16; g.B16 = co.op1_bf16;
@@ -2169,7 +2169,7 @@
     if (KH * KW > MAX_TAPS) return PDF_E_BADARG;
     if (!g_gemm_bf16 && co.ws != nullptr && ldx == Cin && lddy == Cout && aligned16(co.ws)) {
         const X3DeconvPlan plan = x3_deconv_plan(N, H, W, Cin, Cout, KH, KW, stride, pad, 2);
-        if (plan.ok && OH == plan.OH && OW == plan.OW && co.ws_floats >= plan.total) return pdf_internal_x3_deconv_bwd_weight(plan, x, dy, dw, co.ws, lddy, accumulate, s);
+        if (plan.ok && OH == plan.OH && OW == plan.OW && co.ws_floats >= plan.total) return pdf_internal_x3_deconv_bwd_weight(plan, x, dy, dw, co.ws, lddy, accumulate, x3_deconv_dy_planes(plan, co), s);
     }
     WGemm g = {};
     g.P = x; g.Q = dy; g.P16 = co.op0_bf16; g.Q16 = co.op1_bf16; g.M = N * H * W; g.NI = Cin; g.Cq = Cout; g.T = KH * KW;
diff --git a/pdfnet_amd/csrc/gemm_internal.h b/pdfnet_amd/csrc/gemm_internal.h
--- a/pdfnet_amd/csrc/gemm_internal.h
+++ b/pdfnet_amd/csrc/gemm_internal.h
@@ -51,5 +51,6 @@
 };
 X3DeconvPlan x3_deconv_plan(int N, int H, int W, int Cin, int Cout, int KH, int KW, int stride, int pad, int pass);
 int pdf_internal_x3_deconv_fwd(const X3DeconvPlan& p, const float* x, const float* w, const float* bias, float* y, float* ws, int ldy, hipStream_t s);
-int pdf_internal_x3_deconv_bwd_data(const X3DeconvPlan& p, const float* dy, const float* w, float* dx, float* ws, int lddx, int lddy, hipStream_t s);
-int pdf_internal_x3_deconv_bwd_weight(const X3DeconvPlan& p, const float* x, const float* dy, float* dw, float* ws, int lddy, int accumulate, hipStream_t s);
+unsigned short* x3_deconv_dy_planes(const X3DeconvPlan& p, const PdfCallOpts& co);
+int pdf_internal_x3_deconv_bwd_data(const X3DeconvPlan& p, const float* dy, const float* w, float* dx, float* ws, int lddx, int lddy, unsigned short* dy3, hipStream_t s);
+int pdf_internal_x3_deconv_bwd_weight(const X3DeconvPlan& p, const float* x, const float* dy, float* dw, float* ws, int lddy, int accumulate, unsigned short* dy3, hipStream_t s);
diff --git a/pdfnet_amd/csrc/gemm_x3.hip b/pdfnet_amd/csrc/gemm_x3.hip
--- a/pdfnet_amd/csrc/gemm_x3.hip
+++ b/pdfnet_amd/csrc/gemm_x3.hip
@@ -758,6 +758,17 @@
 PDF_API long pdf_deconv2d_x3_workspace_floats(int N, int H, int W, int Cin, int Cout, int KH, int KW, int stride, int pad, int backward) {
     return pdf_debug_gemm_precision() ? 0 : x3_deconv_plan(N, H, W, Cin, Cout, KH, KW, stride, pad, backward).total;
 }
+PDF_API long pdf_deconv2d_x3_dy_layout(int N, int H, int W, int Cin, int Cout, int KH, int KW, int stride, int pad, long* out) {
+    if (pdf_debug_gemm_precision() || out == nullptr) return 0;
+    const X3DeconvPlan d = x3_deconv_plan(N, H, W, Cin, Cout, KH, KW, stride, pad, 1), g = x3_deconv_plan(N, H, W, Cin, Cout, KH, KW, stride, pad, 2);
+    if (!d.ok || !g.ok || d.general != g.general || d.a.ld != g.a.ld || d.a.cs != g.a.cs || d.a.len != g.a.len) return 0;
+    out[0] = d.a.cs; out[1] = d.a.ld; out[2] = d.general ? 1 : d.stride; out[3] = d.general;
+    return d.a.len;
+}
+unsigned short* x3_deconv_dy_planes(const X3DeconvPlan& p, const PdfCallOpts& co) {
+    if (co.dy_x3 == nullptr || co.dy_x3_cs != p.a.cs || co.dy_x3_ld != p.a.ld || ((uintptr_t)co.dy_x3 & 15)) return nullptr;
+    return reinterpret_cast<unsigned short*>(co.dy_x3);
+}
 static void x3_gemm_desc(X3Gemm& g, const void* A3, long csA, long lda, const void* B3, long csB, long ldb, float* C, int M, int N, int K, int ldc) {
     g = X3Gemm{};
     g.A = (const unsigned short*)A3; g.B = (const unsigned short*)B3; g.C = C;
@@ -833,20 +844,20 @@
     }
     return 0;
 }
-int pdf_internal_x3_deconv_bwd_data(const X3DeconvPlan& p, const float* dy, const float* w, float* dx, float* ws, int lddx, int lddy, hipStream_t s) {
+int pdf_internal_x3_deconv_bwd_data(const X3DeconvPlan& p, const float* dy, const float* w, float* dx, float* ws, int lddx, int lddy, unsigned short* dy3, hipStream_t s) {
     const int Cin = p.Cin, Cout = p.Cout;
     const long M = (long)p.N * p.H * p.W, Mout = (long)p.N * p.OH * p.OW, NT = (long)p.K * p.K * Cout;
     unsigned short* w3 = reinterpret_cast<unsigned short*>(ws + p.w.off);
-    unsigned short* d3 = reinterpret_cast<unsigned short*>(ws + p.a.off);
+    unsigned short* d3 = dy3 != nullptr ? dy3 : reinterpret_cast<unsigned short*>(ws + p.a.off);
     {
         KTimer kt("x3_split_rows_kernel", 0.0, 10.0 * NT * Cin, s);
         hipLaunchKernelGGL(x3_split_rows_kernel, dim3(grid_for(NT * Cin / 8, 256, 256 * 16)), dim3(256), 0, s, w, NT, w3, p.w.ld, p.w.cs, (long)Cin, (int)(NT / 8));
     }
     X3Gemm g;
     x3_gemm_desc(g, d3, p.a.cs, p.a.ld, w3, p.w.cs, p.w.ld, dx, (int)M, Cin, (int)NT, lddx);
-    if (!p.general) x3_split_unshuffle(dy, lddy, d3, p, s);
+    if (!p.general) { if (dy3 == nullptr) x3_split_unshuffle(dy, lddy, d3, p, s); }
     else {
-        {
+        if (dy3 == nullptr) {
             KTimer kt("x3_split_rows_kernel", 0.0, 10.0 * Mout * Cout, s);
             hipLaunchKernelGGL(x3_split_rows_kernel, dim3(grid_for(Mout * Cout / 8, 256, 256 * 16)), dim3(256), 0, s, dy, (long)lddy, d3, p.a.ld, p.a.cs, Mout, Cout / 8);
         }
@@ -865,22 +876,22 @@
         reinterpret_cast<float4*>(dw)[i] = v;
     }
 }
-int pdf_internal_x3_deconv_bwd_weight(const X3DeconvPlan& p, const float* x, const float* dy, float* dw, float* ws, int lddy, int accumulate, hipStream_t s) {
+int pdf_internal_x3_deconv_bwd_weight(const X3DeconvPlan& p, const float* x, const float* dy, float* dw, float* ws, int lddy, int accumulate, unsigned short* dy3, hipStream_t s) {
     const int Cin = p.Cin, Cout = p.Cout;
     const long M = (long)p.N * p.H * p.W, Mout = (long)p.N * p.OH * p.OW, NT = (long)p.K * p.K * Cout;
     unsigned short* x3 = reinterpret_cast<unsigned short*>(ws + p.w.off);
-    unsigned short* d3 = reinterpret_cast<unsigned short*>(ws + p.a.off);
+    unsigned short* d3 = dy3 != nullptr ? dy3 : reinterpret_cast<unsigned short*>(ws + p.a.off);
     hipLaunchKernelGGL(x3_split_rows_kernel, dim3(grid_for(M * Cin / 8, 256, 256 * 16)), dim3(256), 0, s, x, (long)Cin, x3, p.w.ld, p.w.cs, M, Cin / 8);
     X3Gemm g = {};
     g.A = x3; g.B = d3; g.C = dw;
     g.csA = p.w.cs; g.csB = p.a.cs; g.lda = (int)p.w.ld; g.ldb = (int)p.a.ld;
     g.M = Cin; g.N = (int)NT; g.K = (int)M; g.batch = 1; g.splits = 1; g.rows_per_split = (int)M; g.accum = accumulate;
     if (!p.general) {
-        x3_split_unshuffle(dy, lddy, d3, p, s);
+        if (dy3 == nullptr) x3_split_unshuffle(dy, lddy, d3, p, s);
         PDF_LAUNCH_CHECK();
         return x3_launch_tn_deconv(g, s);
     }
-    {
+    if (dy3 == nullptr) {
         KTimer kt("x3_split_rows_kernel", 0.0, 10.0 * Mout * Cout, s);
         hipLaunchKernelGGL(x3_split_rows_kernel, dim3(grid_for(Mout * Cout / 8, 256, 256 * 16)), dim3(256), 0, s, dy, (long)lddy, d3, p.a.ld, p.a.cs, Mout, Cout / 8);
     }
diff --git a/pdfnet_amd/csrc/norm.hip b/pdfnet_amd/csrc/norm.hip
--- a/pdfnet_amd/csrc/norm.hip
+++ b/pdfnet_amd/csrc/norm.hip
@@ -1046,6 +1046,8 @@
     const float* x[L2_MAXPARTS]; const float* w[L2_MAXPARTS]; float* norm[L2_MAXPARTS]; float* dx[L2_MAXPARTS]; float* dw[L2_MAXPARTS];
     unsigned short* dx16[L2_MAXPARTS];
     int C[L2_MAXPARTS], off[L2_MAXPARTS];
+    unsigned short* x3[L2_MAXPARTS]; long x3_cs[L2_MAXPARTS], x3_ld[L2_MAXPARTS]; int x3_s[L2_MAXPARTS];
+    int OH, OW;
 };
 __global__ __launch_bounds__(256) void l2norm_cat_fwd_kernel(const L2Parts p, long R, float eps, float* __restrict__ y, int ldy,
                                                              unsigned short* __restrict__ y16) {
@@ -1099,9 +1101,11 @@
         }
     }
 }
-template <int MAXV>
+template <int MAXV, bool X3>
 __global__ __launch_bounds__(256) void l2norm_cat_bwd_kernel(const L2Parts p, long R, float eps, const float* __restrict__ dy, int lddy) {
     __shared__ float sw[64 * MAXV];
+    __shared__ __attribute__((aligned(16))) float ex[X3 ? 4 : 1][X3 ? 64 * MAXV : 4];
+    unsigned short* __restrict__ x3 = X3 ? p.x3[blockIdx.y] : nullptr;
     const int q = blockIdx.y, C = p.C[q], lane = threadIdx.x & 63;
     const float* __restrict__ x = p.x[q]; const float* __restrict__ w = p.w[q]; const float* __restrict__ norm = p.norm[q];
     const float* __restrict__ g0 = dy + p.off[q];
@@ -1138,7 +1142,25 @@
                 const float on = __shfl_down(o, 1, 64);
                 if (c < C && (lane & 1) == 0) *reinterpret_cast<unsigned int*>(dx16 + r * C + c) = pdf_pk_bf16(o, on);
             }
+            if constexpr (X3) if (x3 != nullptr && c < C) ex[threadIdx.x >> 6][c] = o;
             acc[i] += g[i] * xv[i] * in;
+        }
+        if constexpr (X3) if (x3 != nullptr) {
+            const unsigned ru = (unsigned)__builtin_amdgcn_readfirstlane((int)r), s = (unsigned)p.x3_s[q], OW = (unsigned)p.OW, hw = (unsigned)p.OH * OW;
+            const unsigned n = ru / hw, rem = ru - n * hw, oy = rem / OW, ox = rem - oy * OW, qy = oy / s, qx = ox / s;
+            const long row = ((long)n * (p.OH / s) + qy) * (OW / s) + qx;
+            unsigned short* __restrict__ d = x3 + row * p.x3_ld[q] + (long)((oy - qy * s) * s + (ox - qx * s)) * C;
+            const long cs = p.x3_cs[q];
+            __builtin_amdgcn_wave_barrier();
+            for (int j = lane; 4 * j < C; j += 64) {
+                const float4 v = *reinterpret_cast<const float4*>(&ex[threadIdx.x >> 6][4 * j]);
+                uint2 h, m, l;
+                pdf_x3_split2(v.x, v.y, h.x, m.x, l.x); pdf_x3_split2(v.z, v.w, h.y, m.y, l.y);
+                *reinterpret_cast<uint2*>(d + 4 * j) = h;
+                *reinterpret_cast<uint2*>(d + cs + 4 * j) = m;
+                *reinterpret_cast<uint2*>(d + 2 * cs + 4 * j) = l;
+            }
+            __builtin_amdgcn_wave_barrier();
         }
     }
 #pragma unroll
@@ -1185,8 +1207,8 @@
     return pdf_call_plain(pdf_l2norm_cat_fwd_impl, nparts, x, C, w, eps, R, y, ldy, norm, stream);
 }
 
-PDF_API int pdf_l2norm_cat_bwd(int nparts, const float* dy, int lddy, const float* const* x, const int* C, const float* const* w, float eps, long R,
-                               float* const* norm, float* const* dx, float* const* dw, void* const* dx16, void* stream) {
+static int pdf_l2norm_cat_bwd_impl(int nparts, const float* dy, int lddy, const float* const* x, const int* C, const float* const* w, float eps, long R,
+                                   float* const* norm, float* const* dx, float* const* dw, void* const* dx16, void* stream, PdfCallOpts& co) {
     hipStream_t s = (hipStream_t)stream;
     if (R <= 0) return 0;
     L2Parts p = {};
@@ -1195,11 +1217,36 @@
         if (dx16[i] != nullptr && C[i] % 64) return PDF_E_BADARG;
         p.dx16[i] = reinterpret_cast<unsigned short*>(dx16[i]);
     }
+    bool planes = false;
+    for (int i = 0; i < nparts; ++i) {
+        if (co.l2_x3[i] == nullptr) continue;
+        const int sh = co.l2_x3_s[i], OH = co.l2_x3_oh, OW = co.l2_x3_ow;
+        const long cs = co.l2_x3_cs[i], ld = co.l2_x3_ld[i];
+        if (OH <= 0 || OW <= 0 || R % ((long)OH * OW) != 0 || R > 2147483647L || sh < 1 || OH % sh != 0 || OW % sh != 0 || C[i] % 4 != 0 || ld % 4 != 0 ||
+            cs % 4 != 0 || (reinterpret_cast<uintptr_t>(co.l2_x3[i]) & 7) != 0 || ld < (long)sh * sh * C[i] || cs < R / ((long)sh * sh) * ld)
+            return PDF_E_BADARG;
+        p.x3[i] = reinterpret_cast<unsigned short*>(co.l2_x3[i]); p.x3_cs[i] = cs; p.x3_ld[i] = ld; p.x3_s[i] = sh; p.OH = OH; p.OW = OW;
+        planes = true;
+    }
     int cmax = 0;
     for (int i = 0; i < nparts; ++i) cmax = max(cmax, C[i]);
     const dim3 grid(grid_for(R * 64, 256, 1024), nparts);
-    if (cmax <= 256) hipLaunchKernelGGL(l2norm_cat_bwd_kernel<4>, grid, dim3(256), 0, s, p, R, eps, dy, lddy);
-    else hipLaunchKernelGGL(l2norm_cat_bwd_kernel<L2_MAXV>, grid, dim3(256), 0, s, p, R, eps, dy, lddy);
-    PDF_LAUNCH_CHECK();
-    return 0;
-}
+    if (cmax <= 256) {
+        if (planes) hipLaunchKernelGGL((l2norm_cat_bwd_kernel<4, true>), grid, dim3(256), 0, s, p, R, eps, dy, lddy);
+        else hipLaunchKernelGGL((l2norm_cat_bwd_kernel<4, false>), grid, dim3(256), 0, s, p, R, eps, dy, lddy);
+    } else {
+        if (planes) hipLaunchKernelGGL((l2norm_cat_bwd_kernel<L2_MAXV, true>), grid, dim3(256), 0, s, p, R, eps, dy, lddy);
+        else hipLaunchKernelGGL((l2norm_cat_bwd_kernel<L2_MAXV, false>), grid, dim3(256), 0, s, p, R, eps, dy, lddy);
+    }
+    PDF_LAUNCH_CHECK();
+    return 0;
+}
+PDF_API int pdf_l2norm_cat_bwd_planes_x(int nparts, const float* dy, int lddy, const float* const* x, const int* C, const float* const* w, float eps, long R,
+                                        float* const* norm, float* const* dx, float* const* dw, void* const* dx16, void* stream, PdfCallOpts* opts) {
+    return pdf_call_x(opts, pdf_l2norm_cat_bwd_impl, nparts, dy, lddy, x, C, w, eps, R, norm, dx, dw, dx16, stream);
+}
+PDF_API int pdf_l2norm_cat_bwd(int nparts, const float* dy, int lddy, const float* const* x, const int* C, const float* const* w, float eps, long R,
+                               float* const* norm, float* const* dx, float* const* dw, void* const* dx16, void* stream) {
+    PdfCallOpts none = {};
+    return pdf_l2norm_cat_bwd_impl(nparts, dy, lddy, x, C, w, eps, R, norm, dx, dw, dx16, stream, none);
+}
diff --git a/pdfnet_amd/functional.py b/pdfnet_amd/functional.py
--- a/pdfnet_amd/functional.py
+++ b/pdfnet_amd/functional.py
@@ -213,6 +213,33 @@
     if not X3_DECONV or _GEMM_BF16 or KH != KW or stride < 2:
         return None, None
     return _ws_alloc(_ws_query("pdf_deconv2d_x3_workspace_floats", N, H, W, Cin, Cout, KH, KW, stride, pad, backward), dev)
+
+
+X3_DY_PLANES = _os.environ.get("PDFNET_X3_DY_PLANES", "1") != "0"
+
+
+def _x3_dy_layout(layer):
+    N, H, W, Cin, Cout, KH, KW, stride, pad = layer
+    if not (X3_DY_PLANES and X3_DECONV) or _GEMM_BF16 or KH != KW or stride < 2:
+        return None
+    v = _ws_sizes.get(("pdf_deconv2d_x3_dy_layout", layer))
+    if v is None:
+        out = (ctypes.c_long * 4)()
+        n = _L().pdf_deconv2d_x3_dy_layout(*layer, out)
+        v = _ws_sizes[("pdf_deconv2d_x3_dy_layout", layer)] = (n, out[0], out[1], out[2]) if n > 0 else ()
+    return v or None
+
+
+def attach_x3_planes(t, planes, layer, lay):
+    t._pdf_x3 = (planes, layer, lay, t._version)
+    return t
+
+
+def x3_planes_of(t, layer):
+    v = getattr(t, '_pdf_x3', None)
+    if v is None or v[3] != t._version or v[1] != layer or v[2] != _x3_dy_layout(layer):
+        return None
+    return v[0]
 
 
 WINOGRAD_KEEP_V = _os.environ.get("PDFNET_WINOGRAD_KEEP_V", "1") != "0"
@@ -619,6 +646,8 @@
         ws, nws = _x3_deconv_ws(N, H, W, Cin, Cout, KH, KW, stride, pad, 0, x.device)
         L.pdf_deconv2d_fwd_x(ptr(x), ptr(w), ptr(b), ptr(y), N, H, W, Cin, Cin, Cout, KH, KW, stride, pad, OH, OW, Cout, stream(),
                              _O(op0_bf16=ptr(x16), op1_bf16=ptr(w16), ws=ptr(ws), ws_floats=nws)[1])
+        if ws is not None and (ctx.needs_input_grad[0] or ctx.needs_input_grad[1]):
+            y._pdf_x3_dy = (N, H, W, Cin, Cout, KH, KW, stride, pad)
         ctx.save_for_backward(x, w)
         ctx.s16 = (x16, w16)
         ctx.cfg = (stride, pad, b is not None)
@@ -635,21 +664,24 @@
         g = cl(dy)
         x16, w16 = ctx.s16
         g16 = shadow_of(g)
+        g3 = x3_planes_of(g, (N, H, W, Cin, Cout, KH, KW, stride, pad))
+        g3p, g3cs, g3ld = (ptr(g3), ) + _x3_dy_layout((N, H, W, Cin, Cout, KH, KW, stride, pad))[1:3] if g3 is not None else (None, None, None)
         L = _L()
         dx = dw = db = None
         if ctx.needs_input_grad[0]:
             dx = torch.empty_like(x)
             ws, nws = _x3_deconv_ws(N, H, W, Cin, Cout, KH, KW, stride, pad, 1, x.device)
             L.pdf_deconv2d_bwd_data_x(ptr(g), ptr(w), ptr(dx), N, H, W, Cin, Cin, Cout, KH, KW, stride, pad, OH, OW, Cout, stream(),
-                                      _O(op0_bf16=ptr(g16), op1_bf16=ptr(w16), ws=ptr(ws), ws_floats=nws)[1])
+                                      _O(op0_bf16=ptr(g16), op1_bf16=ptr(w16), ws=ptr(ws), ws_floats=nws, dy_x3=g3p, dy_x3_cs=g3cs, dy_x3_ld=g3ld)[1])
         w_par, b_par = ctx.params
 
         def launch_w(out, out_b, acc):
             ws, n = _wgrad_ws(N * H * W, Cin, KH * KW * Cout, x.device)
             xws, nx = _x3_deconv_ws(N, H, W, Cin, Cout, KH, KW, stride, pad, 2, x.device)
             L.pdf_deconv2d_bwd_weight_x(ptr(x), ptr(g), ptr(out), ptr(ws), n, N, H, W, Cin, Cin, Cout, KH, KW,
-                                        stride, pad, OH, OW, Cout, acc, stream(), _O(op0_bf16=ptr(x16), op1_bf16=ptr(g16), ws=ptr(xws), ws_floats=nx)[1])
-        dw, db = _param_grads(ctx, x, g, w, w_par, b_par, has_b, launch_w, Cout, N * OH * OW, 2.0 * N * H * W * Cin * KH * KW * Cout, shadows=(x16, g16))
+                                        stride, pad, OH, OW, Cout, acc, stream(),
+                                        _O(op0_bf16=ptr(x16), op1_bf16=ptr(g16), ws=ptr(xws), ws_floats=nx, dy_x3=g3p, dy_x3_cs=g3cs, dy_x3_ld=g3ld)[1])
+        dw, db = _param_grads(ctx, x, g, w, w_par, b_par, has_b, launch_w, Cout, N * OH * OW, 2.0 * N * H * W * Cin * KH * KW * Cout, shadows=(x16, g16, g3))
         return dx, dw, db, None, None
 
 
@@ -1100,6 +1132,7 @@
         _L().pdf_l2norm_cat_fwd_x(n, _ptr_array(xs), _int_array(Cs), _ptr_array(ws), eps, R, ptr(out), Ct, _ptr_array(norms), stream(), _O(out_bf16=ptr(out16))[1])
         ctx.save_for_backward(*xs, *ws, *norms)
         ctx.cfg = (eps, n, Cs)
+        ctx.x3_dy = [getattr(a, '_pdf_x3_dy', None) if a is x else None for a, x in zip(args[:n], xs)]
         return out
 
     @staticmethod
@@ -1114,11 +1147,26 @@
         d16 = [new_shadow(d) for d in dxs] if all(C % 64 == 0 for C in Cs) and _os.environ.get('PDFNET_L2_SHADOW', '1') != '0' else None
         if d16 is not None and d16[0] is None:
             d16 = None
-        _L().pdf_l2norm_cat_bwd(n, ptr(g), Ct, _ptr_array(xs), _int_array(Cs), _ptr_array(ws), eps, R, _ptr_array(norms),
-                                _ptr_array(dxs), _ptr_array(dws), _ptr_array(d16) if d16 is not None else None, stream())
+        o3, planes = None, [None] * n
+        for q, layer in enumerate(ctx.x3_dy):
+            lay = _x3_dy_layout(layer) if layer is not None and ctx.needs_input_grad[1 + q] else None
+            B, _, OH, OW = xs[q].shape
+            if lay is None or (B, Cs[q], OH, OW) != (layer[0], layer[4], (layer[1] - 1) * layer[7] - 2 * layer[8] + layer[5], (layer[2] - 1) * layer[7] - 2 * layer[8] + layer[6]):
+                continue
+            if o3 is None:
+                o3 = _CallOpts()
+                o3.l2_x3_oh, o3.l2_x3_ow = OH, OW
+            planes[q] = torch.empty(lay[0], dtype=torch.float32, device=g.device)
+            o3.l2_x3[q], o3.l2_x3_cs[q], o3.l2_x3_ld[q], o3.l2_x3_s[q] = planes[q].data_ptr(), lay[1], lay[2], lay[3]
+        _L().pdf_l2norm_cat_bwd_planes_x(n, ptr(g), Ct, _ptr_array(xs), _int_array(Cs), _ptr_array(ws), eps, R, _ptr_array(norms),
+                                         _ptr_array(dxs), _ptr_array(dws), _ptr_array(d16) if d16 is not None else None, stream(),
+                                         _byref(o3) if o3 is not None else None)
         if d16 is not None:
             for d, s16 in zip(dxs, d16):
                 attach_shadow(d, s16)
+        for q, pl in enumerate(planes):
+            if pl is not None:
+                attach_x3_planes(dxs[q], pl, ctx.x3_dy[q], _x3_dy_layout(ctx.x3_dy[q]))
         return (None,) + tuple(dxs) + tuple(dws)
 
 
```

New measurement: 714.6. About the same (-0.1%).
